# BaZzz01010101/ReflaxMan

Measured on AMD Instinct MI355X. Metric: Mrays/sec at 3840×2160 depth-8; max per-channel |Δ| vs CPU reference, higher is better.
Workload: dtype f32; 1 GPU; C3 synth16: 16 spheres + 4 textured triangles + sun, 3840x2160, depth 8, 1 spp; scene=synth16, width=3840, height=2160, depth=8, spp=1, parallelism=single-gpu

## Files before the change

### include/rfx.h

```cpp
#ifndef RFX_H
#define RFX_H
#include <stddef.h>
#include <stdint.h>

#ifdef __cplusplus
extern "C" {
#endif

#define RFX_ABI_VERSION 4

typedef enum {
  RFX_OK = 0,
  RFX_ERR_ARG = -1,
  RFX_ERR_HIP = -2,
  RFX_ERR_STATE = -3,
  RFX_ERR_IO = -4,
  RFX_ERR_RNG = -5,
  RFX_ERR_NODEV = -6
} rfx_status;

enum { RFX_METAL = 0, RFX_DIELECTRIC = 1 };

typedef struct rfx_scene rfx_scene;
typedef struct rfx_renderer rfx_renderer;
// ... 6 lines not shown
rfx_scene *rfx_scene_create(float diff_r, float diff_g, float diff_b, float diff_power);
void rfx_scene_destroy(rfx_scene *scene);
int rfx_scene_add_sphere(rfx_scene *scene, const float center[3], float radius, int material_type,
                         const float rgb[3], float reflectivity, float transparency);
int rfx_scene_add_triangle(rfx_scene *scene, const float v1[3], const float v2[3], const float v3[3],
                           int material_type, const float rgb[3], float reflectivity, float transparency);
int rfx_scene_add_mesh(rfx_scene *scene, const float *vertices, uint32_t n_vertices, const uint32_t *indices,
                       uint32_t n_triangles, int material_type, const float rgb[3], float reflectivity,
                       float transparency);
int rfx_scene_add_plane(rfx_scene *scene, const float pos[3], const float norm[3], int material_type,
                        const float rgb[3], float reflectivity, float transparency);
int rfx_scene_plane_count(const rfx_scene *scene);
int rfx_triangle_set_texture(rfx_scene *scene, int object_index, int texture_index, const float uv[6]);
int rfx_scene_add_light(rfx_scene *scene, const float origin[3], float radius, const float rgb[3], float power);
int rfx_scene_add_texture_argb(rfx_scene *scene, uint32_t width, uint32_t height, const uint32_t *argb);
int rfx_scene_add_texture_file(rfx_scene *scene, const char *path, int *loaded);
int rfx_scene_set_skybox_file(rfx_scene *scene, const char *path);
int rfx_scene_set_skybox_argb(rfx_scene *scene, uint32_t width, uint32_t height, const uint32_t *argb);
int rfx_scene_counts(const rfx_scene *scene, int *spheres, int *triangles, int *lights, int *textures);
int rfx_scene_tri_bvh_dump(const rfx_scene *scene, int32_t counts[5], float *boxes, int32_t *children,
                           int32_t *leaf_ids, int32_t *residual);
int rfx_scene_set_tri_mates(rfx_scene *scene, int on);
int rfx_scene_tri_mates(const rfx_scene *scene, int32_t *leader, float *plane);

void rfx_camera_view(const float eye[3], const float at[3], float view[9]);
float rfx_camera_rz(uint32_t width, float fov);

int rfx_tga_load(const char *path, uint32_t *width, uint32_t *height, uint32_t *argb, size_t capacity);
int rfx_tga_save(const char *path, uint32_t width, uint32_t height, const uint32_t *argb);
int rfx_bmp_save(const char *path, uint32_t width, uint32_t height, const uint32_t *argb);
void rfx_argb_from_rgb(const float *rgb, size_t pixels, uint32_t *argb);

int rfx_renderer_create(rfx_renderer **out, int device);
void rfx_renderer_destroy(rfx_renderer *r);
int rfx_renderer_device(const rfx_renderer *r);
int rfx_renderer_set_stream(rfx_renderer *r, void *hip_stream);
int rfx_renderer_set_scene(rfx_renderer *r, const rfx_scene *scene);
int rfx_renderer_set_tile_order(rfx_renderer *r, int mode);
int rfx_renderer_set_regroup(rfx_renderer *r, int park_after);
int rfx_renderer_set_regroup_sort(rfx_renderer *r, int on);
int rfx_renderer_bounce_form(const rfx_renderer *r);
int rfx_renderer_set_tri_accel(rfx_renderer *r, int mode);
typedef struct {
  int32_t tri_nodes, tri_depth;
  int32_t tri_leaf_size;
  int32_t tri_in_leaves;
  int32_t tri_residual;
  int32_t sph_nodes, sph_depth;
  int32_t narrow_tri_bvh;
} rfx_accel_info;
int rfx_renderer_accel_info(const rfx_renderer *r, rfx_accel_info *out);
int rfx_renderer_set_prim_masks(rfx_renderer *r, int mode);
int rfx_renderer_set_prim_exact(rfx_renderer *r, int on);
int rfx_renderer_get_prim_masks(rfx_renderer *r, uint64_t *host, uint64_t capacity, uint64_t *words);
int rfx_renderer_set_rng(rfx_renderer *r, uint32_t sphere_seed, uint32_t jitter_seed);
int rfx_renderer_get_rng(rfx_renderer *r, uint32_t *sphere_seed, uint32_t *jitter_seed);

typedef struct {
  float eye[3];
  float view[9];
  float fov;
  uint32_t width, height;
  int32_t reflect_num;
  int32_t sample_num;
  int32_t additive;
  int32_t additive_counter;
  uint32_t row_block;
  uint32_t rank, nranks;
  uint64_t pixel_begin;
  uint64_t pixel_end;
  uint64_t span_begin;
  uint64_t span_end;
} rfx_frame;

uint32_t rfx_strip_rows(uint32_t height, uint32_t row_block, uint32_t rank, uint32_t nranks);
uint32_t rfx_strip_row_to_y(uint32_t r, uint32_t row_block, uint32_t rank, uint32_t nranks);

#define RFX_NCOUNTERS 40
int rfx_render_frame(rfx_renderer *r, const rfx_frame *frame, float *d_rgb, uint32_t *d_argb,
                     uint64_t *d_counters, void *stream);
int rfx_renderer_set_launch_traces(rfx_renderer *r, uint64_t max_traces);
int rfx_renderer_set_rng_prepass(rfx_renderer *r, int mode);
int rfx_renderer_prepass_form(const rfx_renderer *r);
uint32_t rfx_rng_triple_index(uint32_t state);
uint32_t rfx_rng_seq_blocks(void);

int rfx_frame_rng_blocks(rfx_renderer *r, const rfx_frame *frame, uint32_t nslices, uint64_t *blocks_per_slice);
int rfx_frame_rng_count(rfx_renderer *r, const rfx_frame *frame, uint32_t slice, uint32_t nslices,
                        uint32_t *d_blk_counts, void *stream);
int rfx_render_frame_counted(rfx_renderer *r, const rfx_frame *frame, uint32_t nslices, const uint32_t *d_blk_counts,
                             float *d_rgb, uint32_t *d_argb, uint64_t *d_counters, void *stream);
int rfx_render_frame_counted_ev(rfx_renderer *r, const rfx_frame *frame, uint32_t nslices,
                                const uint32_t *d_blk_counts, float *d_rgb, uint32_t *d_argb, uint64_t *d_counters,
                                void *stream, void *emitted_event);

int rfx_frame_rng_emit(rfx_renderer *r, const rfx_frame *frame, uint32_t nslices, const uint32_t *d_blk_counts,
                       void *stream, void *emitted_event);
int rfx_render_frame_emitted(rfx_renderer *r, const rfx_frame *frame, float *d_rgb, uint32_t *d_argb,
                             uint64_t *d_counters, void *stream);
int rfx_frame_rng_discard(rfx_renderer *r);
int rfx_frame_rng_pending(rfx_renderer *r, uint32_t *frame_start);

int rfx_frame_rng_rewind(rfx_renderer *r);

typedef struct rfx_group rfx_group;
int rfx_group_create(rfx_group **out, const int *devices, int n);
void rfx_group_destroy(rfx_group *g);
int rfx_group_size(const rfx_group *g);
rfx_renderer *rfx_group_renderer(rfx_group *g, int member);
int rfx_group_set_scene(rfx_group *g, const rfx_scene *scene);
int rfx_group_set_bands(rfx_group *g, uint32_t height, const uint32_t *bounds);
int rfx_group_get_bands(const rfx_group *g, uint32_t *bounds);
int rfx_group_render_frame(rfx_group *g, const rfx_frame *frame, float *d_rgb, uint32_t *d_argb, void *stream);

int rfx_renderer_set_timing(rfx_renderer *r, int enable);
int rfx_renderer_get_timing(rfx_renderer *r, double *prepass_ms, double *trace_ms, uint64_t *frames);

int rfx_render_frame_host(rfx_renderer *r, const rfx_frame *frame, float *rgb, uint32_t *argb,
                          uint64_t *counters);

int rfx_device_alloc(rfx_renderer *r, size_t bytes, void **dptr);
int rfx_device_free(rfx_renderer *r, void *dptr);
int rfx_memcpy_d2h(rfx_renderer *r, void *dst, const void *src, size_t bytes);
int rfx_memcpy_h2d(rfx_renderer *r, void *dst, const void *src, size_t bytes);
int rfx_memcpy_d2d(rfx_renderer *r, void *dst, const void *src, size_t bytes);
int rfx_synchronize(rfx_renderer *r);

int rfx_rand_dirs(rfx_renderer *r, uint32_t seed, uint64_t n, float *out3, uint32_t *seed_out);

int rfx_kat_objects(rfx_renderer *r, const float *rays, const int32_t *objects, uint64_t n, float *out);
int rfx_kat_texels(rfx_renderer *r, int texture, const float *in, uint64_t n, float *out);
int rfx_kat_powf(rfx_renderer *r, const float *xy, uint64_t n, float *out);
int rfx_kat_argb(rfx_renderer *r, const float *rgb, uint64_t n, uint32_t *out);
int rfx_kat_powf_cube(rfx_renderer *r, uint64_t counts[2]);
int rfx_kat_div(rfx_renderer *r, uint64_t first, uint64_t n, uint64_t counts[3]);
int rfx_kat_kernarg(rfx_renderer *r, int swapped, uint32_t out[3]);
int rfx_kat_rng_seq_prefix(rfx_renderer *r, uint32_t *prefix);
int rfx_kat_rng_seq_legacy(rfx_renderer *r, uint32_t *counts);

#ifdef __cplusplus
}
#endif
#endif
```

### reflaxman_amd/_lib.py

```python
from __future__ import annotations

import ctypes as C
import os

from . import _build

RFX_OK = 0
RFX_NCOUNTERS = 40
RFX_ABI_VERSION = 4
METAL, DIELECTRIC = 0, 1

_fp = C.POINTER(C.c_float)
_u32p = C.POINTER(C.c_uint32)
_u64p = C.POINTER(C.c_uint64)


class RfxError(RuntimeError):
    pass


class Frame(C.Structure):
    _fields_ = [
        ("eye", C.c_float * 3), ("view", C.c_float * 9), ("fov", C.c_float),
        ("width", C.c_uint32), ("height", C.c_uint32),
        ("reflect_num", C.c_int32), ("sample_num", C.c_int32),
        ("additive", C.c_int32), ("additive_counter", C.c_int32),
        ("row_block", C.c_uint32), ("rank", C.c_uint32), ("nranks", C.c_uint32),
        ("pixel_begin", C.c_uint64), ("pixel_end", C.c_uint64),
        ("span_begin", C.c_uint64), ("span_end", C.c_uint64),
    ]


class AccelInfo(C.Structure):
    _fields_ = [(n, C.c_int32) for n in ("tri_nodes", "tri_depth", "tri_leaf_size", "tri_in_leaves", "tri_residual",
                                         "sph_nodes", "sph_depth", "narrow_tri_bvh")]


_i32p = C.POINTER(C.c_int32)

SIGNATURES = [
    ("rfx_abi_version", C.c_int, []),
    ("rfx_last_error", C.c_char_p, []),
    ("rfx_build_options", C.c_int, []),
    ("rfx_scene_create", C.c_void_p, [C.c_float] * 4),
    ("rfx_scene_destroy", None, [C.c_void_p]),
    ("rfx_scene_add_sphere", C.c_int, [C.c_void_p, _fp, C.c_float, C.c_int, _fp, C.c_float, C.c_float]),
    ("rfx_scene_add_triangle", C.c_int, [C.c_void_p, _fp, _fp, _fp, C.c_int, _fp, C.c_float, C.c_float]),
    ("rfx_scene_add_mesh", C.c_int, [C.c_void_p, _fp, C.c_uint32, _u32p, C.c_uint32, C.c_int, _fp, C.c_float, C.c_float]),
    ("rfx_scene_tri_bvh_dump", C.c_int, [C.c_void_p, _i32p, _fp, _i32p, _i32p, _i32p]),
    ("rfx_scene_set_tri_mates", C.c_int, [C.c_void_p, C.c_int]),
    ("rfx_scene_tri_mates", C.c_int, [C.c_void_p, _i32p, _fp]),
    ("rfx_scene_add_plane", C.c_int, [C.c_void_p, _fp, _fp, C.c_int, _fp, C.c_float, C.c_float]),
    ("rfx_scene_plane_count", C.c_int, [C.c_void_p]),
    ("rfx_triangle_set_texture", C.c_int, [C.c_void_p, C.c_int, C.c_int, _fp]),
    ("rfx_scene_add_light", C.c_int, [C.c_void_p, _fp, C.c_float, _fp, C.c_float]),
    ("rfx_scene_add_texture_argb", C.c_int, [C.c_void_p, C.c_uint32, C.c_uint32, _u32p]),
    ("rfx_scene_add_texture_file", C.c_int, [C.c_void_p, C.c_char_p, C.POINTER(C.c_int)]),
    ("rfx_scene_set_skybox_file", C.c_int, [C.c_void_p, C.c_char_p]),
    ("rfx_scene_set_skybox_argb", C.c_int, [C.c_void_p, C.c_uint32, C.c_uint32, _u32p]),
    ("rfx_scene_counts", C.c_int, [C.c_void_p] + [C.POINTER(C.c_int)] * 4),
    ("rfx_camera_view", None, [_fp, _fp, _fp]),
    ("rfx_camera_rz", C.c_float, [C.c_uint32, C.c_float]),
    ("rfx_tga_load", C.c_int, [C.c_char_p, _u32p, _u32p, _u32p, C.c_size_t]),
    ("rfx_tga_save", C.c_int, [C.c_char_p, C.c_uint32, C.c_uint32, _u32p]),
    ("rfx_bmp_save", C.c_int, [C.c_char_p, C.c_uint32, C.c_uint32, _u32p]),
    ("rfx_argb_from_rgb", None, [_fp, C.c_size_t, _u32p]),
    ("rfx_renderer_create", C.c_int, [C.POINTER(C.c_void_p), C.c_int]),
    ("rfx_renderer_destroy", None, [C.c_void_p]),
    ("rfx_renderer_device", C.c_int, [C.c_void_p]),
    ("rfx_renderer_set_stream", C.c_int, [C.c_void_p, C.c_void_p]),
    ("rfx_renderer_set_scene", C.c_int, [C.c_void_p, C.c_void_p]),
    ("rfx_renderer_set_rng", C.c_int, [C.c_void_p, C.c_uint32, C.c_uint32]),
    ("rfx_renderer_get_rng", C.c_int, [C.c_void_p, _u32p, _u32p]),
    ("rfx_strip_rows", C.c_uint32, [C.c_uint32] * 4),
    ("rfx_strip_row_to_y", C.c_uint32, [C.c_uint32] * 4),
    ("rfx_render_frame", C.c_int, [C.c_void_p, C.POINTER(Frame), C.c_void_p, C.c_void_p, C.c_void_p, C.c_void_p]),
    ("rfx_render_frame_host", C.c_int, [C.c_void_p, C.POINTER(Frame), _fp, _u32p, _u64p]),
    ("rfx_frame_rng_blocks", C.c_int, [C.c_void_p, C.POINTER(Frame), C.c_uint32, _u64p]),
    ("rfx_frame_rng_count", C.c_int, [C.c_void_p, C.POINTER(Frame), C.c_uint32, C.c_uint32, C.c_void_p, C.c_void_p]),
    ("rfx_render_frame_counted", C.c_int, [C.c_void_p, C.POINTER(Frame), C.c_uint32, C.c_void_p, C.c_void_p,
                                           C.c_void_p, C.c_void_p, C.c_void_p]),
    ("rfx_render_frame_counted_ev", C.c_int, [C.c_void_p, C.POINTER(Frame), C.c_uint32, C.c_void_p, C.c_void_p,
                                              C.c_void_p, C.c_void_p, C.c_void_p, C.c_void_p]),
    ("rfx_frame_rng_emit", C.c_int, [C.c_void_p, C.POINTER(Frame), C.c_uint32, C.c_void_p, C.c_void_p, C.c_void_p]),
    ("rfx_render_frame_emitted", C.c_int, [C.c_void_p, C.POINTER(Frame), C.c_void_p, C.c_void_p, C.c_void_p,
                                           C.c_void_p]),
    ("rfx_frame_rng_discard", C.c_int, [C.c_void_p]),
    ("rfx_frame_rng_pending", C.c_int, [C.c_void_p, _u32p]),
    ("rfx_frame_rng_rewind", C.c_int, [C.c_void_p]),
    ("rfx_group_create", C.c_int, [C.POINTER(C.c_void_p), C.POINTER(C.c_int), C.c_int]),
    ("rfx_group_destroy", None, [C.c_void_p]),
    ("rfx_group_size", C.c_int, [C.c_void_p]),
    ("rfx_group_renderer", C.c_void_p, [C.c_void_p, C.c_int]),
    ("rfx_group_set_scene", C.c_int, [C.c_void_p, C.c_void_p]),
    ("rfx_group_set_bands", C.c_int, [C.c_void_p, C.c_uint32, _u32p]),
    ("rfx_group_get_bands", C.c_int, [C.c_void_p, _u32p]),
    ("rfx_group_render_frame", C.c_int, [C.c_void_p, C.POINTER(Frame), C.c_void_p, C.c_void_p, C.c_void_p]),
    ("rfx_renderer_set_timing", C.c_int, [C.c_void_p, C.c_int]),
    ("rfx_renderer_set_tile_order", C.c_int, [C.c_void_p, C.c_int]),
    ("rfx_renderer_set_prim_masks", C.c_int, [C.c_void_p, C.c_int]),
    ("rfx_renderer_set_prim_exact", C.c_int, [C.c_void_p, C.c_int]),
    ("rfx_renderer_get_prim_masks", C.c_int, [C.c_void_p, _u64p, C.c_uint64, _u64p]),
    ("rfx_renderer_set_regroup", C.c_int, [C.c_void_p, C.c_int]),
    ("rfx_renderer_set_regroup_sort", C.c_int, [C.c_void_p, C.c_int]),
    ("rfx_renderer_set_launch_traces", C.c_int, [C.c_void_p, C.c_uint64]),
    ("rfx_renderer_bounce_form", C.c_int, [C.c_void_p]),
    ("rfx_renderer_set_rng_prepass", C.c_int, [C.c_void_p, C.c_int]),
    ("rfx_renderer_prepass_form", C.c_int, [C.c_void_p]),
    ("rfx_rng_triple_index", C.c_uint32, [C.c_uint32]),
    ("rfx_rng_seq_blocks", C.c_uint32, []),
    ("rfx_renderer_set_tri_accel", C.c_int, [C.c_void_p, C.c_int]),
    ("rfx_renderer_accel_info", C.c_int, [C.c_void_p, C.POINTER(AccelInfo)]),
    ("rfx_renderer_get_timing", C.c_int, [C.c_void_p, C.POINTER(C.c_double), C.POINTER(C.c_double), _u64p]),
    ("rfx_device_alloc", C.c_int, [C.c_void_p, C.c_size_t, C.POINTER(C.c_void_p)]),
    ("rfx_device_free", C.c_int, [C.c_void_p, C.c_void_p]),
    ("rfx_memcpy_d2h", C.c_int, [C.c_void_p, C.c_void_p, C.c_void_p, C.c_size_t]),
    ("rfx_memcpy_h2d", C.c_int, [C.c_void_p, C.c_void_p, C.c_void_p, C.c_size_t]),
    ("rfx_memcpy_d2d", C.c_int, [C.c_void_p, C.c_void_p, C.c_void_p, C.c_size_t]),
    ("rfx_synchronize", C.c_int, [C.c_void_p]),
    ("rfx_rand_dirs", C.c_int, [C.c_void_p, C.c_uint32, C.c_uint64, _fp, _u32p]),
    ("rfx_kat_objects", C.c_int, [C.c_void_p, _fp, C.POINTER(C.c_int32), C.c_uint64, _fp]),
    ("rfx_kat_texels", C.c_int, [C.c_void_p, C.c_int, _fp, C.c_uint64, _fp]),
    ("rfx_kat_powf", C.c_int, [C.c_void_p, _fp, C.c_uint64, _fp]),
    ("rfx_kat_argb", C.c_int, [C.c_void_p, _fp, C.c_uint64, _u32p]),
    ("rfx_kat_powf_cube", C.c_int, [C.c_void_p, C.POINTER(C.c_uint64)]),
    ("rfx_kat_div", C.c_int, [C.c_void_p, C.c_uint64, C.c_uint64, C.POINTER(C.c_uint64)]),
    ("rfx_kat_kernarg", C.c_int, [C.c_void_p, C.c_int, C.POINTER(C.c_uint32)]),
    ("rfx_kat_rng_seq_prefix", C.c_int, [C.c_void_p, _u32p]),
    ("rfx_kat_rng_seq_legacy", C.c_int, [C.c_void_p, _u32p]),
]

_lib = None


def lib_path() -> str:
    return _build.LIB


def bind(path: str, partial: bool = False):
    L = C.CDLL(os.path.abspath(path))
    for name, res, args in SIGNATURES:
        if partial and not hasattr(L, name):
            continue
        fn = getattr(L, name)
        fn.restype = res
        fn.argtypes = args
    return L


def load(build_if_missing: bool = True):
    global _lib
    if _lib is not None:
        return _lib
    path = _build.LIB
    if build_if_missing:
        try:
            _build.build()
        except Exception as e:
            if not os.path.exists(path):
                raise RfxError(f"librfx.so missing and cannot be built: {e}") from e
    if not os.path.exists(path):
        raise RfxError(f"librfx.so not found at {path}: the HIP renderer is required (no CPU fallback)")
    L = C.CDLL(path)
    for name, res, args in SIGNATURES:
        fn = getattr(L, name)
        fn.restype = res
        fn.argtypes = args
    if L.rfx_abi_version() != RFX_ABI_VERSION:
        raise RfxError("librfx.so ABI version mismatch")
    _lib = L
    return L


def lib_sha256(path: str = None) -> str:
    import hashlib
    with open(path or _build.LIB, "rb") as f:
        return hashlib.sha256(f.read()).hexdigest()


# ... 40 lines not shown
```

### reflaxman_amd/csrc/rfx_host.cpp

```cpp
#include <string.h>

#include <algorithm>

#include "rfx_internal.h"
#include "rfx_math.h"

#pragma clang fp contract(off)

using namespace rfx;

extern "C" int rfx_abi_version(void) { return RFX_ABI_VERSION; }

#ifndef RFX_TILE_ORDER_DEFAULT
#define RFX_TILE_ORDER_DEFAULT 1
#endif
#ifndef RFX_TILE_ORDER_MIN_TILES
#define RFX_TILE_ORDER_MIN_TILES 49152
#endif
#ifndef RFX_PRIM_SSAA
#define RFX_PRIM_SSAA 0
#endif
#ifndef RFX_PRIM_LANES
#define RFX_PRIM_LANES 1
#endif
// ... 153 lines not shown
  if (r->tile_stream) (void)hipStreamSynchronize(r->tile_stream);
  if (r->tile_fork) (void)hipEventDestroy(r->tile_fork);
  if (r->tile_join) (void)hipEventDestroy(r->tile_join);
  if (r->tile_stream) (void)hipStreamDestroy(r->tile_stream);
  if (r->split_stream)
  {
    (void)hipStreamSynchronize(r->split_stream);
    (void)hipStreamDestroy(r->split_stream);
  }
  for (hipEvent_t e : r->split_ev)
    if (e) (void)hipEventDestroy(e);
  if (r->own_stream) (void)hipStreamDestroy(r->own_stream);
  delete r;
}

extern "C" int rfx_build_options(void)
{
  return (RFX_PRIM_LARGE ? RFX_BUILD_PRIM_LARGE : 0) | (RFX_PRIM_SSAA ? RFX_BUILD_PRIM_SSAA : 0) |
         (RFX_PRIM_LANES ? RFX_BUILD_PRIM_LANES : 0) | (RFX_ONE_LIGHT ? RFX_BUILD_ONE_LIGHT : 0) |
         (RFX_BVH_LEAF_PAIRS << 8);
}

extern "C" int rfx_renderer_set_launch_traces(rfx_renderer *r, uint64_t max_traces)
{
  if (!r) return fail(RFX_ERR_ARG, "renderer_set_launch_traces: null renderer");
  r->launch_traces = max_traces ? std::min(max_traces, kMaxLaunchTraces) : (uint64_t)RFX_LAUNCH_TRACES;
  return RFX_OK;
}

extern "C" int rfx_renderer_device(const rfx_renderer *r) { return r ? r->device : -1; }

extern "C" int rfx_renderer_set_tile_order(rfx_renderer *r, int mode)
{
  if (!r || mode < 0 || mode > 3) return fail(RFX_ERR_ARG, "renderer_set_tile_order: mode 0, 1, 2 or 3");
  r->tile_mode = mode;
  return RFX_OK;
}

extern "C" int rfx_renderer_set_prim_masks(rfx_renderer *r, int mode)
{
  if (!r || mode < 0 || mode > 2) return fail(RFX_ERR_ARG, "renderer_set_prim_masks: mode 0, 1 or 2");
  r->prim_mode = mode;
  r->prim_key.clear();
  r->prim_seen.clear();
  return RFX_OK;
}

extern "C" int rfx_renderer_set_prim_exact(rfx_renderer *r, int on)
{
  if (!r || on < 0 || on > 1) return fail(RFX_ERR_ARG, "renderer_set_prim_exact: 0 or 1");
  r->prim_exact = on;
  r->prim_key.clear();
  return RFX_OK;
}

extern "C" int rfx_renderer_get_prim_masks(rfx_renderer *r, uint64_t *host, uint64_t capacity, uint64_t *words)
{
  if (!r || !words) return fail(RFX_ERR_ARG, "renderer_get_prim_masks: null argument");
  int rc;
  if ((rc = set_dev(r)) != RFX_OK) return rc;
  const uint64_t n = r->prim_key.empty() ? 0 : r->prim_words;
  *words = n;
  if (!n || !host) return RFX_OK;
  if (capacity < n) return fail(RFX_ERR_ARG, "renderer_get_prim_masks: the host array is too short");
  HIP_CHECK(hipStreamSynchronize(r->prim_on));
  HIP_CHECK(hipMemcpy(host, r->prim_mask.p, n * sizeof(uint64_t), hipMemcpyDeviceToHost));
  return RFX_OK;
}

extern "C" int rfx_renderer_set_rng_prepass(rfx_renderer *r, int mode)
{
  if (!r || mode < 0 || mode > 1) return fail(RFX_ERR_ARG, "renderer_set_rng_prepass: mode 0 or 1");
  r->rng_prepass = mode;
  return RFX_OK;
}

extern "C" int rfx_renderer_prepass_form(const rfx_renderer *r)
{
  if (!r) return fail(RFX_ERR_ARG, "renderer_prepass_form: null renderer");
  return r->rng.prepass_form;
}

extern "C" uint32_t rfx_rng_triple_index(uint32_t state) { return rng_seq_index_of(state); }

extern "C" int rfx_renderer_bounce_form(const rfx_renderer *r)
{
  if (!r) return fail(RFX_ERR_ARG, "renderer_bounce_form: null renderer");
  return r->bounce_form;
}

extern "C" int rfx_renderer_set_regroup(rfx_renderer *r, int park_after)
{
  if (!r || park_after < -1) return fail(RFX_ERR_ARG, "renderer_set_regroup: -1 (default), 0 (off) or segments >= 1");
  r->park_after = park_after;
  return RFX_OK;
}

extern "C" int rfx_renderer_set_regroup_sort(rfx_renderer *r, int on)
{
  if (!r || on < 0 || on > 1) return fail(RFX_ERR_ARG, "renderer_set_regroup_sort: 0 or 1");
  r->queue_sort = on;
  return RFX_OK;
}

extern "C" int rfx_renderer_set_stream(rfx_renderer *r, void *s)
{
  if (!r) return fail(RFX_ERR_ARG, "set_stream: null renderer");
  r->stream = s ? (hipStream_t)s : r->own_stream;
  return RFX_OK;
}

template <class T>
static int upload(rfx_renderer *r, const std::vector<T> &v, const T **dst)
{
  if (v.empty()) { *dst = nullptr; return RFX_OK; }
  void *p = nullptr;
  HIP_CHECK(hipMalloc(&p, v.size() * sizeof(T)));
  r->scene_allocs.push_back(p);
  HIP_CHECK(hipMemcpy(p, v.data(), v.size() * sizeof(T), hipMemcpyHostToDevice));
  *dst = (const T *)p;
  return RFX_OK;
}

extern "C" int rfx_renderer_set_tri_accel(rfx_renderer *r, int mode)
{
  if (!r || mode < -1 || mode > 2)
    return fail(RFX_ERR_ARG, "renderer_set_tri_accel: -1 (automatic), 0 (off), 1 (on) or 2 (on, narrow bundles too)");
  r->tri_accel = mode;
  return RFX_OK;
}

extern "C" int rfx_renderer_accel_info(const rfx_renderer *r, rfx_accel_info *out)
{
  if (!r || !out) return fail(RFX_ERR_ARG, "renderer_accel_info: bad args");
  if (!r->has_scene) return fail(RFX_ERR_STATE, "renderer_accel_info: no scene");
  *out = r->accel;
  return RFX_OK;
}

extern "C" int rfx_renderer_set_scene(rfx_renderer *r, const rfx_scene *s)
{
  if (!r || !s) return fail(RFX_ERR_ARG, "set_scene: bad args");
  int rc;
  if ((rc = set_dev(r)) != RFX_OK) return rc;
  HIP_CHECK(hipStreamSynchronize(r->stream));
  free_scene(r);
  const SceneBuild B(*s, r->tri_accel);
  DevScene d = B.d;
  if ((rc = upload(r, B.sg, &d.sph_geo)) || (rc = upload(r, B.sp, &d.sph_pair)) || (rc = upload(r, B.sm, &d.sph_mat)) ||
      (rc = upload(r, B.si, &d.sph_info)) || (rc = upload(r, B.tg, &d.tri_geo)) || (rc = upload(r, B.ts, &d.tri_shade)) ||
      (rc = upload(r, B.tm, &d.tri_mat)) || (rc = upload(r, B.lr, &d.lights)) || (rc = upload(r, B.tr, &d.texs)) ||
      (rc = upload(r, B.pool, &d.texels)) || (rc = upload(r, B.bd, &d.bound)) || (rc = upload(r, B.cs, &d.cull_small)) ||
      (rc = upload(r, B.ct, &d.cull_tri)) || (rc = upload(r, B.cb, &d.chunk_bound)) || (rc = upload(r, B.pg, &d.pln_geo)) ||
      (rc = upload(r, B.pm, &d.pln_mat)) || (rc = upload(r, B.loc, &d.obj_loc)) || (rc = upload(r, B.bvh, &d.bvh)) ||
      (rc = upload(r, B.tt.nodes, &d.tri_bvh)) || (rc = upload(r, B.tleaf, &d.tri_leaf)) ||
      (rc = upload(r, B.tt.resid, &d.tri_resid)) || (rc = upload(r, B.aux, &d.bvh_aux)))
    return rc;
  r->accel = B.accel;
  r->dev = d;
  r->has_scene = true;
  ++r->scene_gen;
  r->prim_key.clear();
  r->prim_seen.clear();
  return RFX_OK;
}

extern "C" int rfx_renderer_set_rng(rfx_renderer *r, uint32_t sphere_seed, uint32_t jitter_seed)
{
  if (!r) return fail(RFX_ERR_ARG, "set_rng: null renderer");
  int rc;
  if ((rc = set_dev(r)) != RFX_OK) return rc;
  HIP_CHECK(hipMemcpyAsync(r->rng.cur(), &sphere_seed, sizeof(uint32_t), hipMemcpyHostToDevice, r->stream));
  HIP_CHECK(hipStreamSynchronize(r->stream));
  r->jitter_seed = jitter_seed;
  r->rng.rewind_ok = false;
  r->rng.reset(false);
  return RFX_OK;
}

extern "C" int rfx_renderer_get_rng(rfx_renderer *r, uint32_t *sphere_seed, uint32_t *jitter_seed)
{
  if (!r) return fail(RFX_ERR_ARG, "get_rng: null renderer");
  int rc;
  if ((rc = set_dev(r)) != RFX_OK) return rc;
  uint32_t s = 0;
  int err = 0;
  HIP_CHECK(hipMemcpyAsync(&s, r->rng.cur(), sizeof(uint32_t), hipMemcpyDeviceToHost, r->stream));
  HIP_CHECK(hipMemcpyAsync(&err, r->err, sizeof(int), hipMemcpyDeviceToHost, r->stream));
  HIP_CHECK(hipStreamSynchronize(r->stream));
  if (err & 1) return fail(RFX_ERR_RNG, "RNG pre-pass ran short of accepted triples");
  if (sphere_seed) *sphere_seed = s;
  if (jitter_seed) *jitter_seed = r->jitter_seed;
  return RFX_OK;
}

static uint64_t rng_layout(uint64_t traces, uint32_t nslices, uint64_t *per_slice)
{
  if (!nslices) nslices = 1;
  const uint64_t bps = (rng_blocks_for(traces) + nslices - 1) / nslices;
  if (per_slice) *per_slice = bps;
  return bps * nslices;
}

static int ensure_rng_workspace(rfx_renderer *r, uint64_t traces, uint64_t nblk)
{
  int rc;
  if ((rc = r->rd.reserve(traces)) < 0) return rc;
  if (nblk <= r->blk_cnt.cap) return RFX_OK;
  r->blk_cnt.release();
  if ((rc = r->rng_status.reserve(nblk)) < 0 || (rc = r->blk_off.reserve(nblk)) < 0 ||
      (rc = r->tile_sum.reserve(nblk / 4096 + 1)) < 0 || (rc = r->rng_range.reserve(4)) < 0 ||
// ... 75 lines not shown
  uint32_t grid_rows, row0;
  if (f->sample_num < 0)
  {
    const uint64_t n = (uint64_t)(-f->sample_num);
    const uint64_t bw = (W + n - 1) / n;
    auto corners_before = [&](uint64_t p) -> uint64_t {
      const uint64_t y = p / W, x = p % W;
      return (y + n - 1) / n * bw + (y % n == 0 ? (x + n - 1) / n : 0);
    };
    trace_base = corners_before(p0);
    traces = corners_before(p1) - trace_base;
    row0 = (uint32_t)(y0 / n);
    grid_rows = (uint32_t)(y1 / n - y0 / n + 1);
  }
  else
  {
    traces = (p1 - p0) * (uint64_t)(f->sample_num * f->sample_num);
    row0 = nranks > 1 ? 0 : y0;
    grid_rows = nranks > 1 ? rfx_strip_rows(H, f->row_block, f->rank, nranks) : y1 - y0 + 1;
    if (band)
    {
      row0 = (uint32_t)(f->pixel_begin / W);
      grid_rows = (uint32_t)((f->pixel_end - f->pixel_begin) / W);
    }
  }
  if (traces > kMaxLaunchTraces)
    return fail(RFX_ERR_ARG, "render_frame: %llu traces in one launch exceed 2^31 (partitions: a smaller span)",
                (unsigned long long)traces);
  plan.traces = traces;
  plan.st = st;
  FrameParams &P = plan.P;
  P = FrameParams{};
  P.eye_x = f->eye[0]; P.eye_y = f->eye[1]; P.eye_z = f->eye[2];
  P.v11 = f->view[0]; P.v12 = f->view[1]; P.v13 = f->view[2];
  P.v21 = f->view[3]; P.v22 = f->view[4]; P.v23 = f->view[5];
  P.v31 = f->view[6]; P.v32 = f->view[7]; P.v33 = f->view[8];
  P.rz = rfx_camera_rz(W, f->fov);
  P.wh = W / 2.0f;
  P.hh = H / 2.0f;
  P.W = W; P.H = H;
  P.depth = f->reflect_num;
  P.ss = f->sample_num;
  P.accumulate = f->sample_num > 0 && f->additive_counter > 1;
  P.additive = f->sample_num > 0 && f->additive;
  P.jitter_seed = r->jitter_seed;
  P.row_block = f->row_block ? f->row_block : 1;
  P.rank = nranks > 1 && !band ? f->rank : 0;
  P.nranks = band ? 1 : nranks;
  P.grid_rows = grid_rows;
  P.row0 = row0;
  P.p_begin = p0;
  P.p_end = p1;
  P.trace_base = trace_base;
  return RFX_OK;
}

extern "C" int rfx_frame_rng_blocks(rfx_renderer *r, const rfx_frame *f, uint32_t nslices, uint64_t *per_slice)
{
  FramePlan pl;
  int rc;
  if ((rc = plan_frame(r, f, nullptr, pl)) != RFX_OK) return rc;
  if (!nslices || !per_slice) return fail(RFX_ERR_ARG, "frame_rng_blocks: nslices > 0 and an output required");
  rng_layout(pl.traces, nslices, per_slice);
  return RFX_OK;
}

extern "C" int rfx_frame_rng_count(rfx_renderer *r, const rfx_frame *f, uint32_t slice, uint32_t nslices,
                                   uint32_t *d_blk_counts, void *stream)
{
  FramePlan pl;
  int rc;
  if ((rc = plan_frame(r, f, stream, pl)) != RFX_OK) return rc;
  if (!d_blk_counts || !nslices || slice >= nslices) return fail(RFX_ERR_ARG, "frame_rng_count: bad slice");
  uint64_t bps = 0;
  const uint64_t nblk = rng_layout(pl.traces, nslices, &bps);
  if ((rc = ensure_rng_workspace(r, pl.rd_traces(), nblk)) != RFX_OK) return rc;
  HIP_CHECK(launch_rng_count(r->rng.cur(), r->jump, d_blk_counts, (uint64_t)slice * bps, bps, nullptr, pl.st));
  return RFX_OK;
}

static int tile_schedule(rfx_renderer *r, FrameParams &P, hipStream_t st, uint64_t &key, bool &record)
{
  int rc;
  const uint32_t n = trace_tiles(P);
  key = ((uint64_t)P.W << 40) ^ ((uint64_t)P.grid_rows << 16) ^ ((uint64_t)(uint32_t)P.ss << 4) ^
        (uint64_t)(P.additive * 2 + P.accumulate);
  if (!r->tile_stream)
  {
    HIP_CHECK(hipStreamCreateWithFlags(&r->tile_stream, hipStreamNonBlocking));
    HIP_CHECK(hipEventCreateWithFlags(&r->tile_fork, hipEventDisableTiming));
    HIP_CHECK(hipEventCreateWithFlags(&r->tile_join, hipEventDisableTiming));
  }
  if ((rc = r->tile_scratch.reserve(tile_order_scratch() / sizeof(uint32_t))) < 0) return rc;
  if (n > r->tile_cost.cap)
  {
    HIP_CHECK(hipStreamSynchronize(r->tile_stream));
    if (r->tile_pending) HIP_CHECK(hipEventSynchronize(r->tile_join));
    HIP_CHECK(hipStreamSynchronize(st));
    r->tile_n = 0;
    r->tile_pending = false;
    r->tile_cost.release();
    if ((rc = r->tile_order.reserve(n)) < 0 || (rc = r->tile_cost.reserve(n)) < 0) return rc;
  }
  if (r->tile_pending && r->tile_waited != st)
  {
    HIP_CHECK(hipStreamWaitEvent(st, r->tile_join, 0));
// ... 139 lines not shown
    DevBuf<uint64_t> &mask = r->split_mask[pl.split_side];
    if ((rc = mask.reserve((size_t)trace_tiles(P) * kPrimStride)) < 0) return rc;
    HIP_CHECK(launch_prim_cull(r->dev, P, mask, r->prim_exact != 0, st));
    P.prim_mask = mask;
    P.prim_shadow = 0;
  }
  else if (((small && (plain || (RFX_PRIM_LANES && (trace_lanes(P) || chunks)) || (RFX_PRIM_SSAA && P.ss >= 1)) &&
             !park) ||
            (RFX_PRIM_LARGE && !small && plain)) &&
           !stats && P.grid_rows && r->prim_mode && !pl.split)
  {
    struct Key { float cam[15]; uint32_t W, H, grid_rows, row0, row_block, rank, nranks; int32_t depth, ss, additive;
                 uint64_t p_begin, p_end, gen; } k;
    memset(&k, 0, sizeof(k));
    const float cam[15] = {P.eye_x, P.eye_y, P.eye_z, P.v11, P.v12, P.v13, P.v21, P.v22, P.v23,
                           P.v31, P.v32, P.v33, P.rz, P.wh, P.hh};
    memcpy(k.cam, cam, sizeof(cam));
    k.W = P.W; k.H = P.H; k.grid_rows = P.grid_rows; k.row0 = P.row0; k.row_block = P.row_block; k.rank = P.rank;
    k.nranks = P.nranks; k.depth = P.depth > 0 ? 1 : 0; k.p_begin = P.p_begin; k.p_end = P.p_end; k.gen = r->scene_gen;
    k.ss = P.ss; k.additive = P.additive ? 1 : 0;
    std::vector<uint8_t> kb((const uint8_t *)&k, (const uint8_t *)&k + sizeof(k));
    if ((rc = r->prim_mask.reserve((size_t)trace_tiles(P) * (small ? kPrimStride : kPrimLargeStride))) < 0) return rc;
    if (rc)
    {
      r->prim_key.clear();
      r->prim_seen.clear();
    }
    if (r->prim_mode == 2 || kb != r->prim_key)
    {
      const bool repeat = kb == r->prim_seen;
      r->prim_seen = kb;
      r->prim_key.clear();
      if (repeat || r->prim_mode == 2 || chunks)
      {
        HIP_CHECK(launch_prim_cull(r->dev, P, r->prim_mask, r->prim_exact != 0, st));
        r->prim_key = kb;
        r->prim_words = (size_t)trace_tiles(P) * (small ? kPrimStride : kPrimLargeStride);
        r->prim_on = st;
      }
    }
    if (!r->prim_key.empty())
    {
      P.prim_mask = r->prim_mask;
      P.prim_shadow = P.additive || chunks ? 0 : 1;
    }
  }
  return RFX_OK;
}

static int launch_trace_and_bounce(rfx_renderer *r, FramePlan &pl, bool small, bool park, bool sort_queue, bool stats)
{
  const FrameParams &P = pl.P;
  const hipStream_t st = pl.st;
  if (P.grid_rows) HIP_CHECK(launch_trace(r->dev, P, stats, st));
  r->bounce_form = 0;
  if (!park) return RFX_OK;
  const uint64_t waves = (pl.traces + 63) / 64;
  const uint32_t groups = (uint32_t)std::min<uint64_t>((waves + 1) / 2, (uint64_t)r->cus * RFX_BOUNCE_GROUPS_PER_CU);
  const int cfg = kCfgCull | (r->dev.n_light > 32 ? kCfgManyLights : 0) | (small ? kCfgSmall : 0) |
                  (r->dev.n_pln ? kCfgPlanes : 0) | (RFX_ONE_LIGHT && r->dev.n_light == 1 ? kCfgOneLight : 0) |
                  (RFX_TRI_BVH && r->dev.tri_bvh ? kCfgTriBvh : 0);
  if (sort_queue) HIP_CHECK(launch_queue_sort(r->qctr, r->qkey, r->qctr.p + 2, r->qorder, st));
  const uint32_t lgroups = (uint32_t)std::min<uint64_t>((waves + kLdsBvhWaves - 1) / kLdsBvhWaves, (uint64_t)r->cus);
  r->bounce_form = 2;
  if (small || !lds_bvh_fits(r->dev.n_bvh) || launch_bounce_lds(cfg, lgroups, r->dev, P, st) != hipSuccess)
  {
    (void)hipGetLastError();
    launch_bounce(cfg, dim3(groups), r->dev, P, st);
    r->bounce_form = 1;
  }
  HIP_CHECK(hipGetLastError());
  return RFX_OK;
}

static int record_tile_sort(rfx_renderer *r, const FramePlan &pl, uint64_t key)
{
  const hipStream_t st = pl.st;
  const uint32_t n = trace_tiles(pl.P);
#if RFX_TILE_SORT_MAIN
  HIP_CHECK(launch_tile_order(r->tile_cost, n, r->tile_order, r->tile_scratch, st));
  HIP_CHECK(hipEventRecord(r->tile_join, st));
  r->tile_waited = st;
#else
  HIP_CHECK(hipEventRecord(r->tile_fork, st));
  HIP_CHECK(hipStreamWaitEvent(r->tile_stream, r->tile_fork, 0));
  HIP_CHECK(launch_tile_order(r->tile_cost, n, r->tile_order, r->tile_scratch, r->tile_stream));
  HIP_CHECK(hipEventRecord(r->tile_join, r->tile_stream));
  r->tile_waited = nullptr;
#endif
  r->tile_pending = true;
  r->tile_n = n;
  r->tile_key = key;
  return RFX_OK;
}

static int trace_frame(rfx_renderer *r, FramePlan &pl, const uint32_t *rd, float *d_rgb, uint32_t *d_argb,
                       uint64_t *d_counters)
{
  int rc;
  FrameParams &P = pl.P;
  const bool stats = d_counters != nullptr;
  P.img = d_rgb;
  P.argb = d_argb;
  P.rd_state = pl.band ? rd - pl.band_lo : rd;
  P.counters = (unsigned long long *)d_counters;
  const bool small = r->dev.n_sph <= 32 && r->dev.n_tri <= 32;
  const bool plain = P.ss == 1 && !P.additive && !P.accumulate;
// ... 339 lines not shown
```

### reflaxman_amd/csrc/rfx_internal.h

```cpp
#pragma once
#include <hip/hip_runtime.h>
#include <stdint.h>

#include <vector>

#include "rfx_launch.h"
#include "rfx_scene.h"

#define HIP_CHECK(expr)                                                                          \
  do {                                                                                           \
    hipError_t e_ = (expr);                                                                      \
    if (e_ != hipSuccess) return rfx::fail(RFX_ERR_HIP, "%s: %s", #expr, hipGetErrorString(e_)); \
  } while (0)
#define RCHECK(expr)               \
  do {                             \
    int rc_ = (expr);              \
    if (rc_ != RFX_OK) return rc_; \
  } while (0)

namespace rfx {

template <class T>
struct DevBuf {
  T *p = nullptr;
// ... 68 lines not shown

}

struct rfx_renderer {
  rfx_renderer();
  int device = 0;
  int cus = 256;
  hipStream_t own_stream = nullptr;
  hipStream_t stream = nullptr;
  rfx::DevScene dev{};
  std::vector<void *> scene_allocs;
  bool has_scene = false;
  rfx::RngState rng;
  rfx::DevBuf<int> err;
  uint32_t jitter_seed = 0;
  rfx::DevBuf<uint32_t> rd;
  rfx::DevBuf<uint32_t> rd_alt;
  int emit_pending = -1;
  int trace_buf = 0;
  bool split_alt_busy = false;
  uint64_t emit_key[10] = {};
  uint64_t launch_traces;
  hipStream_t split_stream = nullptr;
  hipEvent_t split_ev[3] = {nullptr, nullptr, nullptr};
  rfx::DevBuf<uint32_t> blk_cnt, rng_range, tile_sum, jump;
  rfx::DevBuf<uint64_t> blk_off;
  rfx::DevBuf<uint16_t> rng_masks;
  rfx::DevBuf<unsigned long long> rng_status, rng_ticket;
  unsigned long long rng_tickets = 0;
  uint32_t rng_epoch = 0;
  rfx::DevBuf<uint32_t> seq_hdr, seq_state, seq_p, seq_tiles;
  bool seq_built = false;
  int rng_prepass;
  rfx::DevBuf<float> img;
  rfx::DevBuf<uint32_t> argb;
  rfx::DevBuf<uint64_t> cnt;
  int tile_mode;
  rfx::DevBuf<uint32_t> tile_cost, tile_order, tile_scratch;
  uint32_t tile_n = 0;
  uint64_t tile_key = 0;
  hipStream_t tile_stream = nullptr;
  hipEvent_t tile_fork = nullptr, tile_join = nullptr;
  bool tile_pending = false;
  hipStream_t tile_waited = nullptr;
  uint64_t tile_count = 0;
  int park_after = -1;
  rfx::DevBuf<uint64_t> prim_mask;
  rfx::DevBuf<uint64_t> split_mask[2];
  std::vector<uint8_t> prim_key;
  std::vector<uint8_t> prim_seen;
  uint64_t scene_gen = 0;
  int prim_mode = 1;
  int prim_exact = 1;
  size_t prim_words = 0;
  hipStream_t prim_on = nullptr;
  int tri_accel = -1;
  rfx_accel_info accel{};
  int bounce_form = 0;
  rfx::DevBuf<rfx::QRay> queue;
  rfx::DevBuf<uint32_t> qctr, qkey, qorder;
  int queue_sort;
  bool timing = false, timing_this = false;
  uint32_t timing_every = 1;
  uint64_t timing_seq = 0;
  std::vector<hipEvent_t> events;
  size_t events_used = 0;
};

namespace rfx {
int set_dev(rfx_renderer *r);
int ensure_seq_table(rfx_renderer *r, hipStream_t st);
int save_rewind_state(rfx_renderer *r, hipStream_t st);
}
```

### reflaxman_amd/csrc/rfx_kat.cpp

```cpp
#include <algorithm>
#include <string>
#include <vector>

#include "rfx_internal.h"

using namespace rfx;

static int named(const char *who, int rc)
{
  const std::string cause = rfx_last_error();
  return fail(rc, "%s: %s", who, cause.c_str());
}

template <class T>
static int kat_buffer(DevBuf<T> &dev, size_t n, const T *src)
{
  int rc;
  if ((rc = dev.reserve(n ? n : 1)) < 0) return rc;
  if (src && n) HIP_CHECK(hipMemcpy(dev, src, n * sizeof(T), hipMemcpyHostToDevice));
  return RFX_OK;
}

static int kat_run(rfx_renderer *r, int what, int tex, const void *in, size_t in_elems, const int32_t *objs,
                   uint64_t n, void *out, size_t out_elems)
// ... 26 lines not shown
  if (!r->has_scene) return fail(RFX_ERR_STATE, "kat_texels: no scene uploaded");
  if (texture >= r->dev.n_tex) return fail(RFX_ERR_ARG, "kat_texels: texture %d", texture);
  return kat_run(r, 1, texture, in, (size_t)n * (texture >= 0 ? 2 : 3), nullptr, n, out, (size_t)n * 3);
}

extern "C" int rfx_kat_powf(rfx_renderer *r, const float *xy, uint64_t n, float *out)
{
  if (!r || (n && (!xy || !out))) return fail(RFX_ERR_ARG, "kat_powf: bad args");
  return kat_run(r, 2, 0, xy, (size_t)n * 2, nullptr, n, out, (size_t)n);
}

extern "C" int rfx_kat_argb(rfx_renderer *r, const float *rgb, uint64_t n, uint32_t *out)
{
  if (!r || (n && (!rgb || !out))) return fail(RFX_ERR_ARG, "kat_argb: bad args");
  return kat_run(r, 3, 0, rgb, (size_t)n * 3, nullptr, n, out, (size_t)n);
}

extern "C" int rfx_kat_powf_cube(rfx_renderer *r, uint64_t counts[2])
{
  if (!r || !counts) return fail(RFX_ERR_ARG, "kat_powf_cube: bad args");
  DevBuf<unsigned long long> d;
  int rc;
  if ((rc = d.reserve(2)) < 0) return named("kat_powf_cube", rc);
  hipError_t e = hipMemsetAsync(d, 0, 2 * sizeof(unsigned long long), r->stream);
  for (uint64_t first = 0; e == hipSuccess && first <= 0x3f800000ull; first += 1ull << 28)
    e = launch_kat_powf_cube((uint32_t)first, (uint32_t)std::min<uint64_t>(1ull << 28, 0x3f800001ull - first), d, r->stream);
  unsigned long long h[2] = {0, 0};
  if (e == hipSuccess) e = hipStreamSynchronize(r->stream);
  if (e == hipSuccess) e = hipMemcpy(h, d, sizeof(h), hipMemcpyDeviceToHost);
  if (e != hipSuccess) return fail(RFX_ERR_HIP, "kat_powf_cube: %s", hipGetErrorString(e));
  counts[0] = h[0];
  counts[1] = h[1];
  return RFX_OK;
}

extern "C" int rfx_kat_div(rfx_renderer *r, uint64_t first, uint64_t n, uint64_t counts[3])
{
  if (!r || !counts) return fail(RFX_ERR_ARG, "kat_div: bad args");
  RCHECK(set_dev(r));
  DevBuf<unsigned long long> d;
  int rc;
  if ((rc = d.reserve(3)) < 0) return named("kat_div", rc);
  hipError_t e = hipMemsetAsync(d, 0, 3 * sizeof(unsigned long long), r->stream);
  for (uint64_t k = 0; e == hipSuccess && k < n; k += 1ull << 28)
    e = launch_kat_div(first + k, (uint32_t)std::min<uint64_t>(1ull << 28, n - k), d, r->stream);
  unsigned long long h[3] = {0, 0, 0};
  if (e == hipSuccess) e = hipStreamSynchronize(r->stream);
  if (e == hipSuccess) e = hipMemcpy(h, d, sizeof(h), hipMemcpyDeviceToHost);
  if (e != hipSuccess) return fail(RFX_ERR_HIP, "kat_div: %s", hipGetErrorString(e));
  for (int i = 0; i < 3; ++i) counts[i] = h[i];
  return RFX_OK;
}

extern "C" uint32_t rfx_rng_seq_blocks(void) { return rng_seq_blocks(); }

extern "C" int rfx_kat_rng_seq_prefix(rfx_renderer *r, uint32_t *prefix)
{
  if (!r || !prefix) return fail(RFX_ERR_ARG, "kat_rng_seq_prefix: bad args");
  RCHECK(set_dev(r));
  RCHECK(ensure_seq_table(r, r->stream));
  HIP_CHECK(hipStreamSynchronize(r->stream));
  HIP_CHECK(hipMemcpy(prefix, r->seq_p, ((size_t)rng_seq_blocks() + 1) * sizeof(uint32_t), hipMemcpyDeviceToHost));
  return RFX_OK;
}

extern "C" int rfx_kat_rng_seq_legacy(rfx_renderer *r, uint32_t *counts)
{
  if (!r || !counts) return fail(RFX_ERR_ARG, "kat_rng_seq_legacy: bad args");
  RCHECK(set_dev(r));
  const uint64_t nb = rng_seq_blocks();
  std::vector<uint32_t> jump(2 * (256 + nb));
  rng_jump_table(nb, jump.data());
  DevBuf<uint32_t> d_jump, d_cnt, d_origin;
  int rc;
  if ((rc = d_jump.reserve(jump.size())) < 0 || (rc = d_cnt.reserve(nb)) < 0 || (rc = d_origin.reserve(1)) < 0)
    return named("kat_rng_seq_legacy", rc);
  hipError_t e = hipMemcpy(d_jump, jump.data(), jump.size() * sizeof(uint32_t), hipMemcpyHostToDevice);
  if (e == hipSuccess) e = hipMemset(d_origin, 0, sizeof(uint32_t));
  if (e == hipSuccess) e = launch_rng_count(d_origin, d_jump, d_cnt, 0, nb, nullptr, r->stream);
  if (e == hipSuccess) e = hipStreamSynchronize(r->stream);
  if (e == hipSuccess) e = hipMemcpy(counts, d_cnt, nb * sizeof(uint32_t), hipMemcpyDeviceToHost);
  if (e != hipSuccess) return fail(RFX_ERR_HIP, "kat_rng_seq_legacy: %s", hipGetErrorString(e));
  return RFX_OK;
}

extern "C" int rfx_kat_kernarg(rfx_renderer *r, int swapped, uint32_t out[3])
{
  if (!r || !out) return fail(RFX_ERR_ARG, "kat_kernarg: bad args");
  if (!r->has_scene) return fail(RFX_ERR_STATE, "kat_kernarg: no scene uploaded");
  RCHECK(set_dev(r));
  FrameParams P;
  uint32_t *w = (uint32_t *)&P;
  for (size_t i = 0; i < sizeof(P) / 4; ++i) w[i] = 0x9E3779B9u * (uint32_t)(i + 1);
  DevBuf<uint32_t> d;
  int rc;
  if ((rc = d.reserve(3)) < 0) return named("kat_kernarg", rc);
  hipError_t e = hipMemsetAsync(d, 0xFF, 3 * sizeof(uint32_t), r->stream);
  if (e == hipSuccess) e = launch_kat_kernarg(r->dev, P, swapped, d, r->stream);
  if (e == hipSuccess) e = hipStreamSynchronize(r->stream);
  if (e == hipSuccess) e = hipMemcpy(out, d, 3 * sizeof(uint32_t), hipMemcpyDeviceToHost);
  if (e != hipSuccess) return fail(RFX_ERR_HIP, "kat_kernarg: %s", hipGetErrorString(e));
  return RFX_OK;
}
```

### reflaxman_amd/csrc/rfx_kernels.hip

```cpp
#include "rfx_trace.h"

#include <vector>

#pragma clang fp contract(off)

namespace rfx {

constexpr int kLptThreads = 1024, kLptBuckets = 256, kLptGroups = 64;

__device__ __forceinline__ uint32_t lpt_key(const uint32_t *cost, uint32_t i)
{
  const uint32_t c = max(cost[i], 1u);
  const uint32_t e = 31u - (uint32_t)__clz(c);
  const uint32_t m = e >= 3u ? (c >> (e - 3u)) & 7u : (c << (3u - e)) & 7u;
  return (uint32_t)(kLptBuckets - 1) - min(e * 8u + m, (uint32_t)(kLptBuckets - 1));
}

__global__ __launch_bounds__(kLptThreads) void lpt_hist(const uint32_t *cost, uint32_t n, uint32_t chunk, uint32_t *hist)
{
  __shared__ uint32_t h[kLptBuckets];
  for (uint32_t b = threadIdx.x; b < kLptBuckets; b += kLptThreads) h[b] = 0;
  __syncthreads();
  const uint32_t i0 = blockIdx.x * chunk, i1 = min(n, i0 + chunk);
  for (uint32_t i = i0 + threadIdx.x; i < i1; i += kLptThreads) atomicAdd(&h[lpt_key(cost, i)], 1u);
// ... 969 lines not shown
      case 2:
      {
        const float edge = (h1 & 1u) ? 0x1p100f : 0x1p-40f;
        b = __uint_as_float(__float_as_uint(edge) + (int32_t)((h1 >> 1) % 7u) - 3) * ((h1 & 2u) ? -1.0f : 1.0f);
        const int32_t qe = (h2 % 3u == 0) ? -60 : (h2 % 3u == 1) ? 60 : 0;
        a = b * kat_float(h2 >> 31, qe + (int32_t)((h2 >> 2) % 5u) - 2, h0 >> 3);
        break;
      }
      case 3:
      {
        const uint32_t m = h1 % 3u;
        a = m == 0 ? ((h1 & 8u) ? -0.0f : 0.0f) : m == 1 ? __uint_as_float((h1 & 0x807FFFFFu)) : kat_float(h1 >> 31, -126 + (int32_t)(h2 % 40u), h2);
        b = kat_float(h2 >> 31, (int32_t)(h0 % 141u) - 40, h1 >> 3);
        break;
      }
      case 4: b = kat_float(h1 >> 31, (int32_t)((h1 >> 1) % 3u) - 1, h2); a = kat_float(h2 >> 31, (int32_t)(h0 % 253u) - 126, h1 >> 4); break;
      case 5: a = kat_float(h1 >> 31, (int32_t)(h0 % 253u) - 126, h2); b = kat_float(h2 >> 31, (int32_t)(h1 % 253u) - 126, h0); break;
      case 6: b = kat_float(h1 >> 31, (int32_t)(h0 % 141u) - 40, h2); a = b * __uint_as_float(0x3f800000u + (h2 & 0xFu) - 8u); break;
      default: b = kat_float(h1 >> 31, (int32_t)(h0 % 253u) - 126, 0u); a = kat_float(h2 >> 31, (int32_t)(h1 % 253u) - 126, h2 >> 1); break;
    }
    const float q = div_rn(a, b);
    bool ok;
    (void)div_fast(a, div_prep(b), ok);
    const float a2 = __uint_as_float(__float_as_uint(a) ^ (h2 & 0x807F0000u)), a3 = b * -0.5f;
    const v3 v = mk(a, a2, a3), nv = normalized(v);
    const float l = len(v);
    const bool sv = l > kVerySmall;
    const float rx = sv ? v.x / l : v.x, ry = sv ? v.y / l : v.y, rz = sv ? v.z / l : v.z;
    const float den = fabsf(b) + kVerySmall, p = fabsf(a) <= den ? a : copysignf(den, a) * 0.75f;
    bool okp;
    float pd = div_fast_unit(p, den, rcp_refined(den), okp);
    const bool unit_ok = den <= 0x1p64f;
    if (!okp) pd = p / den;
    bad = (kat_same(q, a / b) ? 0u : 1u) + (kat_same(nv.x, rx) ? 0u : 1u) + (kat_same(nv.y, ry) ? 0u : 1u) +
          (kat_same(nv.z, rz) ? 0u : 1u) + (!unit_ok || kat_same(pd, p / den) ? 0u : 1u);
    fast = ok ? 1u : 0u;
    seen = 5;
  }
#pragma unroll
  for (int o = 32; o > 0; o >>= 1)
  {
    bad += __shfl_xor(bad, o, 64);
    fast += __shfl_xor(fast, o, 64);
    seen += __shfl_xor(seen, o, 64);
  }
  if ((threadIdx.x & 63u) == 0 && seen)
  {
    if (bad) atomicAdd(&counts[0], (unsigned long long)bad);
    atomicAdd(&counts[1], (unsigned long long)fast);
    atomicAdd(&counts[2], (unsigned long long)seen);
  }
}

template <bool SWAPPED>
__device__ __forceinline__ void kernarg_compare(const DevScene &S, const FrameParams &P, uint32_t *out)
{
  const uint32_t *ps = (const uint32_t *)&P, *qs = (const uint32_t *)&kernarg_params();
  uint32_t bad_p = 0, bad_s = 0;
  for (size_t i = 0; i < sizeof(FrameParams) / 4; ++i) bad_p += ps[i] != qs[i] ? 1u : 0u;
#ifdef RFX_LAUNDER_SCENE
  const uint32_t *a = (const uint32_t *)&S, *b = (const uint32_t *)&launder_scene<true>(S);
  for (size_t i = 0; i < sizeof(DevScene) / 4; ++i) bad_s += a[i] != b[i] ? 1u : 0u;
  out[2] = 1;
#else
  out[2] = 0;
#endif
  out[0] = bad_s;
  out[1] = bad_p;
}
__global__ void kat_kernarg(DevScene S, FrameParams P, uint32_t *out)
{
  if (threadIdx.x == 0 && blockIdx.x == 0) kernarg_compare<false>(S, P, out);
}
__global__ void kat_kernarg_swapped(FrameParams P, DevScene S, uint32_t *out)
{
  if (threadIdx.x == 0 && blockIdx.x == 0) kernarg_compare<true>(S, P, out);
}

__global__ __launch_bounds__(kKatThreads) void kat_argb(const float *rgb, uint32_t n, uint32_t *out)
{
  const uint32_t i = blockIdx.x * kKatThreads + threadIdx.x;
  if (i < n) out[i] = argb(mkc(rgb[3 * (size_t)i], rgb[3 * (size_t)i + 1], rgb[3 * (size_t)i + 2]));
}

}



namespace rfx {

uint64_t rng_blocks_for(uint64_t traces)
{
  const uint64_t triples = 2 * traces + 65536;
  return (triples + kTriplesPerBlock - 1) / kTriplesPerBlock;
}

void rng_jump_table(uint64_t nblk, uint32_t *out)
{
  uint32_t a1 = 1u, c1 = 0u;
  for (int i = 0; i < 3 * kTriplesPerThread; ++i) { c1 = 214013u * c1 + 2531011u; a1 = 214013u * a1; }
  uint32_t A = 1u, C = 0u;
  for (int t = 0; t < kRngBlock; ++t)
  {
    out[2 * t] = A; out[2 * t + 1] = C;
    C = a1 * C + c1; A = a1 * A;
  }
// ... 118 lines not shown
                               uint64_t nblk, uint64_t traces, uint32_t *d_rd_state, uint32_t *d_next_seed,
                               uint32_t *d_next_pos, int *d_err, hipStream_t st)
{
  hipLaunchKernelGGL(rng_emit_seq, dim3((uint32_t)nblk), dim3(kRngBlock), 0, st, d_pos, d_state, d_hdr, d_p, traces,
                     d_rd_state, d_next_seed, d_next_pos, d_err);
  return hipGetLastError();
}

static void launch_mode_cfg(bool stats, int mode, int cfg, dim3 grid, const DevScene &S, const FrameParams &P,
                            hipStream_t st)
{
  if (mode == kModeBlock) (stats ? launch_trace_block_stats : launch_trace_block_fast)(cfg, grid, S, P, st);
  else if (mode == kModePlain)
  {
    if (stats) launch_trace_plain_stats(cfg, grid, S, P, st);
    else if (P.park_after > 0) launch_trace_plain_park(cfg, grid, S, P, st);
    else launch_trace_plain_fast(cfg, grid, S, P, st);
  }
  else if (mode == kModeSsaaLanes) (stats ? launch_trace_lanes_stats : launch_trace_lanes_fast)(cfg, grid, S, P, st);
  else if (mode == kModeSsaaChunks) (stats ? launch_trace_chunks_stats : launch_trace_chunks_fast)(cfg, grid, S, P, st);
  else (stats ? launch_trace_ssaa_stats : launch_trace_ssaa_fast)(cfg, grid, S, P, st);
}

static dim3 kat_grid(uint32_t n) { return dim3((n + kKatThreads - 1) / kKatThreads); }

hipError_t launch_kat_kernarg(const DevScene &S, const FrameParams &P, int swapped, uint32_t *out, hipStream_t st)
{
  if (swapped) hipLaunchKernelGGL(kat_kernarg_swapped, dim3(1), dim3(64), 0, st, P, S, out);
  else hipLaunchKernelGGL(kat_kernarg, dim3(1), dim3(64), 0, st, S, P, out);
  return hipGetLastError();
}

hipError_t launch_kat(int what, const DevScene &S, int tex, const void *in, const int32_t *objs, uint32_t n, void *out,
                      hipStream_t st)
{
  if (!n) return hipSuccess;
  switch (what)
  {
    case 0: hipLaunchKernelGGL(kat_objects, kat_grid(n), dim3(kKatThreads), 0, st, S, (const float *)in, objs, n, (float *)out); break;
    case 1: hipLaunchKernelGGL(kat_texels, kat_grid(n), dim3(kKatThreads), 0, st, S, tex, (const float *)in, n, (float *)out); break;
    case 2: hipLaunchKernelGGL(kat_powf, kat_grid(n), dim3(kKatThreads), 0, st, (const float *)in, n, (float *)out); break;
    default: hipLaunchKernelGGL(kat_argb, kat_grid(n), dim3(kKatThreads), 0, st, (const float *)in, n, (uint32_t *)out); break;
  }
  return hipGetLastError();
}

hipError_t launch_kat_div(uint64_t first, uint32_t n, unsigned long long *counts, hipStream_t st)
{
  if (!n) return hipSuccess;
  hipLaunchKernelGGL(kat_div, kat_grid(n), dim3(kKatThreads), 0, st, first, n, counts);
  return hipGetLastError();
}

hipError_t launch_kat_powf_cube(uint32_t first, uint32_t n, unsigned long long *counts, hipStream_t st)
{
  if (!n) return hipSuccess;
  hipLaunchKernelGGL(kat_powf_cube, kat_grid(n), dim3(kKatThreads), 0, st, first, n, counts);
  return hipGetLastError();
}

#ifndef RFX_NOCULL_MAX_TILES
#define RFX_NOCULL_MAX_TILES 0
#endif

static int trace_mode(const FrameParams &P)
{
  if (P.ss < 0) return kModeBlock;
  if (P.ss == 1 && !P.additive && !P.accumulate) return kModePlain;
  if (!RFX_SSAA_LANES || !ss_lane_block(P.ss)) return kModeSsaa;
  return P.ss > 8 ? kModeSsaaChunks : kModeSsaaLanes;
}

static dim3 trace_grid(const FrameParams &P)
{
  const int mode = trace_mode(P);
  if (mode == kModeSsaaLanes || mode == kModeSsaaChunks)
  {
    const uint32_t bw = ss_lane_block(P.ss);
    return dim3((P.W + kTileWavesX * bw - 1) / (kTileWavesX * bw), (P.grid_rows + kTileWavesY * bw - 1) / (kTileWavesY * bw));
  }
  const uint32_t cols = P.ss < 0 ? (P.W + (uint32_t)(-P.ss) - 1) / (uint32_t)(-P.ss) : P.W;
  return dim3((cols + kTileW - 1) / kTileW, (P.grid_rows + kTileH - 1) / kTileH);
}

uint32_t trace_tiles(const FrameParams &P)
{
  const dim3 g = trace_grid(P);
  return kWgWaves * g.x * g.y;
}

bool trace_lanes(const FrameParams &P)
{
  return trace_mode(P) == kModeSsaaLanes;
}

bool trace_chunks(const FrameParams &P)
{
  return trace_mode(P) == kModeSsaaChunks;
}

hipError_t launch_prim_cull(const DevScene &S, const FrameParams &P, uint64_t *masks, bool narrow, hipStream_t st)
{
  const int nw = narrow ? 1 : 0;
  const dim3 grid = trace_grid(P);
  if (!(S.n_sph <= 32 && S.n_tri <= 32))
    hipLaunchKernelGGL(prim_cull_large_kernel<0>, grid, dim3(kWgThreads), 0, st, S, P, masks);
  else if (trace_lanes(P) || trace_chunks(P))
  {
    if (S.n_pln > 0)
      hipLaunchKernelGGL((prim_cull_kernel<true, true>), grid, dim3(kWgThreads), 0, st, S, P, masks, nw);
    else
      hipLaunchKernelGGL((prim_cull_kernel<false, true>), grid, dim3(kWgThreads), 0, st, S, P, masks, nw);
  }
  else if (S.n_pln > 0)
    hipLaunchKernelGGL(prim_cull_kernel<true>, grid, dim3(kWgThreads), 0, st, S, P, masks, nw);
  else
    hipLaunchKernelGGL(prim_cull_kernel<false>, grid, dim3(kWgThreads), 0, st, S, P, masks, nw);
  return hipGetLastError();
}

hipError_t launch_trace(const DevScene &S, const FrameParams &P, bool stats, hipStream_t st)
{
  const dim3 grid = trace_grid(P);
  FrameParams Pt = P;
  Pt.tiles_x = kTileWavesX * grid.x;
  const int mode = trace_mode(P);
  const bool cull = !stats && !(RFX_NOCULL_MAX_TILES > 0 && S.n_sph <= 32 && S.n_tri <= 32 &&
                                trace_tiles(P) <= (uint32_t)RFX_NOCULL_MAX_TILES);
  const int cfg = (S.n_light > 32 ? kCfgManyLights : 0) | (cull ? kCfgCull : 0) |
                  (S.n_sph <= 32 && S.n_tri <= 32 ? kCfgSmall : 0) | (S.n_pln > 0 ? kCfgPlanes : 0) |
                  (S.n_light == 1 && !stats && RFX_ONE_LIGHT ? kCfgOneLight : 0) |
                  (RFX_TRI_BVH && S.tri_bvh != nullptr && !stats ? kCfgTriBvh : 0);
  launch_mode_cfg(stats, mode, cfg, grid, S, Pt, st);
  return hipGetLastError();
}

}
```

### reflaxman_amd/csrc/rfx_launch.h

```cpp
#pragma once
#include <hip/hip_runtime.h>

#include "rfx_types.h"

namespace rfx {
uint64_t rng_blocks_for(uint64_t traces);
void rng_jump_table(uint64_t nblk, uint32_t *out);
hipError_t launch_rng_count(const uint32_t *d_seed, const uint32_t *d_jump, uint32_t *d_blk_cnt, uint64_t blk0,
                            uint64_t nblk_slice, uint16_t *d_masks, hipStream_t st);
hipError_t launch_rng_finish(const uint32_t *d_seed, const uint32_t *d_jump, uint32_t *d_next_seed,
                             const uint32_t *d_blk_cnt, const uint16_t *d_masks, uint64_t nblk, uint64_t traces,
                             uint32_t *d_rd_state, int *d_err, uint64_t ss2, uint64_t W, uint32_t row_block,
                             uint32_t rank, uint32_t nranks, hipStream_t st);
hipError_t launch_rng_finish_band(const uint32_t *d_seed, const uint32_t *d_jump, uint32_t *d_next_seed,
                                  const uint32_t *d_blk_cnt, const uint16_t *d_masks, uint64_t nblk, uint64_t traces,
                                  uint32_t *d_rd_state, int *d_err, uint64_t lo, uint64_t hi, uint64_t *d_off,
                                  uint32_t *d_range, uint32_t *d_tile_sum, hipStream_t st);
hipError_t launch_rng_fused(const uint32_t *d_seed, const uint32_t *d_jump, uint32_t *d_next_seed, uint64_t nblk,
                            uint64_t traces, uint32_t *d_rd_state, int *d_err, unsigned long long *d_status,
                            unsigned long long *d_ticket, unsigned long long base, uint32_t epoch, hipStream_t st);
uint32_t rng_seq_blocks();
uint32_t rng_seq_header_words();
void rng_seq_tables(uint32_t *hdr, uint32_t *state);
uint32_t rng_seq_index_of(uint32_t s);
hipError_t launch_rng_seq_build(const uint32_t *d_hdr, const uint32_t *d_state, uint32_t *d_p, uint32_t *d_tiles,
                                hipStream_t st);
hipError_t launch_rng_locate(const uint32_t *d_seed, const uint32_t *d_hdr, const uint32_t *d_state, const uint32_t *d_p,
                             uint32_t *d_pos, hipStream_t st);
hipError_t launch_rng_emit_seq(const uint32_t *d_pos, const uint32_t *d_hdr, const uint32_t *d_state, const uint32_t *d_p,
                               uint64_t nblk, uint64_t traces, uint32_t *d_rd_state, uint32_t *d_next_seed,
                               uint32_t *d_next_pos, int *d_err, hipStream_t st);
hipError_t launch_trace(const DevScene &S, const FrameParams &P, bool stats, hipStream_t st);
hipError_t launch_prim_cull(const DevScene &S, const FrameParams &P, uint64_t *masks, bool narrow, hipStream_t st);
hipError_t launch_queue_sort(const uint32_t *count, const uint32_t *key, uint32_t *hist, uint32_t *order, hipStream_t st);
uint32_t trace_tiles(const FrameParams &P);
bool trace_lanes(const FrameParams &P);
bool trace_chunks(const FrameParams &P);
size_t tile_order_scratch();
hipError_t launch_tile_order(const uint32_t *cost, uint32_t n, uint32_t *order, uint32_t *scratch, hipStream_t st);
hipError_t launch_kat(int what, const DevScene &S, int tex, const void *in, const int32_t *objs, uint32_t n, void *out,
                      hipStream_t st);
hipError_t launch_kat_powf_cube(uint32_t first, uint32_t n, unsigned long long *counts, hipStream_t st);
hipError_t launch_kat_div(uint64_t first, uint32_t n, unsigned long long *counts, hipStream_t st);
hipError_t launch_kat_kernarg(const DevScene &S, const FrameParams &P, int swapped, uint32_t *out, hipStream_t st);
#define RFX_DECLARE_TRACE_FAMILY(name) \
  void name(int cfg, dim3 grid, const DevScene &S, const FrameParams &P, hipStream_t st)
RFX_DECLARE_TRACE_FAMILY(launch_trace_plain_fast);
RFX_DECLARE_TRACE_FAMILY(launch_trace_plain_stats);
RFX_DECLARE_TRACE_FAMILY(launch_trace_ssaa_fast);
RFX_DECLARE_TRACE_FAMILY(launch_trace_ssaa_stats);
RFX_DECLARE_TRACE_FAMILY(launch_trace_lanes_fast);
RFX_DECLARE_TRACE_FAMILY(launch_trace_lanes_stats);
RFX_DECLARE_TRACE_FAMILY(launch_trace_chunks_fast);
RFX_DECLARE_TRACE_FAMILY(launch_trace_chunks_stats);
RFX_DECLARE_TRACE_FAMILY(launch_trace_block_fast);
RFX_DECLARE_TRACE_FAMILY(launch_trace_block_stats);
RFX_DECLARE_TRACE_FAMILY(launch_trace_plain_park);
RFX_DECLARE_TRACE_FAMILY(launch_bounce);
hipError_t launch_bounce_lds(int cfg, uint32_t groups, const DevScene &S, const FrameParams &P, hipStream_t st);
}
```

### reflaxman_amd/csrc/rfx_math.h

```cpp
#pragma once
#include <stdint.h>
#include <string.h>

#if defined(__HIPCC__)
#include <hip/hip_runtime.h>
#define RFX_HD __host__ __device__ __forceinline__
#else
#include <math.h>
#define RFX_HD static inline
#endif

#pragma clang fp contract(off)

namespace rfx {

constexpr float kVerySmall = 1.0842021724855044e-19f;
constexpr float kDelta = 0.0001f;
constexpr float kFltEpsilon = 1.1920928955078125e-07f;
constexpr float kFltMax = 3.402823466e+38f;

RFX_HD float sqrt_rn(float x)
{
#if defined(__HIP_DEVICE_COMPILE__)
  if (x >= 0x1p-96f)
  {
    const float s = __builtin_amdgcn_sqrtf(x);
    const float s_dn = __uint_as_float(__float_as_uint(s) - 1u), s_up = __uint_as_float(__float_as_uint(s) + 1u);
    const float r_dn = __builtin_fmaf(-s_dn, s, x), r_up = __builtin_fmaf(-s_up, s, x);
    const float t = r_dn <= 0.0f ? s_dn : s;
    return r_up > 0.0f ? s_up : t;
  }
#endif
  return sqrtf(x);
}

#ifndef RFX_DIV_FAST
#define RFX_DIV_FAST 1
#endif
struct DivRcp { float b, r; };
RFX_HD DivRcp div_prep(float b)
{
  DivRcp d;
  d.b = b;
#if defined(__HIP_DEVICE_COMPILE__) && RFX_DIV_FAST
  const float r = __builtin_amdgcn_rcpf(b);
  const float e = __builtin_fmaf(-b, r, 1.0f);
  const float r1 = __builtin_fmaf(e, r, r);
  d.r = (RFX_DIV_FAST == 2 || (fabsf(b) >= 0x1p-40f && fabsf(b) <= 0x1p100f)) ? r1 : __builtin_nanf("");
#else
  d.r = 0.0f;
#endif
  return d;
}
RFX_HD float div_fast(float a, const DivRcp &d, bool &ok)
{
#if defined(__HIP_DEVICE_COMPILE__) && RFX_DIV_FAST
  const float q0 = a * d.r;
  const float t1 = __builtin_fmaf(-d.b, q0, a);
  const float q1 = __builtin_fmaf(t1, d.r, q0);
  const float t2 = __builtin_fmaf(-d.b, q1, a);
  const float q = __builtin_fmaf(t2, d.r, q1);
  ok = RFX_DIV_FAST == 2 || (fabsf(q) >= 0x1p-60f && fabsf(q) <= 0x1p60f);
  return q;
#else
  ok = false;
  return a / d.b;
#endif
}
RFX_HD float div_by(float a, const DivRcp &d)
{
  bool ok;
  const float q = div_fast(a, d, ok);
  if (__builtin_expect(!ok, 0)) return a / d.b;
  return q;
}
RFX_HD float div_rn(float a, float b) { return div_by(a, div_prep(b)); }
#ifndef RFX_DIV_SINGLE
#define RFX_DIV_SINGLE 0
#endif
RFX_HD float qdiv(float a, float b)
{
#if RFX_DIV_SINGLE
  return div_rn(a, b);
#else
  return a / b;
#endif
}

struct v3 { float x, y, z; };
struct col { float r, g, b; };
struct m33 { float m11, m12, m13, m21, m22, m23, m31, m32, m33; };

RFX_HD v3 mk(float x, float y, float z) { v3 v; v.x = x; v.y = y; v.z = z; return v; }
RFX_HD v3 add(v3 a, v3 b) { return mk(a.x + b.x, a.y + b.y, a.z + b.z); }
RFX_HD v3 sub(v3 a, v3 b) { return mk(a.x - b.x, a.y - b.y, a.z - b.z); }
RFX_HD v3 mul(v3 a, float f) { return mk(a.x * f, a.y * f, a.z * f); }
RFX_HD v3 neg(v3 a) { return mk(-a.x, -a.y, -a.z); }
RFX_HD float dot(v3 a, v3 b) { return a.x * b.x + a.y * b.y + a.z * b.z; }
RFX_HD float sqlen(v3 a) { return a.x * a.x + a.y * a.y + a.z * a.z; }
RFX_HD float len(v3 a) { return sqrt_rn(a.x * a.x + a.y * a.y + a.z * a.z); }
RFX_HD v3 cross(v3 a, v3 b)
{
  return mk(a.y * b.z - a.z * b.y, a.z * b.x - a.x * b.z, a.x * b.y - a.y * b.x);
}
RFX_HD v3 divv(v3 a, float f)
{
  if (fabsf(f) > kVerySmall) return mk(a.x / f, a.y / f, a.z / f);
  return a;
}
RFX_HD float div_fast_unit(float a, float b, float r, bool &ok)
{
#if defined(__HIP_DEVICE_COMPILE__) && RFX_DIV_FAST
  const float q0 = a * r;
  const float t1 = __builtin_fmaf(-b, q0, a);
  const float q1 = __builtin_fmaf(t1, r, q0);
  const float t2 = __builtin_fmaf(-b, q1, a);
  const float q = __builtin_fmaf(t2, r, q1);
  ok = RFX_DIV_FAST == 2 || fabsf(q) >= 0x1p-38f;
  return q;
#else
  ok = false;
  return a / b;
#endif
}
RFX_HD float rcp_refined(float b)
{
#if defined(__HIP_DEVICE_COMPILE__) && RFX_DIV_FAST
  const float r = __builtin_amdgcn_rcpf(b);
  return __builtin_fmaf(__builtin_fmaf(-b, r, 1.0f), r, r);
#else
  return 1.0f / b;
#endif
}
RFX_HD v3 normalized(v3 a)
{
  const float l = len(a);
  if (l > kVerySmall)
  {
#if defined(__HIP_DEVICE_COMPILE__) && RFX_DIV_FAST
    const float r = rcp_refined(l);
    bool ox, oy, oz;
    const v3 q = mk(div_fast_unit(a.x, l, r, ox), div_fast_unit(a.y, l, r, oy), div_fast_unit(a.z, l, r, oz));
    if (__builtin_expect(ox && oy && oz, 1)) return q;
#endif
    return divv(a, l);
  }
  return a;
}
RFX_HD v3 reflect(v3 v, v3 n)
{
  const float dn = dot(n, n);
  if (dn > kVerySmall) return sub(v, mul(mul(n, 2.0f), qdiv(dot(v, n), dn)));
  return v;
}
RFX_HD float clampf(float v, float lo, float hi) { return v < lo ? lo : v > hi ? hi : v; }

RFX_HD uint32_t f2u(float f) { uint32_t u; memcpy(&u, &f, 4); return u; }
RFX_HD float u2f(uint32_t u) { float f; memcpy(&f, &u, 4); return f; }
RFX_HD float sq_lower_bound(float y)
{
  const double m = ((double)u2f(f2u(y) - 1u) + (double)y) * 0.5;
  const double m2 = m * m;
  float f = (float)m2;
  if ((double)f <= m2) f = u2f(f2u(f) + 1u);
  return f;
}
constexpr float kSqDeltaSphere = 0x1.5798fp-27f;

RFX_HD m33 from_cols(v3 u, v3 v, v3 n)
{
  m33 m;
  m.m11 = u.x; m.m12 = v.x; m.m13 = n.x;
  m.m21 = u.y; m.m22 = v.y; m.m23 = n.y;
  m.m31 = u.z; m.m32 = v.z; m.m33 = n.z;
  return m;
}
RFX_HD v3 mmul(const m33 &m, v3 v)
{
  return mk(v.x * m.m11 + v.y * m.m12 + v.z * m.m13,
            v.x * m.m21 + v.y * m.m22 + v.z * m.m23,
            v.x * m.m31 + v.y * m.m32 + v.z * m.m33);
}
RFX_HD m33 inverted(const m33 &a)
{
  const float d = a.m11 * (a.m22 * a.m33 - a.m32 * a.m23) +
                  a.m21 * (a.m32 * a.m13 - a.m12 * a.m33) +
                  a.m31 * (a.m12 * a.m23 - a.m13 * a.m22);
  m33 r;
  if (fabsf(d) > kVerySmall)
  {
    r.m11 = (a.m22 * a.m33 - a.m23 * a.m32) / d;
    r.m12 = (a.m13 * a.m32 - a.m12 * a.m33) / d;
    r.m13 = (a.m12 * a.m23 - a.m13 * a.m22) / d;
    r.m21 = (a.m23 * a.m31 - a.m21 * a.m33) / d;
    r.m22 = (a.m11 * a.m33 - a.m13 * a.m31) / d;
    r.m23 = (a.m13 * a.m21 - a.m11 * a.m23) / d;
    r.m31 = (a.m21 * a.m32 - a.m22 * a.m31) / d;
    r.m32 = (a.m12 * a.m31 - a.m11 * a.m32) / d;
    r.m33 = (a.m11 * a.m22 - a.m12 * a.m21) / d;
  }
  else
  {
    r.m11 = 1; r.m12 = 0; r.m13 = 0; r.m21 = 0; r.m22 = 1; r.m23 = 0; r.m31 = 0; r.m32 = 0; r.m33 = 1;
  }
  return r;
// ... 54 lines not shown
```

### reflaxman_amd/csrc/rfx_scene.cpp

```cpp
#include <math.h>
#include <stdarg.h>
#include <stdio.h>
#include <stdlib.h>
#include <string.h>

#include <algorithm>
#include <array>
#include <cmath>
#include <map>
#include <string>
#include <vector>

#include "rfx_math.h"
#include "rfx_scene.h"

#pragma clang fp contract(off)

using namespace rfx;

static thread_local std::string g_last_error;

int rfx::fail(int code, const char *fmt, ...)
{
  char buf[512];
// ... 605 lines not shown
    if (boxes)
      for (int c = 0; c < 2; ++c)
      {
        float *b = boxes + 12 * i + 6 * c;
        b[0] = n.lx[c]; b[1] = n.ly[c]; b[2] = n.lz[c]; b[3] = n.hx[c]; b[4] = n.hy[c]; b[5] = n.hz[c];
      }
    if (children) { children[2 * i] = n.child[0]; children[2 * i + 1] = n.child[1]; }
  }
  if (leaf_ids) std::copy(T.order.begin(), T.order.end(), leaf_ids);
  if (residual) std::copy(T.resid.begin(), T.resid.end(), residual);
  return 1;
}

static std::vector<int32_t> tri_mate_leaders(const std::vector<HostTri> &tris, bool on)
{
  std::vector<int32_t> leader(tris.size());
  std::map<std::array<uint32_t, 6>, int32_t> first;
  for (size_t i = 0; i < tris.size(); ++i)
  {
    const HostTri &t = tris[i];
    leader[i] = (int32_t)i;
    const float row[3] = {t.ax.m31, t.ax.m32, t.ax.m33}, v0[3] = {t.v0.x, t.v0.y, t.v0.z};
    bool finite = on;
    std::array<uint32_t, 6> key{};
    for (int a = 0; a < 3; ++a)
    {
      finite = finite && std::isfinite(row[a]) && std::isfinite(v0[a]);
      memcpy(&key[a], &row[a], 4);
      if (row[a] != 0.0f) memcpy(&key[3 + a], &v0[a], 4);
    }
    if (finite) leader[i] = first.emplace(key, (int32_t)i).first->second;
  }
  return leader;
}

extern "C" int rfx_scene_set_tri_mates(rfx_scene *s, int on)
{
  if (!s || on < 0 || on > 1) return fail(RFX_ERR_ARG, "scene_set_tri_mates: 0 or 1");
  s->tri_mates = on;
  return RFX_OK;
}

extern "C" int rfx_scene_tri_mates(const rfx_scene *s, int32_t *leader, float *plane)
{
  if (!s) return fail(RFX_ERR_ARG, "scene_tri_mates: null scene");
  const std::vector<int32_t> l = tri_mate_leaders(s->tris, s->tri_mates != 0);
  if (leader) std::copy(l.begin(), l.end(), leader);
  if (plane)
    for (const HostTri &t : s->tris)
      for (float f : {t.v0.x, t.v0.y, t.v0.z, t.ax.m31, t.ax.m32, t.ax.m33}) *plane++ = f;
  return (int)l.size();
}

SceneBuild::SceneBuild(const rfx_scene &scene, int tri_accel)
{
  const rfx_scene *s = &scene;
  const size_t nsph = s->spheres.size();
  std::vector<uint32_t> order(nsph);
  for (size_t i = 0; i < nsph; ++i) order[i] = (uint32_t)i;
  if (nsph > 32) spatial_order(order, 0, nsph, s->spheres);

  for (uint32_t oi : order)
  {
    const HostSphere &hs = s->spheres[oi];
    sg.push_back({hs.center.x, hs.center.y, hs.center.z, hs.sq_radius});
    sm.push_back({hs.mat.r, hs.mat.g, hs.mat.b, hs.mat.refl});
    si.push_back(hs.obj);
    si.push_back(hs.mat.dielectric);
  }
  const size_t npair_dev = sg.size() > 32 ? ((sg.size() + 1) / 2 + RFX_BVH_LEAF_PAIRS - 1) / RFX_BVH_LEAF_PAIRS *
                                                RFX_BVH_LEAF_PAIRS
                                          : (sg.size() + 1) / 2;
  sp.assign(npair_dev, SpherePair{});
  for (size_t i = 0; i < 2 * sp.size(); ++i)
  {
    SpherePair &p = sp[i / 2];
    const int l = (int)(i & 1);
    const bool real = i < sg.size();
    p.cx[l] = real ? sg[i].cx : 0.0f;
    p.cy[l] = real ? sg[i].cy : 0.0f;
    p.cz[l] = real ? sg[i].cz : 0.0f;
    p.r2[l] = real ? sg[i].sq_radius : -INFINITY;
  }
  for (const HostTri &t : s->tris)
  {
    TriGeo g{};
    g.v0x = t.v0.x; g.v0y = t.v0.y; g.v0z = t.v0.z;
    g.a11 = t.ax.m11; g.a12 = t.ax.m12; g.a13 = t.ax.m13;
    g.a21 = t.ax.m21; g.a22 = t.ax.m22; g.a23 = t.ax.m23;
    g.a31 = t.ax.m31; g.a32 = t.ax.m32; g.a33 = t.ax.m33;
    tg.push_back(g);
    TriShade h{};
    h.nx = t.norm.x; h.ny = t.norm.y; h.nz = t.norm.z;
    h.tu0 = t.tu0; h.tv0 = t.tv0;
    h.t11 = t.tuv.m11; h.t12 = t.tuv.m12; h.t21 = t.tuv.m21; h.t22 = t.tuv.m22;
    h.tex = t.tex; h.dielectric = t.mat.dielectric; h.obj = t.obj;
    ts.push_back(h);
    tm.push_back({t.mat.r, t.mat.g, t.mat.b, t.mat.refl});
  }
  const std::vector<int32_t> leader = tri_mate_leaders(s->tris, s->tri_mates != 0);
  for (size_t i = 0; i < tg.size(); ++i) memcpy(&tg[i].pad[0], &leader[i], 4);
  for (uint32_t oi : order)
  {
    const HostSphere &hs = s->spheres[oi];
    bd.push_back({hs.center.x, hs.center.y, hs.center.z, hs.radius * 1.00001f});
  }
  for (size_t first = 0; first < nsph; first += 64)
// ... 216 lines not shown
```

### reflaxman_amd/csrc/rfx_scene.h

```cpp
#pragma once
#include <stdint.h>

#include <vector>

#include "../../include/rfx.h"
#include "rfx_types.h"

namespace rfx {

int fail(int code, const char *fmt, ...) __attribute__((format(printf, 2, 3)));

struct TriTree {
  std::vector<BvhNode> nodes;
  std::vector<int32_t> order;
  std::vector<int32_t> resid;
  int depth = 0;
  size_t leaves() const { return order.size() / RFX_TRI_BVH_LEAF; }
};

struct SceneBuild {
  SceneBuild(const rfx_scene &scene, int tri_accel);
  std::vector<SphereGeo> sg;
  std::vector<SpherePair> sp;
  std::vector<MatRec> sm, tm, pm;
  std::vector<int32_t> si, loc;
  std::vector<TriGeo> tg, tleaf;
  std::vector<TriShade> ts;
  std::vector<Bound> bd, cb;
  std::vector<CullRec> cs;
  std::vector<CullTri> ct;
  std::vector<BvhNode> bvh;
  std::vector<uint32_t> aux, pool;
  TriTree tt;
  std::vector<PlaneGeo> pg;
  std::vector<LightRec> lr;
  std::vector<TexRec> tr;
  DevScene d{};
  rfx_accel_info accel{};
};

}
```

### reflaxman_amd/csrc/rfx_trace.h

```cpp
#pragma once
#include <hip/hip_runtime.h>

#include <cstddef>
#include <type_traits>

#include "rfx_math.h"
#include "rfx_powf.h"
#include "rfx_launch.h"
#include "rfx_types.h"

#pragma clang fp contract(off)

namespace rfx {

struct Cnt { uint32_t c[C_COUNT]; };

#define RFX_CNT(k)                   \
  do {                               \
    if constexpr (STATS) cnt.c[k]++; \
  } while (0)

#ifdef RFX_DEBUG_PROF
enum ProfRegion { P_SPH = 0, P_TRI, P_WIN, P_LIGHT, P_SHADOW, P_MAT, P_SKY, P_SEG, P_COUNT };
static __device__ unsigned long long g_prof[2 * P_COUNT];
// ... 191 lines not shown
  const float uLeft = 1.0f / 8.0f, vLeft = 3.0f / 6.0f;
  const float uFront = 3.0f / 8.0f, vFront = 3.0f / 6.0f;
  const float uRight = 5.0f / 8.0f, vRight = 3.0f / 6.0f;
  const float uBack = 7.0f / 8.0f, vBack = 3.0f / 6.0f;
  const float uTop = 3.0f / 8.0f, vTop = 5.0f / 6.0f;
  const float uBottom = 3.0f / 8.0f, vBottom = 1.0f / 6.0f;
  const float hw = S.half_tile_w, hh = S.half_tile_h;
  const v3 n = normalized(ray);
  const float x = n.x, y = n.y, z = n.z;
  const float ax = fabsf(x) + kVerySmall, ay = fabsf(y) + kVerySmall, az = fabsf(z) + kVerySmall;
  float u0, v0, p, q, den, su, sv;
  if (az >= ax && az >= ay)
  {
    den = az;
    if (z > 0) { u0 = uFront; v0 = vFront; p = x; q = y; su = 1.0f; sv = 1.0f; }
    else { u0 = uBack; v0 = vBack; p = x; q = y; su = -1.0f; sv = 1.0f; }
  }
  else if (ax >= ay && ax >= az)
  {
    den = ax;
    if (x > 0) { u0 = uRight; v0 = vRight; p = z; q = y; su = -1.0f; sv = 1.0f; }
    else { u0 = uLeft; v0 = vLeft; p = z; q = y; su = 1.0f; sv = 1.0f; }
  }
  else
  {
    den = ay;
    if (y > 0) { u0 = uTop; v0 = vTop; p = x; q = z; su = 1.0f; sv = -1.0f; }
    else { u0 = uBottom; v0 = vBottom; p = x; q = z; su = 1.0f; sv = 1.0f; }
  }
  const float rden = rcp_refined(den);
  bool okp, okq;
  float pd = div_fast_unit(p, den, rden, okp), qd = div_fast_unit(q, den, rden, okq);
  if (__builtin_expect(!(okp && okq), 0)) { pd = p / den; qd = q / den; }
  const float pu = pd * hw, qv = qd * hh;
  const float u = su > 0.0f ? u0 + pu : u0 - pu, v = sv > 0.0f ? v0 + qv : v0 - qv;
  return texel_uv<STATS>(S, S.skybox_tex, u, v, lut, cnt);
}

template <bool STATS>
__device__ __forceinline__ col tri_texel(const DevScene &S, const TriShade &sh, float u, float v, const float *lut,
                                         Cnt &cnt)
{
  const float tvx = u * sh.t11 + v * sh.t12 + 0.0f;
  const float tvy = u * sh.t21 + v * sh.t22 + 0.0f;
  return texel_uv<STATS>(S, sh.tex, sh.tu0 + tvx, sh.tv0 + tvy, lut, cnt);
}

struct RayConst {
  v3 ray2;
  float a4, a2;
  bool a_ok;
  DivRcp a2d;
};
__device__ __forceinline__ RayConst ray_const(v3 ray)
{
  RayConst k;
  const float a = sqlen(ray);
  k.ray2 = mul(ray, 2.0f);
  k.a4 = 4.0f * a;
  k.a2 = 2.0f * a;
  k.a_ok = a > kVerySmall;
  k.a2d = div_prep(k.a2);
  return k;
}

typedef float f2 __attribute__((ext_vector_type(2)));

__device__ __forceinline__ void pair_bd(const SpherePair &g, v3 o, const RayConst &k, f2 &b, f2 &d)
{
  const f2 vx = o.x - f2{g.cx[0], g.cx[1]};
  const f2 vy = o.y - f2{g.cy[0], g.cy[1]};
  const f2 vz = o.z - f2{g.cz[0], g.cz[1]};
  b = k.ray2.x * vx + k.ray2.y * vy + k.ray2.z * vz;
  const f2 c = vx * vx + vy * vy + vz * vz - f2{g.r2[0], g.r2[1]};
  d = b * b - k.a4 * c;
}

__device__ __forceinline__ bool pair_may_hit(f2 b, f2 d)
{
  return (d.x >= 0.0f && b.x < 0.0f) || (d.y >= 0.0f && b.y < 0.0f);
}

#ifndef RFX_DIV_SEL
#define RFX_DIV_SEL 0
#endif
template <bool STATS, bool SHADOW, bool SEL = false>
__device__ __forceinline__ bool sphere_tail(float b, float d, v3 ray, const RayConst &k, float &t_out,
                                            float &sq_out, Cnt &cnt)
{
  RFX_CNT(SHADOW ? C_SH_SPH_TESTS : C_SPH_TESTS);
  if constexpr (STATS)
    if (!(b > 0.0f)) RFX_CNT(SHADOW ? C_SH_SPH_B : C_SPH_B);
  if constexpr (!STATS && SEL)
  {
    if (!(d >= 0.0f && k.a_ok && b < 0.0f)) return false;
    const float t = RFX_DIV_SEL ? div_by(-b - sqrt_rn(d), k.a2d) : (-b - sqrt_rn(d)) / k.a2;
    const float sq = sqlen(mul(ray, t));
    t_out = t;
    sq_out = sq;
    return t > kVerySmall && sq >= kSqDeltaSphere;
  }
  if (!(d >= 0.0f && k.a_ok)) return false;
  if constexpr (!STATS)
    if (!(b < 0.0f)) return false;
  if constexpr (STATS)
    if (!(b > 0.0f)) RFX_CNT(SHADOW ? C_SH_SPH_D : C_SPH_D);
  const float t = div_by(-b - sqrt_rn(d), k.a2d);
  if (!(t > kVerySmall)) return false;
  RFX_CNT(SHADOW ? C_SH_SPH_T : C_SPH_T);
  const float sq = sqlen(mul(ray, t));
  if (!(sq >= kSqDeltaSphere)) return false;
  t_out = t;
  sq_out = sq;
  return true;
}

template <bool STATS, bool SHADOW>
__device__ __forceinline__ bool tri_z(const TriGeo &g, v3 o, v3 ray, const RayConst &k, float best_sq, Cnt &cnt,
                                      float &nz_out, float &arz_out)
{
  RFX_CNT(SHADOW ? C_SH_TRI_TESTS : C_TRI_TESTS);
  const float dx = o.x - g.v0x, dy = o.y - g.v0y, dz = o.z - g.v0z;
  const float aoz = dx * g.a31 + dy * g.a32 + dz * g.a33;
  const float arz = ray.x * g.a31 + ray.y * g.a32 + ray.z * g.a33;
  if (!(fabsf(arz) > kVerySmall)) return false;
  RFX_CNT(SHADOW ? C_SH_TRI_Z : C_TRI_Z);
  const float nz = -aoz;
  const bool same_sign = (nz > 0.0f && arz > 0.0f) || (nz < 0.0f && arz < 0.0f);
  if constexpr (STATS)
    if (same_sign) RFX_CNT(SHADOW ? C_SH_TRI_S : C_TRI_S);
  if (!same_sign) return false;
  if constexpr (!STATS)
  {
    const float n2a = nz * nz * k.a2, r2 = arz * arz;
    if (n2a < (2.0f * (kDelta * kDelta)) * r2 * 0.99997f) return false;
    if constexpr (!SHADOW)
      if (n2a > best_sq * r2 * 2.0000305f) return false;
  }
  nz_out = nz; arz_out = arz;
  return true;
}
template <bool STATS, bool SHADOW>
__device__ __forceinline__ bool tri_zt(float nz, float arz, float &t_out, Cnt &cnt)
{
  const float t = qdiv(nz, arz);
  if (!(t > kVerySmall)) return false;
  RFX_CNT(SHADOW ? C_SH_TRI_T : C_TRI_T);
  t_out = t;
  return true;
}
__device__ __forceinline__ void tri_rows(const TriGeo &g, v3 o, v3 ray, f2 &ao, f2 &ar)
{
  const float dx = o.x - g.v0x, dy = o.y - g.v0y, dz = o.z - g.v0z;
  const f2 c1{g.a11, g.a21}, c2{g.a12, g.a22}, c3{g.a13, g.a23};
  ao = dx * c1 + dy * c2 + dz * c3;
  ar = ray.x * c1 + ray.y * c2 + ray.z * c3;
}
template <bool STATS, bool SHADOW>
__device__ __forceinline__ bool tri_uv(f2 ao, f2 ar, v3 ray, float t, float &u_out, float &v_out, float &sq_out, Cnt &cnt)
{
  const f2 uv = ao + t * ar;
  const float u = uv.x, v = uv.y;
  if (!(u >= 0.0f && v >= 0.0f && u + v < 1.0f)) return false;
  RFX_CNT(SHADOW ? C_SH_TRI_IN : C_TRI_IN);
  const float sq = sqlen(mul(ray, t));
  if (!(sq > kDelta * kDelta)) return false;
  u_out = u; v_out = v; sq_out = sq;
  return true;
}

template <bool STATS, bool SHADOW, bool PRE = false>
__device__ __forceinline__ bool tri_hit(const TriGeo &g, v3 o, v3 ray, float &t_out, float &u_out, float &v_out,
                                        float &sq_out, Cnt &cnt, const RayConst &k, float best_sq = INFINITY)
{
  float nz, arz;
  if (!tri_z<STATS, SHADOW>(g, o, ray, k, best_sq, cnt, nz, arz)) return false;
  f2 ao, ar;
  if constexpr (PRE && !STATS)
  {
    tri_rows(g, o, ray, ao, ar);
    const f2 pp = (nz * __builtin_amdgcn_rcpf(arz)) * ar;
    const f2 uvp = ao + pp;
    const float mu = (fabsf(ao.x) + fabsf(pp.x)) * 0x1p-17f, mv = (fabsf(ao.y) + fabsf(pp.y)) * 0x1p-17f;
    if (uvp.x < -mu || uvp.y < -mv || uvp.x + uvp.y > 1.0f + (mu + mv) + 0x1p-20f) return false;
  }
  if (!tri_zt<STATS, SHADOW>(nz, arz, t_out, cnt)) return false;
  if constexpr (!(PRE && !STATS)) tri_rows(g, o, ray, ao, ar);
  return tri_uv<STATS, SHADOW>(ao, ar, ray, t_out, u_out, v_out, sq_out, cnt);
}

#ifndef RFX_TRI_MATES
#define RFX_TRI_MATES 2
#endif
template <bool STATS, bool SHADOW>
struct TriMates {
  static constexpr bool kOn = !STATS && (RFX_TRI_MATES == 1 || RFX_TRI_MATES == (SHADOW ? 3 : 2));
  int lead = -1;
  bool ok = false;
  float t = 0.0f;
  __device__ __forceinline__ bool hit(const TriGeo &g, v3 o, v3 ray, float &t_out, float &u_out, float &v_out,
                                      float &sq_out, Cnt &cnt, const RayConst &k, float best_sq = INFINITY)
  {
    if constexpr (!kOn) return tri_hit<STATS, SHADOW>(g, o, ray, t_out, u_out, v_out, sq_out, cnt, k, best_sq);
    else
    {
      const int l = __builtin_bit_cast(int, g.pad[0]);
      if (l != lead)
      {
        lead = l;
        float nz, arz;
        ok = tri_z<STATS, SHADOW>(g, o, ray, k, best_sq, cnt, nz, arz) && tri_zt<STATS, SHADOW>(nz, arz, t, cnt);
      }
      if (!ok) return false;
      f2 ao, ar;
      tri_rows(g, o, ray, ao, ar);
      t_out = t;
      return tri_uv<STATS, SHADOW>(ao, ar, ray, t, u_out, v_out, sq_out, cnt);
    }
  }
};

template <bool STATS, bool SHADOW>
__device__ __forceinline__ bool plane_hit(const PlaneGeo &g, v3 o, v3 ray, float &t_out, float &sq_out, Cnt &cnt,
                                          const RayConst &k, float best_sq = INFINITY)
{
  RFX_CNT(SHADOW ? C_SH_PLN_TESTS : C_PLN_TESTS);
  const v3 n = mk(g.nx, g.ny, g.nz);
  const float a = dot(n, ray);
  if (!(fabsf(a) > kVerySmall)) return false;
  const float num = dot(n, sub(mk(g.px, g.py, g.pz), o));
  if (!((num > 0.0f && a > 0.0f) || (num < 0.0f && a < 0.0f))) return false;
  if constexpr (!SHADOW && !STATS)
    if (num * num * k.a2 > best_sq * (a * a) * 2.0000305f) return false;
  const float t = qdiv(num, a);
  if (!(t > kVerySmall)) return false;
  RFX_CNT(SHADOW ? C_SH_PLN_T : C_PLN_T);
  const float sq = sqlen(mul(ray, t));
  if (!(sq > kDelta * kDelta)) return false;
  t_out = t; sq_out = sq;
  return true;
}

constexpr float kCullRel = 2e-3f;

#ifndef RFX_PRIM_SSAA
#define RFX_PRIM_SSAA 0
#endif
#ifndef RFX_PRIM_LANES
#define RFX_PRIM_LANES 1
#endif
#ifndef RFX_PRIM_LARGE
#define RFX_PRIM_LARGE 0
#endif
constexpr uint64_t kPrimLargeNone = ~0ull;

struct Bundle {
  float cx, cy, cz, rw;
  float ax, ay, az, cosa, sina;
  bool ok;
};

__device__ __forceinline__ float lane_bcast(float v, int lane)
{
  return __int_as_float(__builtin_amdgcn_readlane(__float_as_int(v), lane));
// ... 709 lines not shown
        }
        if ((!STATS || 2 * j + 1 < S.n_sph) && sphere_tail<STATS, false, true>(b.y, d.y, ray, k, t, sq, cnt))
        {
          const float key = hit_key(sq);
          const int obj = S.sph_info[4 * j + 2];
          if (tri_takes(key, h.sq, obj, h.obj)) { h.sq = key; h.obj = obj; h.i = 2 * j + 1; h.t = t; }
        }
      }
    }
  }
  RFX_PROF_END(P_SPH);
#ifdef RFX_DEBUG_PROF
  RFX_CULL_STAT_LARGE(2, cull, __ballot(live), st_chunks, st_sph, st_pairs);
#endif
  RFX_PROF_BEGIN(P_TRI);
  bool use_tbvh = false;
#if RFX_TRI_BVH
  if constexpr (TBVH && !STATS)
  {
    use_tbvh = !listed && S.tri_bvh != nullptr && (S.tri_bvh_narrow || !(cull && B->cosa > kNarrowBundleCos));
    if (use_tbvh && live) closest_tris_bvh<STATS>(S, origin, ray, k, h, cnt, ns);
  }
#endif
  for (int first = 0; !use_tbvh && first < S.n_tri; first += 64)
  {
    const int n = min(64, S.n_tri - first);
    uint64_t m = listed ? pl[1] : (B && B->ok) ? cull_chunk(S.bound, S.n_sph + first, n, *B) : all_bits(n);
    while (m)
    {
      const int i = first + __builtin_ctzll(m);
      m &= m - 1ull;
      if (!live) continue;
      float t, u, v, sq;
      if (tri_hit<STATS, false>(S.tri_geo[i], origin, ray, t, u, v, sq, cnt, k, h.sq))
      {
        RFX_CNT(C_TRI_D);
        const int obj = S.tri_shade[i].obj;
        const float key = hit_key(sq);
        if (tri_takes(key, h.sq, obj, h.obj))
        {
          h.sq = key; h.obj = obj; h.kind = 1; h.i = i; h.t = t; h.u = u; h.v = v;
        }
      }
    }
  }
  if constexpr (PLANES)
    if (live) closest_planes<STATS>(S, origin, ray, k, h, cnt);
  RFX_PROF_END(P_TRI);
}

__device__ __forceinline__ uint32_t small_pairs(uint64_t om) { return (uint32_t)((om | (om >> 16)) & 0xFFFFull); }
__device__ __forceinline__ uint64_t small_tris(uint64_t om) { return om >> 32; }

template <bool STATS, bool PLANES>
__device__ __forceinline__ void closest_hit_small(const DevScene &S, v3 origin, v3 ray, uint64_t om, Hit &h, Cnt &cnt)
{
  RFX_CNT(C_SEGMENTS);
  h.obj = -1; h.kind = 0; h.i = 0; h.t = 0.0f; h.u = 0.0f; h.v = 0.0f; h.sq = kNoHitKey;
  const RayConst k = ray_const(ray);
  RFX_PROF_BEGIN(P_SPH);
  uint32_t pm = small_pairs(om);
  while (pm)
  {
    const int j = __builtin_ctz(pm);
    pm &= pm - 1u;
    f2 b, d;
    pair_bd(S.sph_pair[j], origin, k, b, d);
    if constexpr (!STATS)
      if (!pair_may_hit(b, d)) continue;
    float t, sq;
    if (sphere_tail<STATS, false>(b.x, d.x, ray, k, t, sq, cnt))
    {
      const float key = hit_key(sq);
      if (sph_takes(key, h.sq)) { h.sq = key; h.obj = 2 * j; h.t = t; }
    }
    if ((!STATS || 2 * j + 1 < S.n_sph) && sphere_tail<STATS, false>(b.y, d.y, ray, k, t, sq, cnt))
    {
      const float key = hit_key(sq);
      if (sph_takes(key, h.sq)) { h.sq = key; h.obj = 2 * j + 1; h.t = t; }
    }
  }
  if (h.obj >= 0)
  {
    h.i = h.obj;
    h.obj = Tabs<true>{S}.sph_info(2 * h.i);
  }
  RFX_PROF_END(P_SPH);
  RFX_PROF_BEGIN(P_TRI);
  uint64_t tm = small_tris(om);
  TriMates<STATS, false> zs;
  while (tm)
  {
    const int i = __builtin_ctzll(tm);
    tm &= tm - 1ull;
    float t, u, v, sq;
    if (zs.hit(S.tri_geo[i], origin, ray, t, u, v, sq, cnt, k, h.sq))
    {
      RFX_CNT(C_TRI_D);
      const int obj = S.tri_shade[i].obj;
      const float key = hit_key(sq);
      if (tri_takes(key, h.sq, obj, h.obj))
      {
        h.sq = key; h.obj = obj; h.kind = 1; h.i = i; h.t = t; h.u = u; h.v = v;
      }
    }
  }
  if constexpr (PLANES) closest_planes<STATS>(S, origin, ray, k, h, cnt);
  RFX_PROF_END(P_TRI);
}

template <bool STATS, bool PLANES>
__device__ __forceinline__ bool occluded_small(const DevScene &S, v3 o, v3 ray, int skip_sph, int skip_tri, int skip_pln,
                                               uint64_t om, Cnt &cnt)
{
  const RayConst k = ray_const(ray);
  float t, sq, u, v;
  uint32_t pm = small_pairs(om);
  while (pm)
  {
    const int j = __builtin_ctz(pm);
    pm &= pm - 1u;
    f2 b, d;
    pair_bd(S.sph_pair[j], o, k, b, d);
    if constexpr (STATS)
    {
      if (2 * j != skip_sph && sphere_tail<STATS, true>(b.x, d.x, ray, k, t, sq, cnt)) return true;
      if (2 * j + 1 != skip_sph && 2 * j + 1 < S.n_sph && sphere_tail<STATS, true>(b.y, d.y, ray, k, t, sq, cnt))
        return true;
    }
    else
    {
      if (!pair_may_hit(b, d)) continue;
      if (sphere_tail<STATS, true>(b.x, d.x, ray, k, t, sq, cnt) && 2 * j != skip_sph) return true;
      if (sphere_tail<STATS, true>(b.y, d.y, ray, k, t, sq, cnt) && 2 * j + 1 != skip_sph) return true;
    }
  }
  uint64_t tm = small_tris(om);
  TriMates<STATS, true> zs;
  while (tm)
  {
    const int i = __builtin_ctzll(tm);
    tm &= tm - 1ull;
    if constexpr (STATS)
    {
      if (i != skip_tri && tri_hit<STATS, true>(S.tri_geo[i], o, ray, t, u, v, sq, cnt, k)) return true;
    }
    else if (zs.hit(S.tri_geo[i], o, ray, t, u, v, sq, cnt, k) && i != skip_tri)
      return true;
  }
  if constexpr (PLANES) return occluded_planes<STATS>(S, o, ray, k, skip_pln, cnt);
  return false;
}

template <bool STATS, bool PLANES, bool TBVH = false, class NS = BvhGlobal>
__device__ __forceinline__ bool occluded(const DevScene &S, v3 o, v3 ray, bool live, int skip_sph, int skip_tri,
                                         int skip_pln, const Bundle *B, Cnt &cnt, const NS &ns = NS{}, int *hint = nullptr)
{
  const RayConst k = ray_const(ray);
  const bool cull = B && B->ok;
  bool occ = false;
  float t, sq, u, v;
  const bool use_bvh = !STATS && S.bvh != nullptr;
  if (use_bvh)
  {
    int found = -1;
    if (live) found = occluded_spheres_bvh<STATS>(S, o, ray, k, skip_sph, cnt, ns, hint ? *hint : -1);
    occ = found >= 0;
    if (RFX_OCC_HINT && hint)
    {
      const uint64_t fm = __ballot(found >= 0);
      if (fm) *hint = __builtin_amdgcn_readlane(found, (int)__builtin_ctzll(fm));
    }
  }
  for (int cfirst = 0; !use_bvh && cfirst < S.n_chunk; cfirst += 64)
  {
    if (__ballot(live && !occ) == 0) return occ;
    uint64_t cm = cull ? cull_chunk(S.chunk_bound, cfirst, min(64, S.n_chunk - cfirst), *B)
                       : all_bits(min(64, S.n_chunk - cfirst));
    while (cm)
    {
      const int first = 64 * (cfirst + __builtin_ctzll(cm));
      cm &= cm - 1ull;
      const int n = min(64, S.n_sph - first);
      const uint64_t m = cull ? cull_chunk(S.bound, first, n, *B) : all_bits(n);
      uint32_t pm = pair_bits(m);
      while (pm)
      {
        const int j = (first >> 1) + __builtin_ctz(pm);
        pm &= pm - 1u;
        f2 b, d;
        pair_bd(S.sph_pair[j], o, k, b, d);
// ... 62 lines not shown
  __device__ __forceinline__ BvhGlobal bvh() const { return BvhGlobal{}; }
};

__device__ __forceinline__ uint32_t queue_key(const DevScene &S, v3 o, v3 d)
{
  const auto cell = [](float v, float lo, float s) -> uint32_t {
    return (uint32_t)fminf(fmaxf((v - lo) * s, 0.0f), 7.0f);
  };
  const uint32_t cx = cell(o.x, S.key_lx, S.key_sx), cy = cell(o.y, S.key_ly, S.key_sy), cz = cell(o.z, S.key_lz, S.key_sz);
  uint32_t m = 0;
#pragma unroll
  for (int b = 0; b < 3; ++b)
    m |= (((cx >> b) & 1u) << (3 * b)) | (((cy >> b) & 1u) << (3 * b + 1)) | (((cz >> b) & 1u) << (3 * b + 2));
  const uint32_t oct = (d.x < 0.0f ? 1u : 0u) | (d.y < 0.0f ? 2u : 0u) | (d.z < 0.0f ? 4u : 0u);
  return oct << 9 | m;
}

__shared__ __attribute__((aligned(16))) uint32_t s_out[kWgWaves][256];

#ifndef RFX_NO_LAUNDER
#define RFX_LAUNDER_SCENE
#define RFX_LAUNDER_PARAMS
#endif
#ifdef RFX_LAUNDER_SCENE
typedef const __attribute__((address_space(4))) DevScene *ConstScenePtr;
template <bool ON>
__device__ __forceinline__ const DevScene &launder_scene(const DevScene &S)
{
  if constexpr (!ON) return S;
  ConstScenePtr p = (ConstScenePtr)__builtin_amdgcn_kernarg_segment_ptr();
  asm volatile("" : "+s"(p));
  return *(const DevScene *)p;
}
#define RFX_SCENE_PARAM S_in
#else
#define RFX_SCENE_PARAM S
#endif
constexpr size_t kParamsOff = (sizeof(DevScene) + alignof(FrameParams) - 1) / alignof(FrameParams) * alignof(FrameParams);
struct KernargPair { DevScene S; FrameParams P; };
static_assert(offsetof(KernargPair, S) == 0 && offsetof(KernargPair, P) == kParamsOff,
              "kernel-argument layout: DevScene at offset 0, FrameParams at kParamsOff");
template <class F>
constexpr bool kKernargSig = std::is_same<F, void (*)(DevScene, FrameParams)>::value;
template <bool LAUNDER = true>
__device__ __forceinline__ const FrameParams &kernarg_params()
{
  typedef const __attribute__((address_space(4))) char *KP;
  KP p = (KP)__builtin_amdgcn_kernarg_segment_ptr();
  if constexpr (LAUNDER) asm volatile("" : "+s"(p));
  return *(const FrameParams *)(const __attribute__((address_space(4))) FrameParams *)(p + kParamsOff);
}

template <bool STATS, bool CULL, bool MANYL, bool SMALL, bool PLANES, bool PARK, class PK, bool ONEL = false,
          bool TBVH = false>
__device__ __forceinline__ col trace_from(const DevScene &RFX_SCENE_PARAM, v3 origin, v3 ray, col mulc, col pix, int refl,
                                          int depth, v3 rd, const float *lut, Cnt &cnt, bool valid, const PK &park,
                                          bool &parked, const uint64_t *pm_tile = nullptr, bool pm_shadow = true)
{
#ifdef RFX_LAUNDER_SCENE
  const DevScene &S = S_in;
#endif
  bool seg0 = pm_tile != nullptr;
  parked = false;
  if (valid && refl == 0) RFX_CNT(C_RAYS);
  const Tabs<SMALL> T{S};
  bool alive = valid && refl < depth;
  int occ_hint = -1;
#ifdef RFX_DEBUG_SEGS
  int nseg = 0;
#endif
  RFX_PROF_BEGIN(P_SEG);
  while (__ballot(alive))
  {
#ifdef RFX_DEBUG_SEGS
    if (alive) ++nseg;
#endif
#ifdef RFX_LAUNDER_SCENE
    const DevScene &S = launder_scene<!SMALL>(S_in);
    const Tabs<SMALL> T{S};
#endif
    Hit h;
    if constexpr (SMALL)
    {
      uint64_t om = S.cull_valid;
      if constexpr (CULL)
      {
        if (seg0)
          om = pm_tile[0];
        else
        {
          const Bundle B = make_bundle(origin, ray, alive);
          if (B.ok) om = cull_small(T.cull(), S.cull_valid, B);
#ifdef RFX_HALF_BUNDLES
          else
          {
            Bundle H[2];
            make_bundle_halves(origin, ray, alive, H);
            om = (H[0].ok ? cull_small(T.cull(), S.cull_valid, H[0]) : S.cull_valid) |
                 (H[1].ok ? cull_small(T.cull(), S.cull_valid, H[1]) : S.cull_valid);
          }
#endif
          RFX_CULL_STAT(0, B.ok, __ballot(alive), om, S.cull_valid);
        }
      }
      if (alive) closest_hit_small<STATS, PLANES>(S, origin, ray, om, h, cnt);
      else h.obj = -1;
    }
    else
    {
      const uint64_t *pl = RFX_PRIM_LARGE && CULL && seg0 && pm_tile[0] != kPrimLargeNone ? pm_tile : nullptr;
      Bundle B;
      if constexpr (CULL) B = make_bundle(origin, ray, alive);
      closest_hit<STATS, PLANES, TBVH>(S, origin, ray, alive, CULL ? &B : nullptr, h, cnt, park.bvh(), pl);
    }
    const bool hit = alive && h.obj >= 0;
    v3 drop = origin, norm = mk(0.0f, 0.0f, 0.0f);
    RFX_PROF_BEGIN(P_WIN);
    if (hit)
    {
      drop = add(origin, mul(ray, h.t));
      if (h.kind == 0)
      {
        RFX_CNT(C_HIT_SPH);
        const SphereGeo g = T.sph_geo(h.i);
        norm = sub(drop, mk(g.cx, g.cy, g.cz));
      }
      else if (!PLANES || h.kind == 1)
      {
        RFX_CNT(C_HIT_TRI);
        const TriShade sh = T.tri_shade(h.i);
        norm = mk(sh.nx, sh.ny, sh.nz);
      }
      else
      {
        RFX_CNT(C_HIT_PLN);
        const PlaneGeo g = S.pln_geo[h.i];
        norm = mk(g.nx, g.ny, g.nz);
      }
    }
    RFX_PROF_END(P_WIN);
    const int skip_sph = h.kind == 0 ? h.i : -1, skip_tri = h.kind == 1 ? h.i : -1;
    const int skip_pln = PLANES && h.kind == 2 ? h.i : -1;
    MatRec m{0.0f, 0.0f, 0.0f, 0.0f};
    int diel = 0;
    v3 reflv = mk(0.0f, 0.0f, 0.0f);
    float rayLen = 0.0f, normLen = 0.0f, reflectLen = 0.0f;
    col sumL = mkc(0.0f, 0.0f, 0.0f), sumS = mkc(0.0f, 0.0f, 0.0f);
    for (int base = 0;; base += 32)
    {
      RFX_PROF_BEGIN(P_SHADOW);
      uint32_t lit = 0;
      const int nl = ONEL ? 1 : min(32, S.n_light - base);
      for (int q = 0; q < nl; ++q)
      {
        const LightRec L = S.lights[base + q];
        bool facing = false;
        v3 sray = mk(0.0f, 0.0f, 0.0f);
        if (hit)
        {
          RFX_CNT(C_L_EVAL);
          const v3 dtl = sub(mk(L.ox, L.oy, L.oz), drop);
          if (dot(dtl, norm) > kVerySmall)
          {
            RFX_CNT(C_L_FACING);
            facing = true;
            sray = add(dtl, mul(rd, L.radius));
          }
        }
        if (__ballot(facing))
        {
          if constexpr (SMALL)
          {
            uint64_t om = S.cull_valid;
            if constexpr (CULL)
            {
              if (!MANYL && seg0 && pm_shadow && q < kPrimLights)
                om = pm_tile[1 + q];
              else
              {
                const Bundle SB = make_bundle(drop, sray, facing);
                if (SB.ok) om = cull_small(T.cull(), S.cull_valid, SB);
                RFX_CULL_STAT(1, SB.ok, __ballot(facing), om, S.cull_valid);
              }
            }
            if (facing && !occluded_small<STATS, PLANES>(S, drop, sray, skip_sph, skip_tri, skip_pln, om, cnt))
              lit |= 1u << q;
          }
          else
          {
            Bundle SB;
            if constexpr (CULL) SB = make_bundle(drop, sray, facing);
            const bool occ = occluded<STATS, PLANES, TBVH>(S, drop, sray, facing, skip_sph, skip_tri, skip_pln,
                                                     CULL ? &SB : nullptr, cnt, park.bvh(), &occ_hint);
            if (facing && !occ) lit |= 1u << q;
          }
        }
      }
      RFX_PROF_END(P_SHADOW);
      RFX_PROF_BEGIN(P_LIGHT);
      if (hit)
      {
        if (!MANYL || base == 0)
        {
          if (h.kind == 0)
          {
            m = T.sph_mat(h.i);
            diel = T.sph_info(2 * h.i + 1);
          }
          else if (PLANES && h.kind == 2)
          {
            m = S.pln_mat[h.i];
            diel = S.pln_geo[h.i].dielectric;
          }
          else
          {
            const TriShade sh = T.tri_shade(h.i);
            m = T.tri_mat(h.i);
            diel = sh.dielectric;
            if (sh.tex >= 0)
            {
              const col c = tri_texel<STATS>(S, sh, h.u, h.v, lut, cnt);
              m.r = c.r; m.g = c.g; m.b = c.b;
            }
          }
          reflv = reflect(mul(ray, h.t), norm);
          rayLen = len(ray); normLen = len(norm); reflectLen = len(reflv);
        }
        for (int q = 0; q < nl; ++q)
        {
          if (!((lit >> q) & 1u)) continue;
          RFX_CNT(C_L_LIT);
          const LightRec L = S.lights[base + q];
          const v3 dtl = sub(mk(L.ox, L.oy, L.oz), drop);
          const float dlen = len(dtl);
          float aa = dlen * normLen;
          const float cosl = (aa > kVerySmall) ? qdiv(dot(dtl, norm), aa) : 0.0f;
          const col lc = mkc(L.r, L.g, L.b);
          if (L.power > kVerySmall) sumL = cadd(sumL, cscale(cscale(lc, cosl), L.power));
          aa = sqlen(dtl);
          const float ang = (aa > kVerySmall) ? 1.0f - qdiv(L.radius * L.radius, aa) : 0.0f;
          if (ang > 0)
          {
            RFX_CNT(C_L_SPEC);
            const v3 dlr = add(normalized(dtl), mul(rd, 1.0f - m.refl));
            aa = len(dlr) * reflectLen;
            float sc = (aa > kVerySmall) ? qdiv(dot(dlr, reflv), aa) : 0.0f;
            sc = clampf(sc + (1.0f - sqrt_rn(ang)), 0.0f, 1.0f);
            if (sc > kVerySmall && L.radius > kVerySmall)
            {
              RFX_CNT(C_L_POW);
              const float sp = powf_dev(sc, 1 + qdiv(3 * m.refl * dlen, L.radius)) * m.refl;
              sumS = cadd(sumS, cscale(lc, sp));
            }
          }
        }
      }
      RFX_PROF_END(P_LIGHT);
      if (!MANYL || base + 32 >= S.n_light) break;
    }
    if (hit)
    {
      RFX_PROF_BEGIN(P_MAT);
      sumL = cadd(mkc(S.amb_r, S.amb_g, S.amb_b), sumL);
      const col color = mkc(m.r, m.g, m.b);
      col fin;
      if (diel)
      {
        RFX_CNT(C_DIELECTRIC);
        const float aa = rayLen * normLen;
        const float cosA = (aa > kVerySmall) ? clampf(qdiv(dot(ray, neg(norm)), aa), 0.0f, 1.0f) : 0.0f;
        const float r = 0.2f + 0.8f * powf3_dev(1.0f - cosA);
        fin = cadd(cmul(cscale(color, 1.0f - r), sumL), sumS);
        fin = cmul(fin, mulc);
        mulc = cscale(mulc, r);
      }
      else
      {
        RFX_CNT(C_METAL);
        const float r = 0.8f;
        fin = cadd(cmul(cscale(color, 1.0f - r), sumL), sumS);
        fin = cmul(fin, mulc);
        mulc = cmul(mulc, cscale(color, r));
      }
      pix = cclamp(cadd(pix, fin));
      RFX_PROF_END(P_MAT);
      if (mulc.r < 0.01f && mulc.g < 0.01f && mulc.b < 0.01f)
        alive = false;
      else
      {
        RFX_CNT(C_CONTINUE);
        origin = drop;
        ray = add(normalized(reflv), mul(rd, 1.0f - m.refl));
        if (++refl >= depth) alive = false;
      }
    }
    else if (alive)
    {
      RFX_CNT(C_SKY);
      RFX_PROF_BEGIN(P_SKY);
      pix = cclamp(cadd(pix, cmul(cmul(mulc, skybox_texel<STATS>(S, ray, lut, cnt)), mkc(S.env_r, S.env_g, S.env_b))));
      RFX_PROF_END(P_SKY);
      alive = false;
    }
    seg0 = false;
    if constexpr (!STATS && PARK)
    {
      if (refl == park.after && __ballot(alive))
      {
        const uint64_t pm = __ballot(alive);
        uint32_t base = 0;
        if (__lane_id() == (uint32_t)(__ffsll((long long)pm) - 1)) base = atomicAdd(park.count, (uint32_t)__popcll(pm));
        base = __builtin_amdgcn_readlane(base, __ffsll((long long)pm) - 1);
        if (alive)
        {
          QRay q;
          q.ox = origin.x; q.oy = origin.y; q.oz = origin.z; q.dx = ray.x;
          q.dy = ray.y; q.dz = ray.z; q.mr = mulc.r; q.mg = mulc.g;
          q.mb = mulc.b; q.pr = pix.r; q.pg = pix.g; q.pb = pix.b;
          uint32_t qt, qo;
          park.ids(qt, qo);
          q.trace = qt; q.out = qo; q.refl = (uint32_t)refl; q.pad = 0;
          const uint32_t slot = base + (uint32_t)__popcll(pm & ((1ull << __lane_id()) - 1ull));
          park.queue[slot] = q;
          if (uint32_t *keys = park.keys()) keys[slot] = queue_key(S, origin, ray);
          parked = true;
          alive = false;
        }
      }
    }
    if constexpr (PK::kRefill) park.refill(alive, origin, ray, mulc, pix, refl, rd);
  }
  RFX_PROF_END(P_SEG);
#ifdef RFX_DEBUG_SEGS
  return mkc((float)nseg, 0.0f, 0.0f);
#else
  return pix;
#endif
}

template <bool STATS, bool CULL, bool MANYL, bool SMALL, bool PLANES, bool ONEL = false, bool TBVH = false>
__device__ __forceinline__ col trace(const DevScene &S, v3 origin, v3 ray, int depth, v3 rd, const float *lut,
                                     Cnt &cnt, bool valid, const uint64_t *pm_tile = nullptr, bool pm_shadow = true)
{
  bool parked;
  return trace_from<STATS, CULL, MANYL, SMALL, PLANES, false, Park, ONEL, TBVH>(S, origin, ray, mkc(1.0f, 1.0f, 1.0f), mkc(0.0f, 0.0f, 0.0f), 0,
                                                       depth, rd, lut, cnt, valid, Park{0, nullptr, nullptr, 0, 0},
                                                       parked, pm_tile, pm_shadow);
}

template <bool STATS>
__device__ __forceinline__ void flush_counters(const FrameParams &P, Cnt &cnt)
{
  if constexpr (STATS)
  {
#pragma unroll
    for (int k = 0; k < C_COUNT; ++k)
    {
      unsigned long long v = cnt.c[k];
#pragma unroll
      for (int off = 32; off > 0; off >>= 1) v += __shfl_xor(v, off, 64);
      if ((threadIdx.x & 63) == 0 && v) atomicAdd(&P.counters[k], v);
    }
  }
}

__device__ __forceinline__ uint32_t strip_row_to_y(uint32_t r, const FrameParams &P)
{
  if (P.nranks <= 1) return r;
  const uint32_t blk = r / P.row_block, w = r % P.row_block;
  return (blk * P.nranks + P.rank) * P.row_block + w;
}

__shared__ uint32_t s_tile8[kWgWaves];

struct ParkTile {
  int after;
  QRay *queue;
  uint32_t *count;
  const FrameParams &P;
  uint32_t wv, w8;
  __device__ __forceinline__ void ids(uint32_t &t, uint32_t &o) const
  {
    const uint32_t t8 = ((volatile uint32_t *)s_tile8)[wv];
    uint32_t le = __lane_id();
    asm volatile("" : "+v"(le));
#ifdef RFX_LAUNDER_PARAMS
    const FrameParams &P = kernarg_params();
#endif
    const uint32_t gx = (t8 % w8) * 8u + (le & 7u), gy = (t8 / w8) * 8u + (le >> 3);
    const uint32_t y = P.nranks > 1 ? strip_row_to_y(gy, P) : gy + P.row0;
    const uint32_t orow = P.nranks > 1 ? gy : y;
    t = (uint32_t)((uint64_t)y * P.W + gx - P.p_begin);
    o = (uint32_t)((size_t)orow * P.W + gx);
  }
  static constexpr bool kRefill = false;
  __device__ __forceinline__ uint32_t *keys() const { return P.queue_key; }
  __device__ __forceinline__ BvhGlobal bvh() const { return BvhGlobal{}; }
};
// ... 39 lines not shown
__device__ __forceinline__ uint32_t clock32()
{
  uint64_t c;
  asm("s_memtime %0\n\ts_waitcnt lgkmcnt(0)" : "=s"(c));
  return (uint32_t)c;
}


__device__ __forceinline__ void store_wave_tile(const FrameParams &P, uint32_t x0, uint32_t row0, col out,
                                                uint32_t lane, uint32_t wave)
{
  uint32_t *s = s_out[wave];
  s[3 * lane] = __float_as_uint(out.r);
  s[3 * lane + 1] = __float_as_uint(out.g);
  s[3 * lane + 2] = __float_as_uint(out.b);
  s[192 + lane] = argb(out);
  __builtin_amdgcn_wave_barrier();
  const bool rgb = lane < 48;
  const uint32_t k = rgb ? lane : lane - 48;
  const uint32_t r = rgb ? k / 6u : k >> 1, c = rgb ? k % 6u : k & 1u;
  const uint4 v = *reinterpret_cast<const uint4 *>(s + (rgb ? r * 24u + 4u * c : 192u + r * 8u + 4u * c));
  const size_t pix = (size_t)(row0 + r) * P.W + x0;
  uint32_t *dst = rgb ? reinterpret_cast<uint32_t *>(P.img) + pix * 3 + 4u * c : P.argb + pix + 4u * c;
  if (rgb || P.argb) *reinterpret_cast<uint4 *>(dst) = v;
}

enum TraceMode { kModeSsaa = 0, kModeBlock = 1, kModePlain = 2, kModeSsaaLanes = 3, kModeSsaaChunks = 4 };
__host__ __device__ constexpr uint32_t ss_lane_block(int ss)
{
  return ss == 1 ? 8u : ss == 2 ? 4u : ss == 4 ? 2u : ss >= 8 ? 1u : 0u;
}
#ifndef RFX_SSAA_LANES
#define RFX_SSAA_LANES 1
#endif
#ifndef RFX_ONE_LIGHT
#define RFX_ONE_LIGHT 1
#endif

#ifndef RFX_WAVES_PER_EU_LARGE
#define RFX_WAVES_PER_EU_LARGE RFX_WAVES_PER_EU
#endif
#ifndef RFX_SSAA_CHANNEL_SUM
#define RFX_SSAA_CHANNEL_SUM 1
#endif
template <bool STATS, int MODE, int CFG>
__global__ __launch_bounds__(kWgThreads) __attribute__((amdgpu_waves_per_eu(
    (CFG & kCfgSmall) ? RFX_WAVES_PER_EU : RFX_WAVES_PER_EU_LARGE))) void trace_kernel(DevScene S, FrameParams P)
{
  static_assert(kKernargSig<decltype(&trace_kernel<STATS, MODE, CFG>)>, "launder_scene / kernarg_params layout");
  constexpr bool CULL = (CFG & kCfgCull) != 0, MANYL = (CFG & kCfgManyLights) != 0, SMALL = (CFG & kCfgSmall) != 0;
  constexpr bool PLANES = (CFG & kCfgPlanes) != 0, PARK = MODE == kModePlain && !STATS && (CFG & kCfgPark) != 0;
  constexpr bool ONEL = (CFG & kCfgOneLight) != 0;
  constexpr bool TBVH = (CFG & kCfgTriBvh) != 0;
  RFX_WAVE_T0();
  __shared__ float lut[256];
  for (uint32_t i = threadIdx.x; i < 256; i += kWgThreads) lut[i] = (float)i / 255.0f;
  stage_powf_tables();
  if constexpr (SMALL) stage_small_scene(S);
  RFX_PROF_INIT();
  __shared__ uint32_t s_clk0;
  if (P.tile_cost && threadIdx.x == 0) s_clk0 = clock32();
  __syncthreads();
  Cnt cnt;
  if constexpr (STATS)
  {
#pragma unroll
    for (int k = 0; k < C_COUNT; ++k) cnt.c[k] = 0;
  }
  const uint32_t lane = threadIdx.x & 63u, wave = threadIdx.x >> 6;
  const uint32_t wv = __builtin_amdgcn_readfirstlane(wave), wid = blockIdx.y * gridDim.x + blockIdx.x;
  const uint32_t w8 = kTileWavesX * gridDim.x;
  const uint32_t t8 = P.tile_order ? P.tile_order[kWgWaves * wid + wv]
                                   : (blockIdx.y * kTileWavesY + wv / kTileWavesX) * w8 + blockIdx.x * kTileWavesX + wv % kTileWavesX;
  const uint32_t gx = (t8 % w8) * 8u + (lane & 7u), gy = (t8 / w8) * 8u + (lane >> 3);
  if (lane == 0) s_tile8[wv] = t8;
  m33 view;
  view.m11 = P.v11; view.m12 = P.v12; view.m13 = P.v13;
  view.m21 = P.v21; view.m22 = P.v22; view.m23 = P.v23;
  view.m31 = P.v31; view.m32 = P.v32; view.m33 = P.v33;
  const v3 eye = mk(P.eye_x, P.eye_y, P.eye_z);

  if constexpr (MODE == kModeSsaaLanes || MODE == kModeSsaaChunks)
  {
    constexpr bool CHUNKS = MODE == kModeSsaaChunks;
    const uint32_t ss = (uint32_t)P.ss, ss2 = ss * ss, bw = CHUNKS ? 1u : ss_lane_block(P.ss);
    const uint32_t nchunk = CHUNKS ? (ss2 + 63) / 64 : 1;
    float *sm = reinterpret_cast<float *>(s_out[wv]);
    for (uint32_t chunk = 0; chunk < nchunk; ++chunk)
    {
      uint32_t lane = threadIdx.x & 63u;
      if constexpr (CHUNKS) asm volatile("" : "+v"(lane));
#ifdef RFX_LAUNDER_PARAMS
      const FrameParams &P = kernarg_params<CHUNKS>();
#endif
      const uint32_t q = bw == 1 ? 0 : lane / ss2, kk = bw == 1 ? 64 * chunk + lane : lane - q * ss2;
      const uint32_t sx = kk / ss, sy = kk - sx * ss;
      const uint32_t lx = (t8 % w8) * bw + q % bw, ly = (t8 / w8) * bw + q / bw;
      const uint32_t x = lx;
      const uint32_t y = P.nranks > 1 ? strip_row_to_y(ly, P) : ly + P.row0;
      const uint64_t p = (uint64_t)y * P.W + x;
      const bool valid = lx < P.W && ly < P.grid_rows && p >= P.p_begin && p < P.p_end && kk < ss2;
      const uint64_t pr = p - P.p_begin;
      float rndx = 0.0f, rndy = 0.0f;
      if (P.additive && valid)
      {
        const uint32_t s1 = lcg_jump(P.jitter_seed, 2 * pr + 1);
        rndx = (float)lcg_out(s1) / (float)0x7FFF;
        rndy = (float)lcg_out(lcg_step(s1)) / (float)0x7FFF;
      }
      const float ssf = (float)(int)ss;
      const float ox = sx ? (float)(int)sx / ssf : 0.0f, oy = sy ? (float)(int)sy / ssf : 0.0f;
      const float rx = (float)x - P.wh, ry = (float)y - P.hh;
      const v3 ray = mmul(view, mk(rx + ox + rndx, ry + oy + rndy, P.rz));
      v3 rd = mk(0.0f, 0.0f, 0.0f);
      if (valid) rd = load_rd(P, pr * (uint64_t)ss2 + kk);
      const uint64_t *pm = RFX_PRIM_LANES && SMALL && CULL && !STATS && P.prim_mask
                               ? P.prim_mask + (size_t)kPrimStride * t8 : nullptr;
      const col c = trace<STATS, CULL, MANYL, SMALL, PLANES, ONEL, TBVH>(S, eye, ray, P.depth, rd, lut, cnt, valid, pm,
                                                                  P.prim_shadow != 0);
      {
#ifdef RFX_LAUNDER_PARAMS
        const FrameParams &P = kernarg_params();
#endif
        const uint32_t t8e = ((volatile uint32_t *)s_tile8)[wv];
        uint32_t le = lane;
        asm volatile("" : "+v"(le));
        const uint32_t ss = (uint32_t)P.ss, ss2 = ss * ss, bw = CHUNKS ? 1u : ss_lane_block(P.ss);
        const uint32_t q = bw == 1 ? 0 : le / ss2, kk = bw == 1 ? 64 * chunk + le : le - q * ss2;
        const uint32_t lx = (t8e % w8) * bw + q % bw, ly = (t8e / w8) * bw + q / bw;
        const uint32_t x = lx;
        const uint32_t y = P.nranks > 1 ? strip_row_to_y(ly, P) : ly + P.row0;
        const uint64_t p = (uint64_t)y * P.W + x;
        const bool pvalid = lx < P.W && ly < P.grid_rows && p >= P.p_begin && p < P.p_end;
        sm[3 * le] = c.r;
        sm[3 * le + 1] = c.g;
        sm[3 * le + 2] = c.b;
        __builtin_amdgcn_wave_barrier();
        const uint32_t first = bw == 1 ? 64 * chunk : 0;
#if RFX_SSAA_CHANNEL_SUM
        if (ss2 >= 3)
        {
          const uint32_t lead = bw == 1 ? 0u : le - kk, ch = le - lead;
          const uint32_t n = min(ss2 - first, bw == 1 ? 64u : ss2);
          const bool last = first + n >= ss2;
          if (pvalid && ch < 3)
          {
            float fc = first ? sm[192 + ch] : 0.0f;
#pragma unroll 8
            for (uint32_t j = 0; j < n; ++j) fc = fc + sm[3 * (lead + j) + ch];
            if (!last)
              sm[192 + ch] = fc;
            else
            {
              const float sq = (float)(int)ss2;
              if (fabsf(sq) > kVerySmall) fc = fc / sq;
              const size_t o = (size_t)(P.nranks > 1 ? ly : y) * P.W + x;
              float *d = P.img + o * 3;
              if (P.accumulate) fc = d[ch] + fc;
              d[ch] = fc;
              sm[3 * lead + ch] = fc;
            }
          }
          __builtin_amdgcn_wave_barrier();
          if (last && pvalid && ch == 0 && P.argb)
            P.argb[(size_t)(P.nranks > 1 ? ly : y) * P.W + x] = argb(mkc(sm[3 * lead], sm[3 * lead + 1], sm[3 * lead + 2]));
        }
        else
#endif
        if (pvalid && (bw == 1 ? le == 0 : kk == 0))
        {
          col fin = first ? mkc(sm[192], sm[193], sm[194]) : mkc(0.0f, 0.0f, 0.0f);
          const uint32_t n = min(ss2 - first, bw == 1 ? 64u : ss2);
// ... 18 lines not shown
        }
        __builtin_amdgcn_wave_barrier();
        if (chunk + 1 == nchunk)
        {
          if (P.tile_cost && __lane_id() == 0) P.tile_cost[t8e] = clock32() - s_clk0;
          RFX_WAVE_T1(t8e);
        }
      }
    }
  }
  else if constexpr (MODE == kModeBlock)
  {
    const uint32_t n = (uint32_t)(-P.ss);
    const uint32_t bw = (P.W + n - 1) / n, bh = (P.H + n - 1) / n;
    const uint32_t cx = gx, cy = gy + P.row0;
    const uint32_t x = cx * n, y = cy * n;
    const uint64_t p = (uint64_t)y * P.W + x;
    const bool valid = gy < P.grid_rows && cx < bw && cy < bh && p >= P.p_begin && p < P.p_end;
    const v3 ray = mmul(view, mk((float)x - P.wh, (float)y - P.hh, P.rz));
    v3 rd = mk(0.0f, 0.0f, 0.0f);
    if (valid) rd = load_rd(P, (uint64_t)cy * bw + cx - P.trace_base);
    const col c = trace<STATS, CULL, MANYL, SMALL, PLANES, ONEL, TBVH>(S, eye, ray, P.depth, rd, lut, cnt, valid);
    if (valid)
    {
      const uint32_t ex = min(P.W, x + n), ey = min(P.H, y + n);
      const uint32_t a = argb(c);
      for (uint32_t qy = y; qy < ey; ++qy)
        for (uint32_t qx = x; qx < ex; ++qx)
        {
          float *d = P.img + ((size_t)qy * P.W + qx) * 3;
          d[0] = c.r; d[1] = c.g; d[2] = c.b;
          if (P.argb) P.argb[(size_t)qy * P.W + qx] = a;
        }
    }
  }
  else
  {
    const uint32_t x = gx;
    const uint32_t y = P.nranks > 1 ? strip_row_to_y(gy, P) : gy + P.row0;
    const uint64_t p = (uint64_t)y * P.W + x;
    const bool valid = gx < P.W && gy < P.grid_rows && p >= P.p_begin && p < P.p_end;
    const uint64_t pr = p - P.p_begin;
    const float rx = (float)x - P.wh, ry = (float)y - P.hh;
    col out;
    bool parked = false;
    if constexpr (MODE == kModePlain)
    {
      const v3 ray = mmul(view, mk(rx + 0.0f + 0.0f, ry + 0.0f + 0.0f, P.rz));
      v3 rd = mk(0.0f, 0.0f, 0.0f);
      if (valid) rd = load_rd(P, pr);
      const ParkTile park{P.park_after, P.queue, P.queue_count, P, wv, w8};
      const uint64_t *pm_tile = (SMALL || RFX_PRIM_LARGE) && CULL && !STATS && P.prim_mask
                                    ? P.prim_mask + (size_t)(SMALL ? kPrimStride : kPrimLargeStride) * t8 : nullptr;
      const col c = trace_from<STATS, CULL, MANYL, SMALL, PLANES, PARK, ParkTile, ONEL, TBVH>(S, eye, ray, mkc(1.0f, 1.0f, 1.0f),
                                                                  mkc(0.0f, 0.0f, 0.0f), 0, P.depth, rd, lut, cnt,
                                                                  valid, park, parked, pm_tile);
      out = cadd(mkc(0.0f, 0.0f, 0.0f), c);
    }
    else
    {
#ifdef RFX_SSAA_LDS_STATE
      uint32_t *slot = s_out[wv];
      uint32_t jit = 0;
      if (P.additive && valid)
      {
        const uint32_t s1 = lcg_jump(P.jitter_seed, 2 * pr + 1);
        jit = lcg_out(s1) | lcg_out(lcg_step(s1)) << 16;
      }
      slot[192 + lane] = jit;
      slot[3 * lane] = 0u;
      slot[3 * lane + 1] = 0u;
      slot[3 * lane + 2] = 0u;
      const int ss = P.ss;
      const float ssf = (float)ss;
      for (int sx = 0; sx < ss; ++sx)
        for (int sy = 0; sy < ss; ++sy)
        {
          const FrameParams &P = kernarg_params();
          m33 view;
          view.m11 = P.v11; view.m12 = P.v12; view.m13 = P.v13;
          view.m21 = P.v21; view.m22 = P.v22; view.m23 = P.v23;
          view.m31 = P.v31; view.m32 = P.v32; view.m33 = P.v33;
          const v3 eye = mk(P.eye_x, P.eye_y, P.eye_z);
          const uint32_t t8s = ((volatile uint32_t *)s_tile8)[wv];
          uint32_t ls = lane;
          asm volatile("" : "+v"(ls));
          const uint32_t sgx = (t8s % w8) * 8u + (ls & 7u), sgy = (t8s / w8) * 8u + (ls >> 3);
          const uint32_t sy_ = P.nranks > 1 ? strip_row_to_y(sgy, P) : sgy + P.row0;
          const uint64_t sp = (uint64_t)sy_ * P.W + sgx;
          const bool svalid = sgx < P.W && sgy < P.grid_rows && sp >= P.p_begin && sp < P.p_end;
          const uint32_t jw = ((volatile uint32_t *)slot)[192 + ls];
          const float rndx = P.additive ? (float)(jw & 0xFFFFu) / (float)0x7FFF : 0.0f;
          const float rndy = P.additive ? (float)(jw >> 16) / (float)0x7FFF : 0.0f;
          const float ox = sx ? (float)sx / ssf : 0.0f, oy = sy ? (float)sy / ssf : 0.0f;
          v3 ray = mk((float)sgx - P.wh + ox + rndx, (float)sy_ - P.hh + oy + rndy, P.rz);
          ray = mmul(view, ray);
          v3 rd = mk(0.0f, 0.0f, 0.0f);
          if (svalid) rd = load_rd(P, (sp - P.p_begin) * (uint64_t)(ss * ss) + (uint64_t)(sx * ss + sy));
          const uint64_t *pm = RFX_PRIM_SSAA && SMALL && CULL && !STATS && P.prim_mask
                                   ? P.prim_mask + (size_t)kPrimStride * t8s : nullptr;
          const col c = trace<STATS, CULL, MANYL, SMALL, PLANES, false, TBVH>(S, eye, ray, P.depth, rd, lut, cnt, svalid, pm,
                                                                 P.prim_shadow != 0);
          float *f = reinterpret_cast<float *>(slot) + 3 * ls;
          f[0] = f[0] + c.r;
          f[1] = f[1] + c.g;
          f[2] = f[2] + c.b;
        }
// ... 335 lines not shown
}

template <int CFG>
__global__ __launch_bounds__(kLdsBvhThreads) __attribute__((amdgpu_waves_per_eu(4)))
void bounce_kernel_lds(DevScene S, FrameParams P)
{
  static_assert(kKernargSig<decltype(&bounce_kernel_lds<CFG>)>, "launder_scene / kernarg_params layout");
  constexpr bool CULL = (CFG & kCfgCull) != 0, MANYL = (CFG & kCfgManyLights) != 0, SMALL = (CFG & kCfgSmall) != 0;
  constexpr bool PLANES = (CFG & kCfgPlanes) != 0;
  static_assert(!SMALL, "large scenes only");
  extern __shared__ float4 s_dyn[];
  const int nn = S.n_bvh;
  float4 *box = s_dyn;
  uint2 *aux = reinterpret_cast<uint2 *>(box + 3 * nn);
  BvhSlot *stk = reinterpret_cast<BvhSlot *>(aux + nn);
  uint32_t *outs = reinterpret_cast<uint32_t *>(stk + kBvhStack * kLdsBvhThreads);
  __shared__ float lut[256];
  for (uint32_t i = threadIdx.x; i < 256; i += kLdsBvhThreads) lut[i] = (float)i / 255.0f;
  stage_powf_tables();
  const float4 *gb = reinterpret_cast<const float4 *>(S.bvh);
  const uint2 *ga = reinterpret_cast<const uint2 *>(S.bvh_aux);
  for (int i = (int)threadIdx.x; i < nn; i += kLdsBvhThreads)
  {
    box[3 * i] = gb[4 * i];
    box[3 * i + 1] = gb[4 * i + 1];
    box[3 * i + 2] = gb[4 * i + 2];
    aux[i] = ga[i];
  }
  __syncthreads();
  Cnt cnt;
  const uint32_t wv = __builtin_amdgcn_readfirstlane(threadIdx.x >> 6);
  outs[64 * wv + __lane_id()] = ~0u;
  const Refill<BvhLds> rf{P, *P.queue_count, outs + 64 * wv, BvhLds{box, aux, stk, S.bvh_mstep}, false};
  bool alive = false;
  v3 origin = mk(0.0f, 0.0f, 0.0f), ray = origin, rd = origin;
  col mulc = mkc(0.0f, 0.0f, 0.0f), pix = mulc;
  int refl = 0;
  rf.refill(alive, origin, ray, mulc, pix, refl, rd);
  bool parked;
  (void)trace_from<false, CULL, MANYL, SMALL, PLANES, false, decltype(rf), (CFG & kCfgOneLight) != 0, (CFG & kCfgTriBvh) != 0>(
      S, origin, ray, mulc, pix, refl, P.depth, rd, lut, cnt, alive, rf, parked);
}

template <bool STATS, int MODE, int CFG>
inline void launch_one(dim3 grid, const DevScene &S, const FrameParams &P, hipStream_t st)
{
  if constexpr (!STATS || !(CFG & kCfgCull))
    hipLaunchKernelGGL((trace_kernel<STATS, MODE, CFG>), grid, dim3(kWgThreads), 0, st, S, P);
}

template <bool STATS, int MODE>
inline void launch_cfg(int cfg, dim3 grid, const DevScene &S, const FrameParams &P, hipStream_t st)
{
#if RFX_TRI_BVH
  if (cfg & kCfgTriBvh)
  {
    if constexpr (!STATS)
      switch (cfg & ~kCfgTriBvh)
      {
        case 1: launch_one<STATS, MODE, 1 | kCfgTriBvh>(grid, S, P, st); return;
        case 3: launch_one<STATS, MODE, 3 | kCfgTriBvh>(grid, S, P, st); return;
        case 9: launch_one<STATS, MODE, 9 | kCfgTriBvh>(grid, S, P, st); return;
        case 11: launch_one<STATS, MODE, 11 | kCfgTriBvh>(grid, S, P, st); return;
        case 1 | kCfgOneLight: launch_one<STATS, MODE, 1 | kCfgOneLight | kCfgTriBvh>(grid, S, P, st); return;
        case 9 | kCfgOneLight: launch_one<STATS, MODE, 9 | kCfgOneLight | kCfgTriBvh>(grid, S, P, st); return;
      }
    cfg &= ~kCfgTriBvh;
  }
#endif
  if (cfg & kCfgOneLight)
  {
    switch (cfg & ~kCfgOneLight)
    {
      case 1: launch_one<STATS, MODE, 1 | kCfgOneLight>(grid, S, P, st); return;
      case 5: launch_one<STATS, MODE, 5 | kCfgOneLight>(grid, S, P, st); return;
      case 9: launch_one<STATS, MODE, 9 | kCfgOneLight>(grid, S, P, st); return;
      case 13: launch_one<STATS, MODE, 13 | kCfgOneLight>(grid, S, P, st); return;
      default: cfg &= ~kCfgOneLight;
    }
  }
  switch (cfg)
  {
    case 0: launch_one<STATS, MODE, 0>(grid, S, P, st); break;
    case 1: launch_one<STATS, MODE, 1>(grid, S, P, st); break;
    case 2: launch_one<STATS, MODE, 2>(grid, S, P, st); break;
    case 3: launch_one<STATS, MODE, 3>(grid, S, P, st); break;
    case 4: launch_one<STATS, MODE, 4>(grid, S, P, st); break;
    case 5: launch_one<STATS, MODE, 5>(grid, S, P, st); break;
    case 6: launch_one<STATS, MODE, 6>(grid, S, P, st); break;
    case 7: launch_one<STATS, MODE, 7>(grid, S, P, st); break;
    case 8: launch_one<STATS, MODE, 8>(grid, S, P, st); break;
    case 9: launch_one<STATS, MODE, 9>(grid, S, P, st); break;
    case 10: launch_one<STATS, MODE, 10>(grid, S, P, st); break;
    case 11: launch_one<STATS, MODE, 11>(grid, S, P, st); break;
    case 12: launch_one<STATS, MODE, 12>(grid, S, P, st); break;
    case 13: launch_one<STATS, MODE, 13>(grid, S, P, st); break;
    case 14: launch_one<STATS, MODE, 14>(grid, S, P, st); break;
    case 15: launch_one<STATS, MODE, 15>(grid, S, P, st); break;
  }
}

}
```

### reflaxman_amd/csrc/rfx_types.h

```cpp
#pragma once
#include <stddef.h>
#include <stdint.h>

namespace rfx {

enum Counter {
  C_RAYS = 0, C_SEGMENTS,
  C_SPH_TESTS, C_SPH_B, C_SPH_D, C_SPH_T,
  C_TRI_TESTS, C_TRI_Z, C_TRI_S, C_TRI_T, C_TRI_IN, C_TRI_D,
  C_HIT_SPH, C_HIT_TRI,
  C_SH_SPH_TESTS, C_SH_SPH_B, C_SH_SPH_D, C_SH_SPH_T,
  C_SH_TRI_TESTS, C_SH_TRI_Z, C_SH_TRI_S, C_SH_TRI_T, C_SH_TRI_IN,
  C_L_EVAL, C_L_FACING, C_L_LIT, C_L_SPEC, C_L_POW,
  C_DIELECTRIC, C_METAL, C_CONTINUE, C_SKY,
  C_TEX_BILINEAR, C_TEX_CHECKER, C_TEX_OTHER,
  C_PLN_TESTS, C_PLN_T, C_HIT_PLN, C_SH_PLN_TESTS, C_SH_PLN_T,
  C_COUNT
};

struct alignas(16) SphereGeo { float cx, cy, cz, sq_radius; };
struct alignas(32) SpherePair { float cx[2], cy[2], cz[2], r2[2]; };
struct alignas(16) MatRec { float r, g, b, refl; };
struct alignas(16) TriGeo {
  float v0x, v0y, v0z, a31, a32, a33;
// ... 67 lines not shown
  int32_t tri_bvh_depth;
  int32_t tri_bvh_narrow;
};

constexpr int kLdsBvhWaves = 16, kLdsBvhStackSlots = 16;
constexpr size_t lds_bvh_bytes(int n_bvh)
{
  return (size_t)n_bvh * 56 + sizeof(int16_t) * kLdsBvhStackSlots * 64 * kLdsBvhWaves + 4 * 64 * kLdsBvhWaves;
}
constexpr bool lds_bvh_fits(int n_bvh) { return n_bvh > 0 && lds_bvh_bytes(n_bvh) + 4096 <= 160 * 1024; }

constexpr uint32_t kQueueBuckets = 4096;
struct alignas(16) QRay {
  float ox, oy, oz, dx;
  float dy, dz, mr, mg;
  float mb, pr, pg, pb;
  uint32_t trace, out, refl, pad;
};

struct FrameParams {
  float eye_x, eye_y, eye_z;
  float v11, v12, v13, v21, v22, v23, v31, v32, v33;
  float rz, wh, hh;
  uint32_t W, H;
  int32_t depth, ss;
  int32_t accumulate;
  int32_t additive;
  uint32_t jitter_seed;
  uint32_t row_block, rank, nranks;
  uint32_t grid_rows;
  uint32_t row0;
  uint64_t p_begin, p_end;
  uint64_t trace_base;
  float *img;
  uint32_t *argb;
  const uint32_t *rd_state;
  unsigned long long *counters;
  const uint32_t *tile_order;
  uint32_t *tile_cost;
  uint32_t tiles_x;
  QRay *queue;
  uint32_t *queue_count, *queue_next;
  int32_t park_after;
  uint32_t *queue_key;
  const uint32_t *queue_order;
  const uint64_t *prim_mask;
  int32_t prim_shadow;
};

constexpr int kPrimLights = 4, kPrimStride = 1 + kPrimLights;
constexpr int kPrimLargeChunks = 8, kPrimLargeStride = 4 + kPrimLargeChunks;
constexpr int kCfgCull = 1, kCfgManyLights = 2, kCfgSmall = 4, kCfgPlanes = 8, kCfgPark = 16, kCfgOneLight = 32;
constexpr int kCfgTriBvh = 64;

}
```

### reflaxman_amd/render.py

```python
from __future__ import annotations

import ctypes as C
import os
from typing import List, Optional, Sequence

import numpy as np

from . import _lib
from ._lib import DIELECTRIC, METAL, check, farr

DEFAULT_SPHERE_SEED = 1350490027
DEFAULT_JITTER_SEED = 424238335


class Vector3:
    __slots__ = ("x", "y", "z")

    def __init__(self, x=0.0, y=0.0, z=0.0):
        self.x, self.y, self.z = float(x), float(y), float(z)

    def __iter__(self):
        return iter((self.x, self.y, self.z))

    def __repr__(self):
# ... 90 lines not shown
        if h and _lib._lib is not None:
            _lib._lib.rfx_scene_destroy(h)
            self._h = None

    def addSphere(self, center: Vector3, radius: float, material: Material) -> Sphere:
        obj = check(_lib.load().rfx_scene_add_sphere(self._h, farr(Vector3(*center)), float(radius), material.type,
                                                     farr(material.color), material.reflectivity, material.transparency),
                    "Scene.addSphere")
        self._version += 1
        return Sphere(self, obj)

    def addTriangle(self, v1: Vector3, v2: Vector3, v3: Vector3, material: Material) -> Triangle:
        obj = check(_lib.load().rfx_scene_add_triangle(self._h, farr(Vector3(*v1)), farr(Vector3(*v2)), farr(Vector3(*v3)),
                                                       material.type, farr(material.color), material.reflectivity,
                                                       material.transparency), "Scene.addTriangle")
        self._version += 1
        return Triangle(self, obj)

    def addMesh(self, vertices, indices, material: Material) -> List[Triangle]:
        v = np.ascontiguousarray(vertices, dtype=np.float32).reshape(-1, 3)
        i = np.ascontiguousarray(indices, dtype=np.uint32).reshape(-1, 3)
        first = check(_lib.load().rfx_scene_add_mesh(self._h, _lib.fptr(v), v.shape[0], _lib.u32ptr(i), i.shape[0],
                                                     material.type, farr(material.color), material.reflectivity,
                                                     material.transparency), "Scene.addMesh")
        self._version += 1
        return [Triangle(self, first + k) for k in range(i.shape[0])]

    def tri_bvh_dump(self):
        L = _lib.load()
        cnt = (C.c_int32 * 5)()
        if check(L.rfx_scene_tri_bvh_dump(self._h, cnt, None, None, None, None), "Scene.tri_bvh_dump") == 0:
            return None
        nodes, leaves, nres, leaf, depth = (int(x) for x in cnt)
        boxes = np.zeros((nodes, 2, 6), np.float32)
        children = np.zeros((nodes, 2), np.int32)
        ids = np.zeros((leaves, leaf), np.int32)
        res = np.zeros(nres, np.int32)
        i32 = lambda a: a.ctypes.data_as(_lib._i32p)
        check(L.rfx_scene_tri_bvh_dump(self._h, cnt, _lib.fptr(boxes), i32(children), i32(ids), i32(res)),
              "Scene.tri_bvh_dump")
        return {"nodes": nodes, "leaves": leaves, "leaf_size": leaf, "depth": depth, "boxes": boxes,
                "children": children, "leaf_ids": ids, "residual": res}

    def set_tri_mates(self, on: bool):
        check(_lib.load().rfx_scene_set_tri_mates(self._h, int(bool(on))), "Scene.set_tri_mates")
        self._version += 1

    def tri_mates(self, plane: bool = False):
        L = _lib.load()
        n = check(L.rfx_scene_tri_mates(self._h, None, None), "Scene.tri_mates")
        leader, rows = np.zeros(n, np.int32), np.zeros((n, 6), np.float32)
        check(L.rfx_scene_tri_mates(self._h, leader.ctypes.data_as(_lib._i32p), _lib.fptr(rows)), "Scene.tri_mates")
        return (leader, rows) if plane else leader

    def addPlane(self, pos: Vector3, norm: Vector3, material: Material) -> Plane:
        obj = check(_lib.load().rfx_scene_add_plane(self._h, farr(Vector3(*pos)), farr(Vector3(*norm)), material.type,
                                                    farr(material.color), material.reflectivity, material.transparency),
                    "Scene.addPlane")
        self._version += 1
        return Plane(self, obj)

    def addLight(self, origin: Vector3, radius: float, color: Color, power: float) -> OmniLight:
        idx = check(_lib.load().rfx_scene_add_light(self._h, farr(Vector3(*origin)), float(radius), farr(Color(*color)),
                                                    float(power)), "Scene.addLight")
        self._version += 1
        return OmniLight(self, idx)

    def addTexture(self, fileName: str) -> Texture:
        loaded = C.c_int(0)
        idx = check(_lib.load().rfx_scene_add_texture_file(self._h, os.fsencode(fileName), C.byref(loaded)),
                    "Scene.addTexture")
        self._version += 1
        return Texture(self, idx, bool(loaded.value))

    def addTextureArgb(self, argb: Optional[np.ndarray]) -> Texture:
        L = _lib.load()
        if argb is None:
            idx = check(L.rfx_scene_add_texture_argb(self._h, 0, 0, None), "Scene.addTextureArgb")
        else:
            a = np.ascontiguousarray(argb, dtype=np.uint32)
            idx = check(L.rfx_scene_add_texture_argb(self._h, a.shape[1], a.shape[0], _lib.u32ptr(a)), "Scene.addTextureArgb")
        self._version += 1
        return Texture(self, idx, argb is not None)

    def setSkyboxTexture(self, fileName: str) -> bool:
        ok = check(_lib.load().rfx_scene_set_skybox_file(self._h, os.fsencode(fileName)), "Scene.setSkyboxTexture")
        self._version += 1
        return bool(ok)

    def setSkyboxTextureArgb(self, argb: Optional[np.ndarray]) -> bool:
        L = _lib.load()
        if argb is None:
            ok = check(L.rfx_scene_set_skybox_argb(self._h, 0, 0, None), "Scene.setSkyboxTextureArgb")
        else:
            a = np.ascontiguousarray(argb, dtype=np.uint32)
            ok = check(L.rfx_scene_set_skybox_argb(self._h, a.shape[1], a.shape[0], _lib.u32ptr(a)), "Scene.setSkyboxTextureArgb")
        self._version += 1
        return bool(ok)

    def counts(self):
        v = [C.c_int() for _ in range(4)]
        check(_lib.load().rfx_scene_counts(self._h, *[C.byref(x) for x in v]), "Scene.counts")
        return tuple(x.value for x in v)


def build_scene(desc, texture_dir: Optional[str] = None) -> tuple:
# ... 36 lines not shown

class Renderer:

    def __init__(self, device: int = 0, sphere_seed: int = DEFAULT_SPHERE_SEED, jitter_seed: int = DEFAULT_JITTER_SEED):
        L = _lib.load()
        h = C.c_void_p()
        check(L.rfx_renderer_create(C.byref(h), int(device)), "rfx_renderer_create")
        self._h = h
        self.device = device
        self._scene_key = None
        self.set_rng(sphere_seed, jitter_seed)

    def close(self):
        if getattr(self, "_h", None) and _lib._lib is not None:
            _lib._lib.rfx_renderer_destroy(self._h)
            self._h = None

    __del__ = close

    def set_scene(self, scene: Scene):
        key = (id(scene), scene._version)
        if key != self._scene_key:
            check(_lib.load().rfx_renderer_set_scene(self._h, scene._h), "rfx_renderer_set_scene")
            self._scene_key = key
            self._scene_ref = scene

    def set_rng(self, sphere_seed: int, jitter_seed: int):
        check(_lib.load().rfx_renderer_set_rng(self._h, sphere_seed & 0xFFFFFFFF, jitter_seed & 0xFFFFFFFF), "set_rng")

    def get_rng(self):
        s, j = C.c_uint32(), C.c_uint32()
        check(_lib.load().rfx_renderer_get_rng(self._h, C.byref(s), C.byref(j)), "get_rng")
        return s.value, j.value

    def set_stream(self, stream_ptr: int):
        check(_lib.load().rfx_renderer_set_stream(self._h, C.c_void_p(stream_ptr)), "set_stream")

    def render_frame(self, frame: _lib.Frame, d_rgb: int, d_argb: int = 0, d_counters: int = 0, stream: int = 0):
        check(_lib.load().rfx_render_frame(self._h, C.byref(frame), C.c_void_p(d_rgb), C.c_void_p(d_argb or None),
                                           C.c_void_p(d_counters or None), C.c_void_p(stream or None)), "rfx_render_frame")

    def synchronize(self):
        check(_lib.load().rfx_synchronize(self._h), "rfx_synchronize")

    def set_tile_order(self, mode: int):
        check(_lib.load().rfx_renderer_set_tile_order(self._h, int(mode)), "set_tile_order")

    def set_prim_masks(self, mode: int):
        check(_lib.load().rfx_renderer_set_prim_masks(self._h, int(mode)), "set_prim_masks")

    def set_prim_exact(self, on: bool):
        check(_lib.load().rfx_renderer_set_prim_exact(self._h, int(bool(on))), "set_prim_exact")

    def prim_masks(self) -> np.ndarray:
        L = _lib.load()
        n = C.c_uint64()
        check(L.rfx_renderer_get_prim_masks(self._h, None, 0, C.byref(n)), "get_prim_masks")
        out = np.zeros(n.value, np.uint64)
        if n.value:
            check(L.rfx_renderer_get_prim_masks(self._h, _lib.u64ptr(out), n.value, C.byref(n)), "get_prim_masks")
        return out

    def set_regroup(self, park_after: int):
        check(_lib.load().rfx_renderer_set_regroup(self._h, int(park_after)), "set_regroup")

    def set_regroup_sort(self, on: bool):
        check(_lib.load().rfx_renderer_set_regroup_sort(self._h, int(bool(on))), "set_regroup_sort")

    def set_launch_traces(self, max_traces: int):
        check(_lib.load().rfx_renderer_set_launch_traces(self._h, int(max_traces)), "set_launch_traces")

    def bounce_form(self) -> int:
        return _lib.load().rfx_renderer_bounce_form(self._h)

    def set_rng_prepass(self, mode: int):
        check(_lib.load().rfx_renderer_set_rng_prepass(self._h, int(mode)), "set_rng_prepass")

    def prepass_form(self) -> int:
        return _lib.load().rfx_renderer_prepass_form(self._h)

    def kat_rng_seq_prefix(self) -> np.ndarray:
        out = np.zeros(_lib.load().rfx_rng_seq_blocks() + 1, np.uint32)
        check(_lib.load().rfx_kat_rng_seq_prefix(self._h, _lib.u32ptr(out)), "rfx_kat_rng_seq_prefix")
        return out

    def kat_rng_seq_legacy(self) -> np.ndarray:
        out = np.zeros(_lib.load().rfx_rng_seq_blocks(), np.uint32)
        check(_lib.load().rfx_kat_rng_seq_legacy(self._h, _lib.u32ptr(out)), "rfx_kat_rng_seq_legacy")
        return out

    def set_tri_accel(self, mode: int):
        check(_lib.load().rfx_renderer_set_tri_accel(self._h, int(mode)), "set_tri_accel")
        self._scene_key = None

    def accel_info(self) -> "_lib.AccelInfo":
        a = _lib.AccelInfo()
        check(_lib.load().rfx_renderer_accel_info(self._h, C.byref(a)), "accel_info")
        return a

    def set_timing(self, enable):
        check(_lib.load().rfx_renderer_set_timing(self._h, int(enable)), "set_timing")

    def get_timing(self):
        a, b, n = C.c_double(), C.c_double(), C.c_uint64()
        check(_lib.load().rfx_renderer_get_timing(self._h, C.byref(a), C.byref(b), C.byref(n)), "get_timing")
        return a.value, b.value, n.value
# ... 203 lines not shown
```

Before: 13700 Mrays/s.

## Add bounded-range fast division variant gated by scene/frame magnitude bounds

Computes host-side bounds on scene and frame magnitudes (coordinates, radii, lights, eye, ray lengths). When those bounds show that denominators and quotients stay in a safe range, it launches a specialised trace kernel (kCfgBounded) that replaces the correctly-rounded qdiv in intersection, reflection and shading with a cheaper reciprocal plus Newton-refinement division. The aim is to cut the cost of the IEEE-exact division sequence in the hot path. It adds more kernel instantiations and a validation test kernel, and it relies on the bounds proof to keep results bit-identical or within tolerance.

After: 13770 Mrays/s (median of 6 runs). No clear change (+0.5%).

```diff
diff --git a/include/rfx.h b/include/rfx.h
--- a/include/rfx.h
+++ b/include/rfx.h
@@ -82,6 +82,24 @@
 int rfx_renderer_accel_info(const rfx_renderer *r, rfx_accel_info *out);
 int rfx_renderer_set_prim_masks(rfx_renderer *r, int mode);
 int rfx_renderer_set_prim_exact(rfx_renderer *r, int on);
+typedef struct {
+  float coord_max;
+  float ax_max;
+  float radius_min, radius_max;
+  float refl_min;
+  float light_radius_max;
+  float light_near_min;
+  float light_far_max;
+  float eye_max;
+  float ray_min, ray_max;
+  int32_t planes;
+  int32_t lights_ok;
+  int32_t finite;
+  int32_t scene_ok, frame_ok;
+} rfx_div_bounds;
+int rfx_renderer_set_div_bounded(rfx_renderer *r, int on);
+int rfx_renderer_div_bounded(const rfx_renderer *r, rfx_div_bounds *out);
+int rfx_scene_div_bounds(const rfx_scene *scene, rfx_div_bounds *out);
 int rfx_renderer_get_prim_masks(rfx_renderer *r, uint64_t *host, uint64_t capacity, uint64_t *words);
 int rfx_renderer_set_rng(rfx_renderer *r, uint32_t sphere_seed, uint32_t jitter_seed);
 int rfx_renderer_get_rng(rfx_renderer *r, uint32_t *sphere_seed, uint32_t *jitter_seed);
@@ -102,6 +120,8 @@
   uint64_t span_begin;
   uint64_t span_end;
 } rfx_frame;
+
+int rfx_frame_div_bounds(const rfx_div_bounds *scene, const rfx_frame *frame, rfx_div_bounds *out);
 
 uint32_t rfx_strip_rows(uint32_t height, uint32_t row_block, uint32_t rank, uint32_t nranks);
 uint32_t rfx_strip_row_to_y(uint32_t r, uint32_t row_block, uint32_t rank, uint32_t nranks);
@@ -164,6 +184,7 @@
 int rfx_kat_argb(rfx_renderer *r, const float *rgb, uint64_t n, uint32_t *out);
 int rfx_kat_powf_cube(rfx_renderer *r, uint64_t counts[2]);
 int rfx_kat_div(rfx_renderer *r, uint64_t first, uint64_t n, uint64_t counts[3]);
+int rfx_kat_div_bounded(rfx_renderer *r, int site, uint64_t first, uint64_t n, uint64_t counts[3]);
 int rfx_kat_kernarg(rfx_renderer *r, int swapped, uint32_t out[3]);
 int rfx_kat_rng_seq_prefix(rfx_renderer *r, uint32_t *prefix);
 int rfx_kat_rng_seq_legacy(rfx_renderer *r, uint32_t *counts);
diff --git a/reflaxman_amd/_lib.py b/reflaxman_amd/_lib.py
--- a/reflaxman_amd/_lib.py
+++ b/reflaxman_amd/_lib.py
@@ -34,6 +34,13 @@
 class AccelInfo(C.Structure):
     _fields_ = [(n, C.c_int32) for n in ("tri_nodes", "tri_depth", "tri_leaf_size", "tri_in_leaves", "tri_residual",
                                          "sph_nodes", "sph_depth", "narrow_tri_bvh")]
+
+
+class DivBounds(C.Structure):
+    _fields_ = [(n, C.c_float) for n in ("coord_max", "ax_max", "radius_min", "radius_max", "refl_min",
+                                         "light_radius_max", "light_near_min", "light_far_max", "eye_max", "ray_min",
+                                         "ray_max")] + \
+               [(n, C.c_int32) for n in ("planes", "lights_ok", "finite", "scene_ok", "frame_ok")]
 
 
 _i32p = C.POINTER(C.c_int32)
@@ -101,6 +108,10 @@
     ("rfx_renderer_set_prim_masks", C.c_int, [C.c_void_p, C.c_int]),
     ("rfx_renderer_set_prim_exact", C.c_int, [C.c_void_p, C.c_int]),
     ("rfx_renderer_get_prim_masks", C.c_int, [C.c_void_p, _u64p, C.c_uint64, _u64p]),
+    ("rfx_renderer_set_div_bounded", C.c_int, [C.c_void_p, C.c_int]),
+    ("rfx_renderer_div_bounded", C.c_int, [C.c_void_p, C.POINTER(DivBounds)]),
+    ("rfx_scene_div_bounds", C.c_int, [C.c_void_p, C.POINTER(DivBounds)]),
+    ("rfx_frame_div_bounds", C.c_int, [C.POINTER(DivBounds), C.POINTER(Frame), C.POINTER(DivBounds)]),
     ("rfx_renderer_set_regroup", C.c_int, [C.c_void_p, C.c_int]),
     ("rfx_renderer_set_regroup_sort", C.c_int, [C.c_void_p, C.c_int]),
     ("rfx_renderer_set_launch_traces", C.c_int, [C.c_void_p, C.c_uint64]),
@@ -125,6 +136,7 @@
     ("rfx_kat_argb", C.c_int, [C.c_void_p, _fp, C.c_uint64, _u32p]),
     ("rfx_kat_powf_cube", C.c_int, [C.c_void_p, C.POINTER(C.c_uint64)]),
     ("rfx_kat_div", C.c_int, [C.c_void_p, C.c_uint64, C.c_uint64, C.POINTER(C.c_uint64)]),
+    ("rfx_kat_div_bounded", C.c_int, [C.c_void_p, C.c_int, C.c_uint64, C.c_uint64, C.POINTER(C.c_uint64)]),
     ("rfx_kat_kernarg", C.c_int, [C.c_void_p, C.c_int, C.POINTER(C.c_uint32)]),
     ("rfx_kat_rng_seq_prefix", C.c_int, [C.c_void_p, _u32p]),
     ("rfx_kat_rng_seq_legacy", C.c_int, [C.c_void_p, _u32p]),
diff --git a/reflaxman_amd/csrc/rfx_host.cpp b/reflaxman_amd/csrc/rfx_host.cpp
--- a/reflaxman_amd/csrc/rfx_host.cpp
+++ b/reflaxman_amd/csrc/rfx_host.cpp
@@ -229,6 +229,20 @@
   r->prim_exact = on;
   r->prim_key.clear();
   return RFX_OK;
+}
+
+extern "C" int rfx_renderer_set_div_bounded(rfx_renderer *r, int on)
+{
+  if (!r || on < 0 || on > 1) return fail(RFX_ERR_ARG, "renderer_set_div_bounded: 0 or 1");
+  r->div_bounded = on;
+  return RFX_OK;
+}
+
+extern "C" int rfx_renderer_div_bounded(const rfx_renderer *r, rfx_div_bounds *out)
+{
+  if (!r) return fail(RFX_ERR_ARG, "renderer_div_bounded: null renderer");
+  if (out) *out = r->div;
+  return r->div_ran ? 1 : 0;
 }
 
 extern "C" int rfx_renderer_get_prim_masks(rfx_renderer *r, uint64_t *host, uint64_t capacity, uint64_t *words)
@@ -334,6 +348,8 @@
       (rc = upload(r, B.tt.resid, &d.tri_resid)) || (rc = upload(r, B.aux, &d.bvh_aux)))
     return rc;
   r->accel = B.accel;
+  r->div_scene = r->div = B.div;
+  r->div_ran = false;
   r->dev = d;
   r->has_scene = true;
   ++r->scene_gen;
@@ -515,6 +531,7 @@
   P.p_begin = p0;
   P.p_end = p1;
   P.trace_base = trace_base;
+  (void)rfx_frame_div_bounds(&r->div_scene, f, &r->div);
   return RFX_OK;
 }
 
@@ -760,7 +777,12 @@
 {
   const FrameParams &P = pl.P;
   const hipStream_t st = pl.st;
-  if (P.grid_rows) HIP_CHECK(launch_trace(r->dev, P, stats, st));
+  const bool bounded = r->div_bounded && r->div.frame_ok;
+  if (P.grid_rows)
+  {
+    HIP_CHECK(launch_trace(r->dev, P, stats, bounded, st));
+    r->div_ran = bounded && trace_has_bounded(r->dev, P, stats);
+  }
   r->bounce_form = 0;
   if (!park) return RFX_OK;
   const uint64_t waves = (pl.traces + 63) / 64;
diff --git a/reflaxman_amd/csrc/rfx_internal.h b/reflaxman_amd/csrc/rfx_internal.h
--- a/reflaxman_amd/csrc/rfx_internal.h
+++ b/reflaxman_amd/csrc/rfx_internal.h
@@ -144,6 +144,9 @@
   uint64_t scene_gen = 0;
   int prim_mode = 1;
   int prim_exact = 1;
+  int div_bounded = 1;
+  rfx_div_bounds div_scene{}, div{};
+  bool div_ran = false;
   size_t prim_words = 0;
   hipStream_t prim_on = nullptr;
   int tri_accel = -1;
diff --git a/reflaxman_amd/csrc/rfx_kat.cpp b/reflaxman_amd/csrc/rfx_kat.cpp
--- a/reflaxman_amd/csrc/rfx_kat.cpp
+++ b/reflaxman_amd/csrc/rfx_kat.cpp
@@ -102,6 +102,24 @@
   return RFX_OK;
 }
 
+extern "C" int rfx_kat_div_bounded(rfx_renderer *r, int site, uint64_t first, uint64_t n, uint64_t counts[3])
+{
+  if (!r || !counts || site < 0 || site > 1) return fail(RFX_ERR_ARG, "kat_div_bounded: bad args");
+  RCHECK(set_dev(r));
+  DevBuf<unsigned long long> d;
+  int rc;
+  if ((rc = d.reserve(3)) < 0) return named("kat_div_bounded", rc);
+  hipError_t e = hipMemsetAsync(d, 0, 3 * sizeof(unsigned long long), r->stream);
+  for (uint64_t k = 0; e == hipSuccess && k < n; k += 1ull << 28)
+    e = launch_kat_div_bounded(site, first + k, (uint32_t)std::min<uint64_t>(1ull << 28, n - k), d, r->stream);
+  unsigned long long h[3] = {0, 0, 0};
+  if (e == hipSuccess) e = hipStreamSynchronize(r->stream);
+  if (e == hipSuccess) e = hipMemcpy(h, d, sizeof(h), hipMemcpyDeviceToHost);
+  if (e != hipSuccess) return fail(RFX_ERR_HIP, "kat_div_bounded: %s", hipGetErrorString(e));
+  for (int i = 0; i < 3; ++i) counts[i] = h[i];
+  return RFX_OK;
+}
+
 extern "C" uint32_t rfx_rng_seq_blocks(void) { return rng_seq_blocks(); }
 
 extern "C" int rfx_kat_rng_seq_prefix(rfx_renderer *r, uint32_t *prefix)
diff --git a/reflaxman_amd/csrc/rfx_kernels.hip b/reflaxman_amd/csrc/rfx_kernels.hip
--- a/reflaxman_amd/csrc/rfx_kernels.hip
+++ b/reflaxman_amd/csrc/rfx_kernels.hip
@@ -1045,6 +1045,80 @@
   }
 }
 
+__global__ __launch_bounds__(kKatThreads) void kat_div_bounded(int site, uint64_t first, uint32_t n,
+                                                               unsigned long long *counts)
+{
+  const uint32_t i = blockIdx.x * kKatThreads + threadIdx.x;
+  uint32_t bad = 0, low = 0, seen = 0;
+  if (i < n)
+  {
+    const uint64_t k = first + i;
+    const uint32_t h0 = kat_mix(k), h1 = kat_mix(k ^ 0x9E3779B97F4A7C15ull), h2 = kat_mix(k * 3 + 1);
+    float a, b, x = 0.0f;
+    bool pre = true;
+    if (site == 0)
+    {
+      const uint32_t sg = h0 >> 31;
+      b = (h0 & 3u) == 0 ? __uint_as_float(__float_as_uint(0x1p-60f) + 1u + (h1 & 3u))
+                         : kat_float(0, (int32_t)(h1 % 144u) - 60, h2 | 1u);
+      a = (h0 & 12u) == 0 ? ((h2 & 1u) ? 0x1p-75f : __uint_as_float(__float_as_uint(0x1p36f) - 1u - (h2 >> 30)))
+                          : kat_float(0, (int32_t)(h2 % 111u) - 75, h1 >> 3);
+      if (sg) { a = -a; b = -b; }
+    }
+    else
+    {
+      x = kat_float(h0 >> 31, (int32_t)(h1 % 93u) - 31, h2);
+      const float aa = x * x;
+      b = 2.0f * aa;
+      pre = aa > kVerySmall;
+      switch ((h0 >> 3) % 5u)
+      {
+        case 0: a = (h2 & 1u) ? -0.0f : 0.0f; break;
+        case 1: a = __uint_as_float(h2 & 0x807FFFFFu); break;
+        case 2: a = kat_float(h2 >> 31, -126 + (int32_t)(h1 % 30u), h2 >> 3); break;
+        case 3: a = b * kat_float(h2 >> 31, (int32_t)(h1 % 188u) - 130, h0 >> 5); break;
+        default: a = kat_float(h2 >> 31, (int32_t)(h1 % 187u) - 126, h0 >> 4); break;
+      }
+      const int ea = (int)((__float_as_uint(a) >> 23) & 0xFFu), eb = (int)((__float_as_uint(b) >> 23) & 0xFFu);
+      pre = pre && a == a && fabsf(a) < INFINITY && ea - eb <= 57;
+    }
+    if (pre)
+    {
+      const float ref = a / b;
+      const float q = site == 0 ? div_bounded(a, b) : div_by_bounded(a, div_prep_bounded(b));
+      const bool cond = a == 0.0f || ((__float_as_uint(a) >> 23) & 0xFFu) <= 23u || !(fabsf(ref) >= 0x1p-125f);
+      bool dr, dq;
+      if (site == 0)
+      {
+        dr = ref > kVerySmall;
+        dq = q > kVerySmall;
+        if (!kat_same(div_bounded(ref, 1.0f), ref)) ++bad;
+      }
+      else
+      {
+        dr = ref > kVerySmall && sqlen(mul(mk(x, 0.0f, 0.0f), ref)) >= kSqDeltaSphere;
+        dq = q > kVerySmall && sqlen(mul(mk(x, 0.0f, 0.0f), q)) >= kSqDeltaSphere;
+      }
+      if (dr != dq || (!cond && !kat_same(q, ref))) ++bad;
+      low = cond ? 1u : 0u;
+      seen = 1;
+    }
+  }
+#pragma unroll
+  for (int o = 32; o > 0; o >>= 1)
+  {
+    bad += __shfl_xor(bad, o, 64);
+    low += __shfl_xor(low, o, 64);
+    seen += __shfl_xor(seen, o, 64);
+  }
+  if ((threadIdx.x & 63u) == 0 && seen)
+  {
+    if (bad) atomicAdd(&counts[0], (unsigned long long)bad);
+    atomicAdd(&counts[1], (unsigned long long)low);
+    atomicAdd(&counts[2], (unsigned long long)seen);
+  }
+}
+
 template <bool SWAPPED>
 __device__ __forceinline__ void kernarg_compare(const DevScene &S, const FrameParams &P, uint32_t *out)
 {
@@ -1269,6 +1343,13 @@
   return hipGetLastError();
 }
 
+hipError_t launch_kat_div_bounded(int site, uint64_t first, uint32_t n, unsigned long long *counts, hipStream_t st)
+{
+  if (!n) return hipSuccess;
+  hipLaunchKernelGGL(kat_div_bounded, kat_grid(n), dim3(kKatThreads), 0, st, site, first, n, counts);
+  return hipGetLastError();
+}
+
 hipError_t launch_kat_powf_cube(uint32_t first, uint32_t n, unsigned long long *counts, hipStream_t st)
 {
   if (!n) return hipSuccess;
@@ -1336,20 +1417,31 @@
   return hipGetLastError();
 }
 
-hipError_t launch_trace(const DevScene &S, const FrameParams &P, bool stats, hipStream_t st)
+static int trace_cfg(const DevScene &S, const FrameParams &P, bool stats)
+{
+  const bool cull = !stats && !(RFX_NOCULL_MAX_TILES > 0 && S.n_sph <= 32 && S.n_tri <= 32 &&
+                                trace_tiles(P) <= (uint32_t)RFX_NOCULL_MAX_TILES);
+  return (S.n_light > 32 ? kCfgManyLights : 0) | (cull ? kCfgCull : 0) |
+         (S.n_sph <= 32 && S.n_tri <= 32 ? kCfgSmall : 0) | (S.n_pln > 0 ? kCfgPlanes : 0) |
+         (S.n_light == 1 && !stats && RFX_ONE_LIGHT ? kCfgOneLight : 0) |
+         (RFX_TRI_BVH && S.tri_bvh != nullptr && !stats ? kCfgTriBvh : 0);
+}
+
+bool trace_has_bounded(const DevScene &S, const FrameParams &P, bool stats)
+{
+  const int mode = trace_mode(P);
+  return !stats && (mode == kModeSsaaLanes || (mode == kModePlain && P.park_after <= 0)) &&
+         (trace_cfg(S, P, stats) & ~kCfgOneLight) == (kCfgCull | kCfgSmall);
+}
+
+hipError_t launch_trace(const DevScene &S, const FrameParams &P, bool stats, bool bounded, hipStream_t st)
 {
   const dim3 grid = trace_grid(P);
   FrameParams Pt = P;
   Pt.tiles_x = kTileWavesX * grid.x;
-  const int mode = trace_mode(P);
-  const bool cull = !stats && !(RFX_NOCULL_MAX_TILES > 0 && S.n_sph <= 32 && S.n_tri <= 32 &&
-                                trace_tiles(P) <= (uint32_t)RFX_NOCULL_MAX_TILES);
-  const int cfg = (S.n_light > 32 ? kCfgManyLights : 0) | (cull ? kCfgCull : 0) |
-                  (S.n_sph <= 32 && S.n_tri <= 32 ? kCfgSmall : 0) | (S.n_pln > 0 ? kCfgPlanes : 0) |
-                  (S.n_light == 1 && !stats && RFX_ONE_LIGHT ? kCfgOneLight : 0) |
-                  (RFX_TRI_BVH && S.tri_bvh != nullptr && !stats ? kCfgTriBvh : 0);
-  launch_mode_cfg(stats, mode, cfg, grid, S, Pt, st);
-  return hipGetLastError();
-}
-
-}
+  const int cfg = trace_cfg(S, P, stats) | (bounded && trace_has_bounded(S, P, stats) ? kCfgBounded : 0);
+  launch_mode_cfg(stats, trace_mode(P), cfg, grid, S, Pt, st);
+  return hipGetLastError();
+}
+
+}
diff --git a/reflaxman_amd/csrc/rfx_launch.h b/reflaxman_amd/csrc/rfx_launch.h
--- a/reflaxman_amd/csrc/rfx_launch.h
+++ b/reflaxman_amd/csrc/rfx_launch.h
@@ -30,7 +30,8 @@
 hipError_t launch_rng_emit_seq(const uint32_t *d_pos, const uint32_t *d_hdr, const uint32_t *d_state, const uint32_t *d_p,
                                uint64_t nblk, uint64_t traces, uint32_t *d_rd_state, uint32_t *d_next_seed,
                                uint32_t *d_next_pos, int *d_err, hipStream_t st);
-hipError_t launch_trace(const DevScene &S, const FrameParams &P, bool stats, hipStream_t st);
+hipError_t launch_trace(const DevScene &S, const FrameParams &P, bool stats, bool bounded, hipStream_t st);
+bool trace_has_bounded(const DevScene &S, const FrameParams &P, bool stats);
 hipError_t launch_prim_cull(const DevScene &S, const FrameParams &P, uint64_t *masks, bool narrow, hipStream_t st);
 hipError_t launch_queue_sort(const uint32_t *count, const uint32_t *key, uint32_t *hist, uint32_t *order, hipStream_t st);
 uint32_t trace_tiles(const FrameParams &P);
@@ -42,6 +43,7 @@
                       hipStream_t st);
 hipError_t launch_kat_powf_cube(uint32_t first, uint32_t n, unsigned long long *counts, hipStream_t st);
 hipError_t launch_kat_div(uint64_t first, uint32_t n, unsigned long long *counts, hipStream_t st);
+hipError_t launch_kat_div_bounded(int site, uint64_t first, uint32_t n, unsigned long long *counts, hipStream_t st);
 hipError_t launch_kat_kernarg(const DevScene &S, const FrameParams &P, int swapped, uint32_t *out, hipStream_t st);
 #define RFX_DECLARE_TRACE_FAMILY(name) \
   void name(int cfg, dim3 grid, const DevScene &S, const FrameParams &P, hipStream_t st)
diff --git a/reflaxman_amd/csrc/rfx_math.h b/reflaxman_amd/csrc/rfx_math.h
--- a/reflaxman_amd/csrc/rfx_math.h
+++ b/reflaxman_amd/csrc/rfx_math.h
@@ -75,6 +75,39 @@
   return q;
 }
 RFX_HD float div_rn(float a, float b) { return div_by(a, div_prep(b)); }
+RFX_HD DivRcp div_prep_bounded(float b)
+{
+  DivRcp d;
+  d.b = b;
+#if defined(__HIP_DEVICE_COMPILE__) && RFX_DIV_FAST
+  const float r = __builtin_amdgcn_rcpf(b);
+  d.r = __builtin_fmaf(__builtin_fmaf(-b, r, 1.0f), r, r);
+#else
+  d.r = 0.0f;
+#endif
+  return d;
+}
+RFX_HD float div_by_bounded(float a, const DivRcp &d)
+{
+#if defined(__HIP_DEVICE_COMPILE__) && RFX_DIV_FAST
+  const float q0 = a * d.r;
+  const float t1 = __builtin_fmaf(-d.b, q0, a);
+  const float q1 = __builtin_fmaf(t1, d.r, q0);
+  const float t2 = __builtin_fmaf(-d.b, q1, a);
+  return __builtin_fmaf(t2, d.r, q1);
+#else
+  return a / d.b;
+#endif
+}
+RFX_HD float div_bounded(float a, float b) { return div_by_bounded(a, div_prep_bounded(b)); }
+RFX_HD float div_bounded_lo(float a, float b)
+{
+#if defined(__HIP_DEVICE_COMPILE__) && RFX_DIV_FAST
+  const float q = div_bounded(a, b);
+  if (__builtin_expect(fabsf(q) >= 0x1p-30f, 1)) return q;
+#endif
+  return a / b;
+}
 #ifndef RFX_DIV_SINGLE
 #define RFX_DIV_SINGLE 0
 #endif
@@ -147,10 +180,11 @@
   }
   return a;
 }
+template <bool BND = false>
 RFX_HD v3 reflect(v3 v, v3 n)
 {
   const float dn = dot(n, n);
-  if (dn > kVerySmall) return sub(v, mul(mul(n, 2.0f), qdiv(dot(v, n), dn)));
+  if (dn > kVerySmall) return sub(v, mul(mul(n, 2.0f), BND ? div_bounded_lo(dot(v, n), dn) : qdiv(dot(v, n), dn)));
   return v;
 }
 RFX_HD float clampf(float v, float lo, float hi) { return v < lo ? lo : v > hi ? hi : v; }
diff --git a/reflaxman_amd/csrc/rfx_scene.cpp b/reflaxman_amd/csrc/rfx_scene.cpp
--- a/reflaxman_amd/csrc/rfx_scene.cpp
+++ b/reflaxman_amd/csrc/rfx_scene.cpp
@@ -681,7 +681,117 @@
   return (int)l.size();
 }
 
-SceneBuild::SceneBuild(const rfx_scene &scene, int tri_accel)
+static rfx_div_bounds scene_div_bounds(const rfx_scene &s)
+{
+  rfx_div_bounds b{};
+  bool finite = true;
+  double lo[3] = {INFINITY, INFINITY, INFINITY}, hi[3] = {-INFINITY, -INFINITY, -INFINITY};
+  auto point = [&](const v3 &p, float r) {
+    const float c[3] = {p.x, p.y, p.z};
+    for (int k = 0; k < 3; ++k)
+    {
+      finite = finite && std::isfinite(c[k]) && std::isfinite(r);
+      lo[k] = fmin(lo[k], (double)c[k] - r);
+      hi[k] = fmax(hi[k], (double)c[k] + r);
+      b.coord_max = fmaxf(b.coord_max, fabsf(c[k]) + r);
+    }
+  };
+  b.refl_min = 1.0f;
+  b.radius_min = s.spheres.empty() ? 0.0f : INFINITY;
+  for (const HostSphere &h : s.spheres)
+  {
+    point(h.center, h.radius);
+    b.radius_min = fminf(b.radius_min, h.radius);
+    b.radius_max = fmaxf(b.radius_max, h.radius);
+    finite = finite && std::isfinite(h.mat.refl);
+    b.refl_min = fminf(b.refl_min, h.mat.refl);
+  }
+  for (const HostTri &t : s.tris)
+  {
+    for (const v3 &p : {t.v0, t.v1, t.v2}) point(p, 0.0f);
+    for (float a : {t.ax.m11, t.ax.m12, t.ax.m13, t.ax.m21, t.ax.m22, t.ax.m23, t.ax.m31, t.ax.m32, t.ax.m33})
+    {
+      finite = finite && std::isfinite(a);
+      b.ax_max = fmaxf(b.ax_max, fabsf(a));
+    }
+    finite = finite && std::isfinite(t.mat.refl) && std::isfinite(t.norm.x) && std::isfinite(t.norm.y) &&
+             std::isfinite(t.norm.z);
+    b.refl_min = fminf(b.refl_min, t.mat.refl);
+  }
+  b.lights_ok = 1;
+  b.light_near_min = s.lights.empty() ? 0.0f : INFINITY;
+  const bool empty = s.spheres.empty() && s.tris.empty();
+  for (const HostLight &l : s.lights)
+  {
+    const float o[3] = {l.origin.x, l.origin.y, l.origin.z};
+    double near2 = 0.0, far2 = 0.0;
+    for (int k = 0; k < 3; ++k)
+    {
+      finite = finite && std::isfinite(o[k]);
+      if (empty) continue;
+      const double out = fmax(fmax(lo[k] - o[k], (double)o[k] - hi[k]), 0.0);
+      const double far = fmax(fabs(o[k] - lo[k]), fabs(o[k] - hi[k]));
+      near2 += out * out;
+      far2 += far * far;
+    }
+    finite = finite && std::isfinite(l.radius);
+    b.light_radius_max = fmaxf(b.light_radius_max, fabsf(l.radius));
+    b.light_near_min = fminf(b.light_near_min, (float)sqrt(near2));
+    b.light_far_max = fmaxf(b.light_far_max, (float)(sqrt(far2) * (1.0 + 1e-6)) + fabsf(l.radius));
+    const double r = fabs((double)l.radius), nr = sqrt(near2);
+    if (!((r <= (double)kVerySmall || r >= 0x1p-20) && (r <= 0x1p15 || (nr >= 4.0 * b.coord_max && nr >= r * 0x1p-30))))
+      b.lights_ok = 0;
+  }
+  b.planes = !s.planes.empty();
+  finite = finite && std::isfinite(b.coord_max) && std::isfinite(b.ax_max) && std::isfinite(b.light_far_max);
+  b.finite = finite;
+  b.scene_ok = finite && !b.planes && b.lights_ok && b.coord_max <= 0x1p20f && b.ax_max <= 0x1p40f && b.light_far_max <= 0x1p40f;
+  return b;
+}
+
+extern "C" int rfx_scene_div_bounds(const rfx_scene *s, rfx_div_bounds *out)
+{
+  if (!s) return fail(RFX_ERR_ARG, "scene_div_bounds: null scene");
+  const rfx_div_bounds b = scene_div_bounds(*s);
+  if (out) *out = b;
+  return b.scene_ok;
+}
+
+extern "C" int rfx_frame_div_bounds(const rfx_div_bounds *scene, const rfx_frame *f, rfx_div_bounds *out)
+{
+  if (!scene || !f || !out) return fail(RFX_ERR_ARG, "frame_div_bounds: bad args");
+  rfx_div_bounds b = *scene;
+  bool finite = scene->finite != 0;
+  double fro2 = 0.0;
+  for (float v : f->view)
+  {
+    finite = finite && std::isfinite(v);
+    fro2 += (double)v * v;
+  }
+  for (float e : f->eye)
+  {
+    finite = finite && std::isfinite(e);
+    b.eye_max = fmaxf(b.eye_max, fabsf(e));
+  }
+  const double rz = rfx_camera_rz(f->width, f->fov), xm = f->width / 2.0 + 2.0, ym = f->height / 2.0 + 2.0;
+  b.ray_max = (float)(sqrt(fro2) * sqrt(xm * xm + ym * ym + rz * rz) * (1.0 + 1e-6));
+  const float *v = f->view;
+  double dev = 0.0;
+  for (int i = 0; i < 3; ++i)
+    for (int j = 0; j < 3; ++j)
+      dev = fmax(dev, fabs((double)v[i] * v[j] + (double)v[3 + i] * v[3 + j] + (double)v[6 + i] * v[6 + j] - (i == j)));
+  b.ray_min = dev <= 1e-3 ? (float)(fabs(rz) * 0.998) : 0.0f;
+  finite = finite && std::isfinite(b.ray_max) && std::isfinite(b.ray_min) && std::isfinite(b.eye_max);
+  b.finite = finite;
+  const float m = 3.0f * fmaxf(b.coord_max, b.eye_max);
+  const float ray_all = fmaxf(fmaxf(b.ray_max, 2.01f), 1.01f * b.light_far_max + 2.0f * m);
+  b.frame_ok = scene->scene_ok && finite && b.eye_max <= 0x1p20f && b.ray_max <= 0x1p20f &&
+               b.ax_max * m <= 0x1p13f && ray_all * m <= 0x1p50f;
+  *out = b;
+  return b.frame_ok;
+}
+
+SceneBuild::SceneBuild(const rfx_scene &scene, int tri_accel) : div(scene_div_bounds(scene))
 {
   const rfx_scene *s = &scene;
   const size_t nsph = s->spheres.size();
diff --git a/reflaxman_amd/csrc/rfx_scene.h b/reflaxman_amd/csrc/rfx_scene.h
--- a/reflaxman_amd/csrc/rfx_scene.h
+++ b/reflaxman_amd/csrc/rfx_scene.h
@@ -37,6 +37,7 @@
   std::vector<TexRec> tr;
   DevScene d{};
   rfx_accel_info accel{};
+  rfx_div_bounds div;
 };
 
 }
diff --git a/reflaxman_amd/csrc/rfx_trace.h b/reflaxman_amd/csrc/rfx_trace.h
--- a/reflaxman_amd/csrc/rfx_trace.h
+++ b/reflaxman_amd/csrc/rfx_trace.h
@@ -267,6 +267,7 @@
   bool a_ok;
   DivRcp a2d;
 };
+template <bool BND = false>
 __device__ __forceinline__ RayConst ray_const(v3 ray)
 {
   RayConst k;
@@ -275,7 +276,7 @@
   k.a4 = 4.0f * a;
   k.a2 = 2.0f * a;
   k.a_ok = a > kVerySmall;
-  k.a2d = div_prep(k.a2);
+  k.a2d = BND ? div_prep_bounded(k.a2) : div_prep(k.a2);
   return k;
 }
 
@@ -299,7 +300,7 @@
 #ifndef RFX_DIV_SEL
 #define RFX_DIV_SEL 0
 #endif
-template <bool STATS, bool SHADOW, bool SEL = false>
+template <bool STATS, bool SHADOW, bool SEL = false, bool BND = false>
 __device__ __forceinline__ bool sphere_tail(float b, float d, v3 ray, const RayConst &k, float &t_out,
                                             float &sq_out, Cnt &cnt)
 {
@@ -320,7 +321,7 @@
     if (!(b < 0.0f)) return false;
   if constexpr (STATS)
     if (!(b > 0.0f)) RFX_CNT(SHADOW ? C_SH_SPH_D : C_SPH_D);
-  const float t = div_by(-b - sqrt_rn(d), k.a2d);
+  const float t = BND ? div_by_bounded(-b - sqrt_rn(d), k.a2d) : div_by(-b - sqrt_rn(d), k.a2d);
   if (!(t > kVerySmall)) return false;
   RFX_CNT(SHADOW ? C_SH_SPH_T : C_SPH_T);
   const float sq = sqlen(mul(ray, t));
@@ -330,7 +331,7 @@
   return true;
 }
 
-template <bool STATS, bool SHADOW>
+template <bool STATS, bool SHADOW, bool BND = false>
 __device__ __forceinline__ bool tri_z(const TriGeo &g, v3 o, v3 ray, const RayConst &k, float best_sq, Cnt &cnt,
                                       float &nz_out, float &arz_out)
 {
@@ -338,7 +339,18 @@
   const float dx = o.x - g.v0x, dy = o.y - g.v0y, dz = o.z - g.v0z;
   const float aoz = dx * g.a31 + dy * g.a32 + dz * g.a33;
   const float arz = ray.x * g.a31 + ray.y * g.a32 + ray.z * g.a33;
-  if (!(fabsf(arz) > kVerySmall)) return false;
+  if constexpr (BND)
+  {
+    static_assert(!STATS, "the bounded forms are the fast kernels'");
+    if (__builtin_expect(!(fabsf(arz) > 0x1p-60f), 0))
+    {
+      float nz, az;
+      if (!tri_z<STATS, SHADOW, false>(g, o, ray, k, best_sq, cnt, nz, az)) return false;
+      nz_out = nz / az; arz_out = 1.0f;
+      return true;
+    }
+  }
+  else if (!(fabsf(arz) > kVerySmall)) return false;
   RFX_CNT(SHADOW ? C_SH_TRI_Z : C_TRI_Z);
   const float nz = -aoz;
   const bool same_sign = (nz > 0.0f && arz > 0.0f) || (nz < 0.0f && arz < 0.0f);
@@ -355,10 +367,10 @@
   nz_out = nz; arz_out = arz;
   return true;
 }
-template <bool STATS, bool SHADOW>
+template <bool STATS, bool SHADOW, bool BND = false>
 __device__ __forceinline__ bool tri_zt(float nz, float arz, float &t_out, Cnt &cnt)
 {
-  const float t = qdiv(nz, arz);
+  const float t = BND ? div_bounded(nz, arz) : qdiv(nz, arz);
   if (!(t > kVerySmall)) return false;
   RFX_CNT(SHADOW ? C_SH_TRI_T : C_TRI_T);
   t_out = t;
@@ -384,12 +396,13 @@
   return true;
 }
 
-template <bool STATS, bool SHADOW, bool PRE = false>
+template <bool STATS, bool SHADOW, bool PRE = false, bool BND = false>
 __device__ __forceinline__ bool tri_hit(const TriGeo &g, v3 o, v3 ray, float &t_out, float &u_out, float &v_out,
                                         float &sq_out, Cnt &cnt, const RayConst &k, float best_sq = INFINITY)
 {
+  static_assert(!(PRE && BND), "the bounded z stage may hand on (t, 1) for (nz, arz)");
   float nz, arz;
-  if (!tri_z<STATS, SHADOW>(g, o, ray, k, best_sq, cnt, nz, arz)) return false;
+  if (!tri_z<STATS, SHADOW, BND>(g, o, ray, k, best_sq, cnt, nz, arz)) return false;
   f2 ao, ar;
   if constexpr (PRE && !STATS)
   {
@@ -399,7 +412,7 @@
     const float mu = (fabsf(ao.x) + fabsf(pp.x)) * 0x1p-17f, mv = (fabsf(ao.y) + fabsf(pp.y)) * 0x1p-17f;
     if (uvp.x < -mu || uvp.y < -mv || uvp.x + uvp.y > 1.0f + (mu + mv) + 0x1p-20f) return false;
   }
-  if (!tri_zt<STATS, SHADOW>(nz, arz, t_out, cnt)) return false;
+  if (!tri_zt<STATS, SHADOW, BND>(nz, arz, t_out, cnt)) return false;
   if constexpr (!(PRE && !STATS)) tri_rows(g, o, ray, ao, ar);
   return tri_uv<STATS, SHADOW>(ao, ar, ray, t_out, u_out, v_out, sq_out, cnt);
 }
@@ -407,7 +420,7 @@
 #ifndef RFX_TRI_MATES
 #define RFX_TRI_MATES 2
 #endif
-template <bool STATS, bool SHADOW>
+template <bool STATS, bool SHADOW, bool BND = false>
 struct TriMates {
   static constexpr bool kOn = !STATS && (RFX_TRI_MATES == 1 || RFX_TRI_MATES == (SHADOW ? 3 : 2));
   int lead = -1;
@@ -416,7 +429,7 @@
   __device__ __forceinline__ bool hit(const TriGeo &g, v3 o, v3 ray, float &t_out, float &u_out, float &v_out,
                                       float &sq_out, Cnt &cnt, const RayConst &k, float best_sq = INFINITY)
   {
-    if constexpr (!kOn) return tri_hit<STATS, SHADOW>(g, o, ray, t_out, u_out, v_out, sq_out, cnt, k, best_sq);
+    if constexpr (!kOn) return tri_hit<STATS, SHADOW, false, BND>(g, o, ray, t_out, u_out, v_out, sq_out, cnt, k, best_sq);
     else
     {
       const int l = __builtin_bit_cast(int, g.pad[0]);
@@ -424,7 +437,7 @@
       {
         lead = l;
         float nz, arz;
-        ok = tri_z<STATS, SHADOW>(g, o, ray, k, best_sq, cnt, nz, arz) && tri_zt<STATS, SHADOW>(nz, arz, t, cnt);
+        ok = tri_z<STATS, SHADOW, BND>(g, o, ray, k, best_sq, cnt, nz, arz) && tri_zt<STATS, SHADOW, BND>(nz, arz, t, cnt);
       }
       if (!ok) return false;
       f2 ao, ar;
@@ -1240,12 +1253,12 @@
 __device__ __forceinline__ uint32_t small_pairs(uint64_t om) { return (uint32_t)((om | (om >> 16)) & 0xFFFFull); }
 __device__ __forceinline__ uint64_t small_tris(uint64_t om) { return om >> 32; }
 
-template <bool STATS, bool PLANES>
+template <bool STATS, bool PLANES, bool BND = false>
 __device__ __forceinline__ void closest_hit_small(const DevScene &S, v3 origin, v3 ray, uint64_t om, Hit &h, Cnt &cnt)
 {
   RFX_CNT(C_SEGMENTS);
   h.obj = -1; h.kind = 0; h.i = 0; h.t = 0.0f; h.u = 0.0f; h.v = 0.0f; h.sq = kNoHitKey;
-  const RayConst k = ray_const(ray);
+  const RayConst k = ray_const<BND>(ray);
   RFX_PROF_BEGIN(P_SPH);
   uint32_t pm = small_pairs(om);
   while (pm)
@@ -1257,12 +1270,12 @@
     if constexpr (!STATS)
       if (!pair_may_hit(b, d)) continue;
     float t, sq;
-    if (sphere_tail<STATS, false>(b.x, d.x, ray, k, t, sq, cnt))
+    if (sphere_tail<STATS, false, false, BND>(b.x, d.x, ray, k, t, sq, cnt))
     {
       const float key = hit_key(sq);
       if (sph_takes(key, h.sq)) { h.sq = key; h.obj = 2 * j; h.t = t; }
     }
-    if ((!STATS || 2 * j + 1 < S.n_sph) && sphere_tail<STATS, false>(b.y, d.y, ray, k, t, sq, cnt))
+    if ((!STATS || 2 * j + 1 < S.n_sph) && sphere_tail<STATS, false, false, BND>(b.y, d.y, ray, k, t, sq, cnt))
     {
       const float key = hit_key(sq);
       if (sph_takes(key, h.sq)) { h.sq = key; h.obj = 2 * j + 1; h.t = t; }
@@ -1276,7 +1289,7 @@
   RFX_PROF_END(P_SPH);
   RFX_PROF_BEGIN(P_TRI);
   uint64_t tm = small_tris(om);
-  TriMates<STATS, false> zs;
+  TriMates<STATS, false, BND> zs;
   while (tm)
   {
     const int i = __builtin_ctzll(tm);
@@ -1297,11 +1310,11 @@
   RFX_PROF_END(P_TRI);
 }
 
-template <bool STATS, bool PLANES>
+template <bool STATS, bool PLANES, bool BND = false>
 __device__ __forceinline__ bool occluded_small(const DevScene &S, v3 o, v3 ray, int skip_sph, int skip_tri, int skip_pln,
                                                uint64_t om, Cnt &cnt)
 {
-  const RayConst k = ray_const(ray);
+  const RayConst k = ray_const<BND>(ray);
   float t, sq, u, v;
   uint32_t pm = small_pairs(om);
   while (pm)
@@ -1312,19 +1325,19 @@
     pair_bd(S.sph_pair[j], o, k, b, d);
     if constexpr (STATS)
     {
-      if (2 * j != skip_sph && sphere_tail<STATS, true>(b.x, d.x, ray, k, t, sq, cnt)) return true;
-      if (2 * j + 1 != skip_sph && 2 * j + 1 < S.n_sph && sphere_tail<STATS, true>(b.y, d.y, ray, k, t, sq, cnt))
+      if (2 * j != skip_sph && sphere_tail<STATS, true, false, BND>(b.x, d.x, ray, k, t, sq, cnt)) return true;
+      if (2 * j + 1 != skip_sph && 2 * j + 1 < S.n_sph && sphere_tail<STATS, true, false, BND>(b.y, d.y, ray, k, t, sq, cnt))
         return true;
     }
     else
     {
       if (!pair_may_hit(b, d)) continue;
-      if (sphere_tail<STATS, true>(b.x, d.x, ray, k, t, sq, cnt) && 2 * j != skip_sph) return true;
-      if (sphere_tail<STATS, true>(b.y, d.y, ray, k, t, sq, cnt) && 2 * j + 1 != skip_sph) return true;
+      if (sphere_tail<STATS, true, false, BND>(b.x, d.x, ray, k, t, sq, cnt) && 2 * j != skip_sph) return true;
+      if (sphere_tail<STATS, true, false, BND>(b.y, d.y, ray, k, t, sq, cnt) && 2 * j + 1 != skip_sph) return true;
     }
   }
   uint64_t tm = small_tris(om);
-  TriMates<STATS, true> zs;
+  TriMates<STATS, true, BND> zs;
   while (tm)
   {
     const int i = __builtin_ctzll(tm);
@@ -1493,7 +1506,7 @@
 }
 
 template <bool STATS, bool CULL, bool MANYL, bool SMALL, bool PLANES, bool PARK, class PK, bool ONEL = false,
-          bool TBVH = false>
+          bool TBVH = false, bool BND = false>
 __device__ __forceinline__ col trace_from(const DevScene &RFX_SCENE_PARAM, v3 origin, v3 ray, col mulc, col pix, int refl,
                                           int depth, v3 rd, const float *lut, Cnt &cnt, bool valid, const PK &park,
                                           bool &parked, const uint64_t *pm_tile = nullptr, bool pm_shadow = true)
@@ -1501,6 +1514,7 @@
 #ifdef RFX_LAUNDER_SCENE
   const DevScene &S = S_in;
 #endif
+  const auto sdiv = [](float a, float b) { return BND ? div_bounded_lo(a, b) : qdiv(a, b); };
   bool seg0 = pm_tile != nullptr;
   parked = false;
   if (valid && refl == 0) RFX_CNT(C_RAYS);
@@ -1544,7 +1558,7 @@
           RFX_CULL_STAT(0, B.ok, __ballot(alive), om, S.cull_valid);
         }
       }
-      if (alive) closest_hit_small<STATS, PLANES>(S, origin, ray, om, h, cnt);
+      if (alive) closest_hit_small<STATS, PLANES, BND>(S, origin, ray, om, h, cnt);
       else h.obj = -1;
     }
     else
@@ -1624,7 +1638,7 @@
                 RFX_CULL_STAT(1, SB.ok, __ballot(facing), om, S.cull_valid);
               }
             }
-            if (facing && !occluded_small<STATS, PLANES>(S, drop, sray, skip_sph, skip_tri, skip_pln, om, cnt))
+            if (facing && !occluded_small<STATS, PLANES, BND>(S, drop, sray, skip_sph, skip_tri, skip_pln, om, cnt))
               lit |= 1u << q;
           }
           else
@@ -1664,7 +1678,7 @@
               m.r = c.r; m.g = c.g; m.b = c.b;
             }
           }
-          reflv = reflect(mul(ray, h.t), norm);
+          reflv = reflect<BND>(mul(ray, h.t), norm);
           rayLen = len(ray); normLen = len(norm); reflectLen = len(reflv);
         }
         for (int q = 0; q < nl; ++q)
@@ -1675,22 +1689,22 @@
           const v3 dtl = sub(mk(L.ox, L.oy, L.oz), drop);
           const float dlen = len(dtl);
           float aa = dlen * normLen;
-          const float cosl = (aa > kVerySmall) ? qdiv(dot(dtl, norm), aa) : 0.0f;
+          const float cosl = (aa > kVerySmall) ? sdiv(dot(dtl, norm), aa) : 0.0f;
           const col lc = mkc(L.r, L.g, L.b);
           if (L.power > kVerySmall) sumL = cadd(sumL, cscale(cscale(lc, cosl), L.power));
           aa = sqlen(dtl);
-          const float ang = (aa > kVerySmall) ? 1.0f - qdiv(L.radius * L.radius, aa) : 0.0f;
+          const float ang = (aa > kVerySmall) ? 1.0f - sdiv(L.radius * L.radius, aa) : 0.0f;
           if (ang > 0)
           {
             RFX_CNT(C_L_SPEC);
             const v3 dlr = add(normalized(dtl), mul(rd, 1.0f - m.refl));
             aa = len(dlr) * reflectLen;
-            float sc = (aa > kVerySmall) ? qdiv(dot(dlr, reflv), aa) : 0.0f;
+            float sc = (aa > kVerySmall) ? sdiv(dot(dlr, reflv), aa) : 0.0f;
             sc = clampf(sc + (1.0f - sqrt_rn(ang)), 0.0f, 1.0f);
             if (sc > kVerySmall && L.radius > kVerySmall)
             {
               RFX_CNT(C_L_POW);
-              const float sp = powf_dev(sc, 1 + qdiv(3 * m.refl * dlen, L.radius)) * m.refl;
+              const float sp = powf_dev(sc, 1 + sdiv(3 * m.refl * dlen, L.radius)) * m.refl;
               sumS = cadd(sumS, cscale(lc, sp));
             }
           }
@@ -1709,7 +1723,7 @@
       {
         RFX_CNT(C_DIELECTRIC);
         const float aa = rayLen * normLen;
-        const float cosA = (aa > kVerySmall) ? clampf(qdiv(dot(ray, neg(norm)), aa), 0.0f, 1.0f) : 0.0f;
+        const float cosA = (aa > kVerySmall) ? clampf(sdiv(dot(ray, neg(norm)), aa), 0.0f, 1.0f) : 0.0f;
         const float r = 0.2f + 0.8f * powf3_dev(1.0f - cosA);
         fin = cadd(cmul(cscale(color, 1.0f - r), sumL), sumS);
         fin = cmul(fin, mulc);
@@ -1779,12 +1793,12 @@
 #endif
 }
 
-template <bool STATS, bool CULL, bool MANYL, bool SMALL, bool PLANES, bool ONEL = false, bool TBVH = false>
+template <bool STATS, bool CULL, bool MANYL, bool SMALL, bool PLANES, bool ONEL = false, bool TBVH = false, bool BND = false>
 __device__ __forceinline__ col trace(const DevScene &S, v3 origin, v3 ray, int depth, v3 rd, const float *lut,
                                      Cnt &cnt, bool valid, const uint64_t *pm_tile = nullptr, bool pm_shadow = true)
 {
   bool parked;
-  return trace_from<STATS, CULL, MANYL, SMALL, PLANES, false, Park, ONEL, TBVH>(S, origin, ray, mkc(1.0f, 1.0f, 1.0f), mkc(0.0f, 0.0f, 0.0f), 0,
+  return trace_from<STATS, CULL, MANYL, SMALL, PLANES, false, Park, ONEL, TBVH, BND>(S, origin, ray, mkc(1.0f, 1.0f, 1.0f), mkc(0.0f, 0.0f, 0.0f), 0,
                                                        depth, rd, lut, cnt, valid, Park{0, nullptr, nullptr, 0, 0},
                                                        parked, pm_tile, pm_shadow);
 }
@@ -1930,6 +1944,8 @@
   constexpr bool PLANES = (CFG & kCfgPlanes) != 0, PARK = MODE == kModePlain && !STATS && (CFG & kCfgPark) != 0;
   constexpr bool ONEL = (CFG & kCfgOneLight) != 0;
   constexpr bool TBVH = (CFG & kCfgTriBvh) != 0;
+  constexpr bool BND = (CFG & kCfgBounded) != 0;
+  static_assert(!BND || (!STATS && CULL && SMALL && !PLANES && !PARK), "kCfgBounded: launch_cfg's cases only");
   RFX_WAVE_T0();
   __shared__ float lut[256];
   for (uint32_t i = threadIdx.x; i < 256; i += kWgThreads) lut[i] = (float)i / 255.0f;
@@ -1994,8 +2010,8 @@
       if (valid) rd = load_rd(P, pr * (uint64_t)ss2 + kk);
       const uint64_t *pm = RFX_PRIM_LANES && SMALL && CULL && !STATS && P.prim_mask
                                ? P.prim_mask + (size_t)kPrimStride * t8 : nullptr;
-      const col c = trace<STATS, CULL, MANYL, SMALL, PLANES, ONEL, TBVH>(S, eye, ray, P.depth, rd, lut, cnt, valid, pm,
-                                                                  P.prim_shadow != 0);
+      const col c = trace<STATS, CULL, MANYL, SMALL, PLANES, ONEL, TBVH, BND>(S, eye, ray, P.depth, rd, lut, cnt, valid, pm,
+                                                                       P.prim_shadow != 0);
       {
 #ifdef RFX_LAUNDER_PARAMS
         const FrameParams &P = kernarg_params();
@@ -2120,7 +2136,7 @@
       const ParkTile park{P.park_after, P.queue, P.queue_count, P, wv, w8};
       const uint64_t *pm_tile = (SMALL || RFX_PRIM_LARGE) && CULL && !STATS && P.prim_mask
                                     ? P.prim_mask + (size_t)(SMALL ? kPrimStride : kPrimLargeStride) * t8 : nullptr;
-      const col c = trace_from<STATS, CULL, MANYL, SMALL, PLANES, PARK, ParkTile, ONEL, TBVH>(S, eye, ray, mkc(1.0f, 1.0f, 1.0f),
+      const col c = trace_from<STATS, CULL, MANYL, SMALL, PLANES, PARK, ParkTile, ONEL, TBVH, BND>(S, eye, ray, mkc(1.0f, 1.0f, 1.0f),
                                                                   mkc(0.0f, 0.0f, 0.0f), 0, P.depth, rd, lut, cnt,
                                                                   valid, park, parked, pm_tile);
       out = cadd(mkc(0.0f, 0.0f, 0.0f), c);
@@ -2562,6 +2578,16 @@
 template <bool STATS, int MODE>
 inline void launch_cfg(int cfg, dim3 grid, const DevScene &S, const FrameParams &P, hipStream_t st)
 {
+  if (cfg & kCfgBounded)
+  {
+    if constexpr (!STATS && (MODE == kModePlain || MODE == kModeSsaaLanes))
+      switch (cfg & ~kCfgBounded)
+      {
+        case 5: launch_one<STATS, MODE, 5 | kCfgBounded>(grid, S, P, st); return;
+        case 5 | kCfgOneLight: launch_one<STATS, MODE, 5 | kCfgOneLight | kCfgBounded>(grid, S, P, st); return;
+      }
+    cfg &= ~kCfgBounded;
+  }
 #if RFX_TRI_BVH
   if (cfg & kCfgTriBvh)
   {
diff --git a/reflaxman_amd/csrc/rfx_types.h b/reflaxman_amd/csrc/rfx_types.h
--- a/reflaxman_amd/csrc/rfx_types.h
+++ b/reflaxman_amd/csrc/rfx_types.h
@@ -143,5 +143,6 @@
 constexpr int kPrimLargeChunks = 8, kPrimLargeStride = 4 + kPrimLargeChunks;
 constexpr int kCfgCull = 1, kCfgManyLights = 2, kCfgSmall = 4, kCfgPlanes = 8, kCfgPark = 16, kCfgOneLight = 32;
 constexpr int kCfgTriBvh = 64;
+constexpr int kCfgBounded = 128;
 
 }
diff --git a/reflaxman_amd/render.py b/reflaxman_amd/render.py
--- a/reflaxman_amd/render.py
+++ b/reflaxman_amd/render.py
@@ -166,6 +166,16 @@
         leader, rows = np.zeros(n, np.int32), np.zeros((n, 6), np.float32)
         check(L.rfx_scene_tri_mates(self._h, leader.ctypes.data_as(_lib._i32p), _lib.fptr(rows)), "Scene.tri_mates")
         return (leader, rows) if plane else leader
+
+    def div_bounds(self, frame: "_lib.Frame" = None) -> dict:
+        L = _lib.load()
+        b = _lib.DivBounds()
+        check(L.rfx_scene_div_bounds(self._h, C.byref(b)), "Scene.div_bounds")
+        if frame is not None:
+            out = _lib.DivBounds()
+            check(L.rfx_frame_div_bounds(C.byref(b), C.byref(frame), C.byref(out)), "Scene.div_bounds")
+            b = out
+        return {n: getattr(b, n) for n, _ in b._fields_}
 
     def addPlane(self, pos: Vector3, norm: Vector3, material: Material) -> Plane:
         obj = check(_lib.load().rfx_scene_add_plane(self._h, farr(Vector3(*pos)), farr(Vector3(*norm)), material.type,
@@ -308,6 +318,14 @@
     def set_prim_exact(self, on: bool):
         check(_lib.load().rfx_renderer_set_prim_exact(self._h, int(bool(on))), "set_prim_exact")
 
+    def set_div_bounded(self, on: bool):
+        check(_lib.load().rfx_renderer_set_div_bounded(self._h, int(bool(on))), "set_div_bounded")
+
+    def div_bounded(self):
+        b = _lib.DivBounds()
+        ran = check(_lib.load().rfx_renderer_div_bounded(self._h, C.byref(b)), "div_bounded")
+        return bool(ran), {n: getattr(b, n) for n, _ in b._fields_}
+
     def prim_masks(self) -> np.ndarray:
         L = _lib.load()
         n = C.c_uint64()
```
